# emreatilgan/P-Companion

Measured on AMD Instinct MI355X. Metric: triplets/sec (Product2Vec pretrain step: gather+fwd+bwd+Adam) + P-Companion joint step under `joint`, higher is better.
Workload: dtype f32

## Files before the change

### include/pcompanion_hip.h

```cpp
#ifndef PCOMPANION_HIP_H
#define PCOMPANION_HIP_H

#include <stddef.h>
#include <stdint.h>

#ifdef __cplusplus
extern "C" {
#endif

#define PC_OK 0
#define PC_EINVAL (-1)
#define PC_ESHAPE (-2)
#define PC_EWORKSPACE (-3)
#define PC_EBATCHNORM (-4)
#define PC_ECOMM (-5)

#define PC_D 128
#define PC_H 256
#define PC_HEADS 4
#define PC_L 64
#define PC_MAX_SEG 4
#define PC_BN_SYNC_DOUBLES (PC_MAX_SEG * 2 * 256 + PC_MAX_SEG)

#define PC_ABI_VERSION 8
int pc_abi_version(void);
enum { PC_OPT_SIDE_QUEUE = 1, PC_OPT_SORTED_TABLE_GRADIENTS = 2, PC_OPT_BN_FINALIZE_SIDE = 3, PC_OPT_FUSED_LOSS = 4,
       PC_OPT_FUSED_OUT_CHAIN = 5, PC_OPT_BN_FINALIZE_RIDES = 6 };
int pc_set_option(int option, int value);
int pc_get_option(int option, int* value);
int pc_release_device_state(void);
enum {
    PC_FLAG_EXP_NO_MFMA = 1, PC_FLAG_EXP_NO_SPLIT = 2, PC_FLAG_EXP_NO_LDSREAD = 4, PC_FLAG_EXP_NO_DMA = 8,
    PC_FLAG_EXP_NO_SLAB = 16, PC_FLAG_EXP_STAGGER = 32, PC_FLAG_EXP_DMA_L2 = 64, PC_FLAG_NT_TIMING = 128,
    PC_FLAG_JOINT_TIMING = 256, PC_FLAG_CHAIN_TIMING = 512, PC_FLAG_EXP_NO_BARRIER = 1024, PC_FLAG_EXP_NO_VMWAIT = 2048
};
unsigned pc_build_flags(void);

typedef struct {
    float p;
    uint64_t seed, offset;
} pc_dropout;

typedef struct {
    float *w0, *b0, *gamma, *beta, *w3, *b3, *w5, *b5;
    float *in_proj_w, *in_proj_b, *out_proj_w, *out_proj_b;
    float *running_mean, *running_var;
    int64_t *num_batches_tracked;
    pc_dropout dropout;
    int dim;
} pc_p2v_tensors;

typedef struct {
    int nseg;
    int start[PC_MAX_SEG + 1];
    int count[PC_MAX_SEG];
    int weighted_row;
    float weight;
    const float *row_weight;
    int row_weight_start, row_weight_rows;
} pc_segments;

typedef struct {
    float *h0;
    float *a2;
    float *bn_mean;
    float *bn_invstd;
    float *bn_scale;
    float *bn_shift;
    float *a1;
} pc_ffn_saved;

size_t pc_p2v_ffn_workspace_bytes(int rows);
int pc_p2v_ffn_forward_train(const pc_p2v_tensors *p, const float *table, const int32_t *idx,
                             int rows, const pc_segments *seg, int update_running,
                             float *y, const pc_ffn_saved *saved, void *ws, size_t ws_bytes,
                             void *stream);

int pc_p2v_ffn_forward_eval(const pc_p2v_tensors *p, const float *table, const int32_t *idx,
                            int rows, float *y, void *ws, size_t ws_bytes, void *stream);

int pc_p2v_ffn_backward(const pc_p2v_tensors *p, const pc_p2v_tensors *g, const float *table,
                        const int32_t *idx, int rows, const pc_segments *seg, const float *dy,
                        const pc_ffn_saved *saved, float *dx, int accumulate, void *ws,
                        size_t ws_bytes, void *stream);

typedef struct {
    float *q, *qt, *probs, *c, *sp, *ctx;
} pc_attn_saved;
size_t pc_p2v_attention_workspace_bytes(int batch, int n_keys);
size_t pc_p2v_attention_workspace_bytes_dim(int batch, int n_keys, int dim);
int pc_p2v_attention_forward(const pc_p2v_tensors *p, const float *query, const float *keys,
                             int batch, int n_keys, float *out, const pc_attn_saved *saved,
                             void *ws, size_t ws_bytes, void *stream);
int pc_p2v_attention_backward(const pc_p2v_tensors *p, const pc_p2v_tensors *g,
                              const float *query, const float *keys, int batch, int n_keys,
                              const float *dout, const pc_attn_saved *saved, float *dquery,
                              float *dkeys, int accumulate, void *ws, size_t ws_bytes,
                              void *stream);
int pc_p2v_attention_forward_masked(const pc_p2v_tensors *p, const float *query, const float *keys,
                                    const uint8_t *key_pad, int batch, int n_keys, float *out,
                                    const pc_attn_saved *saved, void *ws, size_t ws_bytes, void *stream);
int pc_p2v_attention_backward_masked(const pc_p2v_tensors *p, const pc_p2v_tensors *g,
                                     const float *query, const float *keys, const uint8_t *key_pad, int batch,
                                     int n_keys, const float *dout, const pc_attn_saved *saved, float *dquery,
                                     float *dkeys, int accumulate, void *ws, size_t ws_bytes, void *stream);

size_t pc_p2v_export_workspace_bytes(int chunk_rows, int dim);
int pc_p2v_export_embeddings(const pc_p2v_tensors *p, const float *features, int64_t n_products,
                             const int32_t *cv_rowptr, const int32_t *cv_col, float *e1, float *out,
                             int chunk_rows, void *ws, size_t ws_bytes, void *stream);

int pc_p2v_triplet_loss(const float *a, const float *p, const float *n, int batch, int k_neg,
                        float margin, float *loss, float *d_pos, float *d_neg, float *da,
                        float *dp, float *dn, void *stream);
int pc_p2v_triplet_loss_dim(const float *a, const float *p, const float *n, int batch, int k_neg, int dim,
                            float margin, float *loss, float *d_pos, float *d_neg, float *da,
                            float *dp, float *dn, void *stream);

int pc_adam_step(float *param, const float *grad, float *exp_avg, float *exp_avg_sq, size_t n,
                 int64_t *step_count, float *scalars, double lr, double beta1, double beta2,
                 double eps, void *stream);
int pc_adam_step_at(float *param, const float *grad, float *exp_avg, float *exp_avg_sq, size_t n,
                    int64_t *step_count, int64_t t, double lr, double beta1, double beta2, double eps,
                    void *stream);

size_t pc_p2v_train_step_workspace_bytes(int batch, int n_nbr, int k_neg);
size_t pc_p2v_train_step_workspace_bytes_dim(int batch, int n_nbr, int k_neg, int dim);
int pc_p2v_train_step(const pc_p2v_tensors *p, const pc_p2v_tensors *g, const float *table,
                      const int32_t *anchor_idx, const int32_t *positive_idx,
                      const int32_t *negative_idx, const int32_t *neighbor_idx, int batch,
                      int n_nbr, int k_neg, float margin, float *loss, float *d_pos,
                      float *d_neg, float *anchor_emb, void *profile, void *ws, size_t ws_bytes,
                      void *stream);

int pc_p2v_train_step_compact(const pc_p2v_tensors *p, const pc_p2v_tensors *g, const float *table,
                              const int32_t *anchor_idx, const int32_t *positive_idx,
                              const int32_t *negative_idx, const int32_t *nb_rows, int n_real,
                              const int32_t *slot_row, int batch, int n_nbr, int k_neg, float margin,
                              float *loss, float *d_pos, float *d_neg, float *anchor_emb, void *profile,
                              void *ws, size_t ws_bytes, void *stream);

int pc_p2v_train_step_unique(const pc_p2v_tensors *p, const pc_p2v_tensors *g, const float *table,
                             const int32_t *anchor_idx, const int32_t *positive_idx,
                             const int32_t *negative_idx, const int32_t *nb_rows, const float *nb_weight,
                             int n_unique, const int32_t *slot_row, const int32_t *ref_off,
                             const int32_t *ref_slot, int batch, int n_nbr, int k_neg,
                             float margin, float *loss, float *d_pos, float *d_neg, float *anchor_emb,
                             void *profile, int phase, double *fwd_sums, double *bwd_local,
                             const double *bwd_global, void *ws, size_t ws_bytes, void *stream);

int pc_p2v_train_step_compact_sync(const pc_p2v_tensors *p, const pc_p2v_tensors *g, const float *table,
                                   const int32_t *anchor_idx, const int32_t *positive_idx,
                                   const int32_t *negative_idx, const int32_t *nb_rows, int n_real,
                                   const int32_t *slot_row, int batch, int n_nbr, int k_neg, float margin,
                                   float *loss, float *d_pos, float *d_neg, float *anchor_emb, int phase,
                                   double *fwd_sums, double *bwd_local, const double *bwd_global,
                                   void *ws, size_t ws_bytes, void *stream);
int pc_build_similarity_batch_compact(const int32_t *pair_ids, int batch, const int32_t *sim_pairs,
                                      const int32_t *cv_rowptr, const int32_t *cv_col,
                                      const int32_t *sim_rowptr, const int32_t *sim_col,
                                      int n_products, int n_pad, int k_neg, uint64_t seed,
                                      uint64_t step, int32_t *anchor_idx, int32_t *positive_idx,
                                      int32_t *negative_idx, int32_t *nb_rows, int32_t *slot_row,
                                      int32_t *row_off, void *stream);

size_t pc_build_similarity_batch_unique_scratch_bytes(int n_products, int max_slots );
int pc_build_similarity_batch_unique(const int32_t *pair_ids, int batch, const int32_t *sim_pairs,
                                     const int32_t *cv_rowptr, const int32_t *cv_col,
                                     const int32_t *sim_rowptr, const int32_t *sim_col, int n_products,
                                     int n_pad, int k_neg, uint64_t seed, uint64_t step, int n_real,
                                     int32_t *anchor_idx, int32_t *positive_idx, int32_t *negative_idx,
                                     int32_t *nb_rows, float *nb_weight, int32_t *slot_row,
                                     int32_t *ref_off, int32_t *ref_slot, int32_t *n_unique, void *scratch,
                                     size_t scratch_bytes, void *stream);

int pc_profile_create(int capacity, void **out);
int pc_profile_destroy(void *profile);
int pc_profile_set_kinds(void *prof, unsigned kinds);
int pc_profile_reset(void *profile);
int pc_profile_summary(void *profile, int kind, int *launches, double *total_ms,
                       double *total_flops);

int pc_build_similarity_batch(const int32_t *pair_ids, int batch, const int32_t *sim_pairs,
                              const int32_t *cv_rowptr, const int32_t *cv_col,
                              const int32_t *sim_rowptr, const int32_t *sim_col, int n_products,
                              int n_pad, int k_neg, uint64_t seed, uint64_t step,
                              int32_t *anchor_idx, int32_t *positive_idx, int32_t *negative_idx,
                              int32_t *neighbor_idx, void *stream);

int pc_build_complementary_batch(const int32_t *pairs, int batch, const float *features,
                                 const int32_t *type_idx, int n_types, uint64_t seed, uint64_t step,
                                 int32_t *query_idx, int32_t *query_types, int32_t *pos_types,
                                 int32_t *neg_types, float *pos_items, float *neg_items,
                                 float *target_features, void *stream);
int pc_build_complementary_batch_dim(const int32_t *pairs, int batch, const float *features,
                                     const int32_t *type_idx, int n_types, int dim, uint64_t seed, uint64_t step,
                                     int32_t *query_idx, int32_t *query_types, int32_t *pos_types,
                                     int32_t *neg_types, float *pos_items, float *neg_items,
                                     float *target_features, void *stream);

size_t pc_mt_state_bytes(void);
int pc_mt_seed(void *state, uint64_t seed);
uint32_t pc_mt_getrandbits(void *state, int k);
uint64_t pc_mt_randbelow(void *state, uint64_t n);
int pc_mt_shuffle(void *state, int64_t *perm, int64_t n);
int pc_mt_negative_samples(void *state, int32_t n_products, const int32_t *sim_rowptr,
                           const int32_t *sim_col, const int32_t *anchors, int64_t n, int k,
                           int32_t *out);

typedef struct {
    float *product_table;
    float *enc_w, *enc_b;
    float *dec_w, *dec_b;
    float *typ_w, *typ_b;
    float *itm_w, *itm_b;
    float *query_types;
    float *comp_types;
    pc_dropout dropout;
} pc_joint_tensors;

typedef struct {
    float *h;
    float *c;
    float *pi;
    float *tp;
} pc_joint_saved;

size_t pc_joint_workspace_bytes(int batch, int num_types, int k);
int pc_joint_forward(const pc_joint_tensors *p, const int32_t *query_idx,
                     const int32_t *query_types, int batch, int num_types, int k, float *sims,
                     int32_t *topk, float *proj, const pc_joint_saved *saved, void *ws,
                     size_t ws_bytes, void *stream);

int pc_joint_loss(const float *sims, const float *proj, const int32_t *pos_types,
                  const int32_t *neg_types, const float *pos_items, const float *neg_items,
                  int batch, int num_types, int k, float margin, float alpha, float *losses,
                  float *dsims_val, float *dproj, float *partials, void *stream);
int pc_joint_loss_dim(const float *sims, const float *proj, const int32_t *pos_types, const int32_t *neg_types,
                      const float *pos_items, const float *neg_items, int batch, int num_types, int k, int dim,
                      float margin, float alpha, float *losses, float *dsims_val, float *dproj, float *partials,
                      void *stream);

int pc_expand_type_grad(const float *dsims_val, const int32_t *pos_types,
                        const int32_t *neg_types, int batch, int num_types, float *dense,
                        void *stream);

int pc_joint_backward(const pc_joint_tensors *p, const pc_joint_tensors *g,
                      const int32_t *query_idx, const int32_t *query_types,
                      const int32_t *pos_types, const int32_t *neg_types, const int32_t *topk,
                      int batch, int num_types, int k, const float *dsims_val,
                      const float *dproj, const pc_joint_saved *saved, void *ws,
                      size_t ws_bytes, void *stream);

int pc_joint_train_step(const pc_joint_tensors *p, const pc_joint_tensors *g,
                        const int32_t *query_idx, const int32_t *query_types,
                        const int32_t *pos_types, const int32_t *neg_types,
                        const float *pos_items, const float *neg_items, int batch,
                        int num_types, int k, float margin, float alpha, float *losses,
                        int32_t *topk, void *ws, size_t ws_bytes, void *stream);

size_t pc_joint_fused_workspace_bytes(int batch, int num_types, int k);
int pc_joint_fused_supported(int num_types, int k, float dropout_p);
int pc_joint_fused_touched(void *ws, size_t ws_bytes, int batch, int num_types, int k, const int32_t **rows_comp,
                           const int32_t **rows_query, const int32_t **n_touched);
int pc_joint_fused_step(const pc_joint_tensors *p, const pc_joint_tensors *g, const pc_joint_tensors *exp_avg,
                        const pc_joint_tensors *exp_avg_sq, int64_t *step_count, double lr, double beta1,
                        double beta2, double eps, const int32_t *query_idx, const int32_t *query_types,
                        const int32_t *pos_types, const int32_t *neg_types, const float *pos_items,
                        const float *neg_items, int batch, int num_types, int k, int num_products, float margin,
                        float alpha, float *losses, int32_t *topk, int32_t *bad_count, void *ws, size_t ws_bytes,
                        void *stream);

int pc_joint_fused_step_pairs(const pc_joint_tensors *p, const pc_joint_tensors *g, const pc_joint_tensors *exp_avg,
                              const pc_joint_tensors *exp_avg_sq, int64_t *step_count, double lr, double beta1,
                              double beta2, double eps, const int32_t *pairs, const float *features,
                              const int32_t *type_idx, int n_types, uint64_t seed, uint64_t step,
                              int32_t *query_idx, int32_t *query_types, int32_t *pos_types, int32_t *neg_types,
                              float *pos_items, float *neg_items, int batch, int num_types, int k, int num_products,
                              float margin, float alpha, float *losses, int32_t *topk, int32_t *bad_count, void *ws,
                              size_t ws_bytes, void *stream);

int pc_joint_train_epoch(const pc_joint_tensors *p, const pc_joint_tensors *g, const pc_joint_tensors *exp_avg,
                         const pc_joint_tensors *exp_avg_sq, int64_t *step_count, double lr, double beta1,
                         double beta2, double eps, const int32_t *pairs, int64_t n_pairs, const float *features,
                         const int32_t *type_idx, int n_types, uint64_t seed, uint64_t first_step,
                         int32_t *query_idx, int32_t *query_types, int32_t *pos_types, int32_t *neg_types,
                         float *pos_items, float *neg_items, int batch, int drop_last, int num_types, int k,
                         int num_products, float margin, float alpha, float *losses_out, int32_t *topk,
                         int32_t *bad_count, void *ws, size_t ws_bytes, void *stream);

typedef struct pc_adam_fused {
    float *param, *grad, *exp_avg, *exp_avg_sq;
    size_t n;
    int64_t *step_count;
    int64_t t;
    double lr, beta1, beta2, eps;
} pc_adam_fused;
int pc_p2v_train_step_unique_adam(const pc_p2v_tensors *p, const pc_p2v_tensors *g, const float *table,
                                  const int32_t *anchor_idx, const int32_t *positive_idx,
                                  const int32_t *negative_idx, const int32_t *nb_rows, const float *nb_weight,
                                  int n_unique, const int32_t *slot_row, const int32_t *ref_off,
                                  const int32_t *ref_slot, int batch, int n_nbr, int k_neg, float margin,
                                  float *loss, float *d_pos, float *d_neg, float *anchor_emb, void *profile,
                                  void *ws, size_t ws_bytes, const pc_adam_fused *adam, void *stream);

int pc_p2v_concat_step_rows(const int32_t *anchor_idx, const int32_t *positive_idx, const int32_t *negative_idx,
                            const int32_t *nb_rows, const int32_t *n_unique_dev, int nb_capacity, int batch, int k_neg,
                            int32_t *rows_out, int rows_capacity, void *stream);
int pc_p2v_train_step_unique_rows(const pc_p2v_tensors *p, const pc_p2v_tensors *g, const float *table,
                                  const int32_t *step_rows, const int32_t *nb_rows, const float *nb_weight, int n_unique,
                                  const int32_t *slot_row, const int32_t *ref_off, const int32_t *ref_slot, int batch,
                                  int n_nbr, int k_neg, float margin, float *loss, float *d_pos, float *d_neg,
                                  float *anchor_emb, void *profile, void *ws, size_t ws_bytes, const pc_adam_fused *adam,
                                  void *stream);

int pc_p2v_train_step_compact_masked(const pc_p2v_tensors *p, const pc_p2v_tensors *g, const float *table,
                                     const int32_t *anchor_idx, const int32_t *positive_idx,
                                     const int32_t *negative_idx, const int32_t *nb_rows, int n_real,
                                     const int32_t *slot_row, int batch, int n_nbr, int k_neg, float margin,
                                     float *loss, float *d_pos, float *d_neg, float *anchor_emb, void *profile,
                                     void *ws, size_t ws_bytes, void *stream);
int pc_p2v_train_step_unique_masked(const pc_p2v_tensors *p, const pc_p2v_tensors *g, const float *table,
                                    const int32_t *anchor_idx, const int32_t *positive_idx,
                                    const int32_t *negative_idx, const int32_t *step_rows, const int32_t *nb_rows,
                                    const float *nb_weight, int n_unique, int n_real_slots, const int32_t *slot_row,
                                    const int32_t *ref_off, const int32_t *ref_slot, int batch, int n_nbr, int k_neg,
                                    float margin, float *loss, float *d_pos, float *d_neg, float *anchor_emb,
                                    void *profile, void *ws, size_t ws_bytes, const pc_adam_fused *adam, void *stream);

typedef int (*pc_exchange_fn)(void *ctx, float *grad, size_t n, void *stream);

int pc_exchange_adam(pc_exchange_fn exchange, void *exchange_ctx, float *param, float *grad, float *exp_avg,
                     float *exp_avg_sq, size_t n, int64_t *step_count, int64_t t, float *scalars, double lr,
                     double beta1, double beta2, double eps, void *stream);

typedef int (*pc_shard_collective_fn)(void *ctx, float *buf, size_t n_per_rank, void *stream);
typedef struct pc_exchange_plan {
    pc_exchange_fn all_reduce_mean;
    pc_shard_collective_fn reduce_scatter_mean;
    pc_shard_collective_fn all_gather;
    void *ctx;
    int rank, world;
    int shard_optimizer;
} pc_exchange_plan;
int pc_rccl_reduce_scatter_mean(void *comm, float *buf, size_t n_per_rank, void *stream);
int pc_rccl_all_gather(void *comm, float *buf, size_t n_per_rank, void *stream);
int pc_exchange_adam_plan(const pc_exchange_plan *plan, float *param, float *grad, float *exp_avg, float *exp_avg_sq,
                          size_t n, int64_t *step_count, int64_t t, float *scalars, double lr, double beta1, double beta2,
                          double eps, void *stream);

int pc_joint_train_epoch_dp(const pc_joint_tensors *p, const pc_joint_tensors *g, float *param_flat, float *grad_flat,
                            float *exp_avg_flat, float *exp_avg_sq_flat, size_t n_flat, int64_t *step_count,
                            int64_t t_first, float *adam_scalars, double lr, double beta1, double beta2, double eps,
                            pc_exchange_fn exchange, void *exchange_ctx, const int32_t *pairs, int64_t n_pairs,
                            const float *features, const int32_t *type_idx, int n_types, uint64_t seed,
                            uint64_t first_step, int32_t *query_idx, int32_t *query_types, int32_t *pos_types,
                            int32_t *neg_types, float *pos_items, float *neg_items, int batch, int drop_last,
                            int num_types, int k, int num_products, float margin, float alpha, float *losses_out,
                            int32_t *topk, int32_t *bad_count, void *ws, size_t ws_bytes, void *stream);

int pc_joint_train_epoch_plan(const pc_joint_tensors *p, const pc_joint_tensors *g, float *param_flat, float *grad_flat,
                              float *exp_avg_flat, float *exp_avg_sq_flat, size_t n_flat, int64_t *step_count,
                              int64_t t_first, float *adam_scalars, double lr, double beta1, double beta2, double eps,
                              const pc_exchange_plan *plan, const int32_t *pairs, int64_t n_pairs,
                              const float *features, const int32_t *type_idx, int n_types, uint64_t seed,
                              uint64_t first_step, int32_t *query_idx, int32_t *query_types, int32_t *pos_types,
                              int32_t *neg_types, float *pos_items, float *neg_items, int batch, int drop_last,
                              int num_types, int k, int num_products, float margin, float alpha, float *losses_out,
                              int32_t *topk, int32_t *bad_count, void *ws, size_t ws_bytes, void *stream);

int pc_rccl_available(void);
int pc_rccl_unique_id(void *out_128_bytes);
int pc_rccl_comm_create(const void *unique_id_128_bytes, int rank, int world, void **comm_out);
int pc_rccl_comm_destroy(void *comm);
int pc_rccl_allreduce_mean(void *comm, float *grad, size_t n, void *stream);
int pc_rccl_allreduce_sum_f64(void *comm, double *buf, size_t n, void *stream);
int pc_rccl_alltoall(void *comm, const void *send, void *recv, size_t bytes_per_peer, void *stream);
int pc_rccl_comm_stats(void *comm, int64_t *issued, int64_t *chained);
const char *pc_rccl_last_error(void);

int pc_linear_forward(const float *x, const int32_t *idx, int rows, int in_dim, const float *w,
                      const float *b, int out_dim, int act, float *y, void *stream);
int pc_linear_backward_input(const float *dy, int rows, int out_dim, const float *w, int in_dim,
                             int act, const float *y_saved, float *dx, float *wt_scratch,
                             void *stream);
size_t pc_linear_backward_weight_workspace_bytes(int rows, int out_dim, int in_dim);
int pc_linear_backward_weight(const float *dy, int rows, int out_dim, const float *x,
                              const int32_t *idx, int in_dim, float *dw, float *db,
                              int accumulate, void *ws, size_t ws_bytes, void *stream);
int pc_topk_rows(const float *sims, int batch, int num_types, int k, int32_t *idx_out,
                 float *val_out, void *stream);
int pc_hit_rank(const float *sims, int rows, int cols, int32_t *rank, void *stream);
int pc_cosine_rows(const float *x, const float *y, int batch, int k, float *out, void *stream);
int pc_cosine_rows_dim(const float *x, const float *y, int batch, int k, int dim, float *out, void *stream);

int pc_eval_batch_stats(const float *proj, const float *targets, const float *pos_items, const int32_t *types, int batch,
                        int k, int dim, int32_t *stats, float *cos_sum, void *ws, size_t ws_bytes, void *stream);
size_t pc_joint_eval_workspace_bytes(int batch, int num_types, int k, int dim);
int pc_joint_eval_epoch(const pc_joint_tensors *p, const int32_t *pairs, int64_t n_pairs, const float *features,
                        const int32_t *type_idx, int n_types, int dim, uint64_t seed, uint64_t first_step, int batch,
                        int num_types, int k, int num_products, int32_t *stats_out, float *cos_sum_out, double *metrics_out,
                        int32_t *bad_count, void *ws, size_t ws_bytes, void *stream);

int pc_hadamard_forward(const float *pi, const float *tp, int batch, int k, float *proj,
                        void *stream);
int pc_hadamard_forward_dim(const float *pi, const float *tp, int batch, int k, int dim, float *proj, void *stream);
int pc_hadamard_backward(const float *dproj, const float *pi, const float *tp, int batch, int k,
                         float *dpi, float *dtp, void *stream);
int pc_hadamard_backward_dim(const float *dproj, const float *pi, const float *tp, int batch, int k, int dim,
                             float *dpi, float *dtp, void *stream);

int pc_gather_rows(const float *table, const int32_t *idx, int rows, int width, float *out,
                   void *stream);
int pc_scatter_add_rows(float *table, const int32_t *idx, int rows, int width, const float *src,
                        void *stream);
int pc_scatter_add_rows_small(float *table, int table_rows, const int32_t *idx, int rows, int width,
                              const float *src, void *stream);

int pc_scatter_rows(float *out, const int32_t *idx, int rows, int width, const float *src,
                    void *stream);
int pc_act_backward(const float *dy, const float *y, size_t n, int act, float *dx, void *stream);

int pc_sample_negatives_zipf(const int32_t *pair_ids, int batch, const int32_t *sim_pairs,
                             const int32_t *sim_rowptr, const int32_t *sim_col, int n_products, int k_neg,
                             uint64_t seed, uint64_t step, const uint32_t *octave_cum, int n_octaves,
                             const int32_t *perm, int32_t *negative_idx, int32_t *failed, void *stream);

int pc_gen_types(int64_t n_products, int num_types, uint64_t seed, int32_t *type_idx, void *stream);
int pc_gen_features(int64_t first, int64_t stride, int64_t n_local, int dim, int num_types, uint64_t seed,
                    float *features, void *stream);
int pc_gen_degrees(int64_t n_products, double mean_degree, int degree_cap, double comp_mean, uint64_t seed,
                   int32_t *deg, int32_t *comp_cand, void *stream);
size_t pc_scan_scratch_bytes(int64_t n);
int pc_exclusive_scan_i32(const int32_t *in, int64_t n, int32_t *out, int64_t *total_out, void *scratch,
                          size_t scratch_bytes, void *stream);
int pc_gen_coview(int64_t n_products, int num_types, uint64_t seed, const int32_t *cv_rowptr, int32_t *cv_col,
                  int32_t *sim_count, void *stream);
int pc_gen_similarity(int64_t n_products, const int32_t *cv_rowptr, int32_t *cv_col, const int32_t *sim_rowptr,
                      int32_t *sim_pairs, int32_t *sim_col, int32_t *pair_deg, void *stream);
int pc_gen_complementary(int64_t n_products, int num_types, uint64_t seed, const int32_t *comp_cand,
                         const int32_t *cv_rowptr, const int32_t *cv_col, int32_t *count,
                         const int32_t *comp_rowptr, int32_t *comp_pairs, void *stream);

int pc_ingest_count(const int32_t *edges, int64_t n_edges, int64_t n_products, int list_bit, int32_t *cnt, int32_t *bad,
                    void *stream);
int pc_ingest_scatter(const int32_t *edges, int64_t n_edges, int64_t n_products, const int32_t *rowptr, int32_t *cursor,
                      int32_t *bucket, void *stream);
int pc_ingest_row_limits(int *wave_row_max, int *lds_row_max);
size_t pc_ingest_rows_workspace_bytes(int64_t n_products);
int pc_ingest_rows(int64_t n_products, const int32_t *rowptr, int32_t *bucket, int32_t *scratch, int degree_cap,
                   int32_t *full_cnt, int32_t *kept_cnt, int32_t *max_kept, void *ws, size_t ws_bytes, void *stream);
int pc_ingest_flag(int64_t n_products, int32_t *src, const int32_t *src_rowptr, const int32_t *src_cnt, const int32_t *need,
                   const int32_t *need_rowptr, const int32_t *need_cnt, const int32_t *forbid1,
                   const int32_t *forbid1_rowptr, const int32_t *forbid1_cnt, const int32_t *forbid2,
                   const int32_t *forbid2_rowptr, const int32_t *forbid2_cnt, int32_t *count, void *stream);
int pc_ingest_emit(int64_t n_products, int32_t *src, const int32_t *src_rowptr, const int32_t *src_cnt,
                   const int32_t *out_rowptr, int32_t *out_col, int32_t *out_pairs, int32_t *out_deg,
                   const int32_t *deg_rowptr, int clear, void *stream);

int pc_epoch_permutation(int n, uint64_t seed, uint64_t epoch, int32_t *out, void *stream);
int pc_shuffle_rows_i32(const int32_t *rows, int n, int width, uint64_t seed, uint64_t epoch, int32_t *out,
                        void *stream);
int pc_comp_split_pairs(const int32_t *comp_pairs, int64_t n_comp, const int32_t *sim_pairs, int64_t n_sim, int64_t lo,
                        int64_t hi, uint64_t seed, int mode, int32_t *out, void *stream);
int pc_epoch_plan(const int32_t *order, const int32_t *deg, int n, int batch, int n_batches, int64_t *plan,
                  void *stream);

int pc_shard_bucket(const int32_t *const *ids, const int *n, const int32_t *const *n_dev, const int *n_dev_add,
                    int32_t *const *remap_out, int count, int world, int capacity, int32_t *counts,
                    int32_t *send_ids, int32_t *overflow, void *stream);
int pc_shard_bucket_hot(const int32_t *const *ids, const int *n, const int32_t *const *n_dev, const int *n_dev_add,
                        int32_t *const *remap_out, int count, int world, int capacity, const int32_t *hot_ids,
                        int hot_rows, int32_t *counts, int32_t *send_ids, int32_t *overflow, int32_t *hot_served,
                        void *stream);

int pc_dropout_hidden(const float *x, size_t n, const pc_dropout *d, float *y, void *stream);

int pc_check_indices(const int32_t *const *idx, const int *n, const int *hi, const int *allow_pad, int count,
                     int32_t *bad, void *stream);

int pc_retrieve_topk(const float *proj, const int32_t *types, int rows, const int32_t *type_rowptr,
                     const int32_t *type_col, const float *table, int n_types, int n, int32_t *out_idx,
                     float *out_score, void *stream);
int pc_retrieve_topk_dim(const float *proj, const int32_t *types, int rows, const int32_t *type_rowptr,
                        const int32_t *type_col, const float *table, int n_types, int n, int dim, int32_t *out_idx,
                        float *out_score, void *stream);
size_t pc_retrieve_topk_grouped_workspace_bytes(int rows, int n_types, int n, int slices);
int pc_retrieve_topk_grouped(const float *proj, const int32_t *types, int rows, const int32_t *type_rowptr,
                             const int32_t *type_col, const float *table, int n_types, int n, int dim, int slices,
                             int32_t *out_idx, float *out_score, void *ws, size_t ws_bytes, void *stream);

size_t pc_rank_grouped_workspace_bytes(int rows, int n_types, int slices);
int pc_rank_grouped(const float *proj, const int32_t *types, const int32_t *targets, int rows,
                    const int32_t *type_rowptr, const int32_t *type_col, const float *table,
                    int n_types, int num_products, int dim, int slices,
                    int32_t *rank_out, int32_t *bad_count, void *ws, size_t ws_bytes, void *stream);

size_t pc_retrieve_topk_grouped_excluding_workspace_bytes(int rows, int n_types, int n, int slices);
int pc_retrieve_topk_grouped_excluding(const float *proj, const int32_t *types, const int32_t *row_key, int rows,
                                       const int32_t *type_rowptr, const int32_t *type_col, const float *table, int n_types,
                                       const int32_t *ex_rowptr, const int32_t *ex_col, int n_keys, int n, int dim, int slices,
                                       int32_t *out_idx, float *out_score, int32_t *bad_count, void *ws, size_t ws_bytes,
                                       void *stream);
int pc_rank_grouped_excluding(const float *proj, const int32_t *types, const int32_t *targets, const int32_t *row_key, int rows,
                              const int32_t *type_rowptr, const int32_t *type_col, const float *table, int n_types,
                              int num_products, const int32_t *ex_rowptr, const int32_t *ex_col, int n_keys,
                              const int32_t *cand_type, int dim, int slices, int32_t *rank_out, int32_t *bad_count, void *ws,
                              size_t ws_bytes, void *stream);

size_t pc_retrieve_list_grouped_workspace_bytes(int rows, int n_types, int n, int slices);
int pc_retrieve_list_grouped(const float *proj, const int32_t *types, const int32_t *row_key, int rows,
                             const int32_t *type_rowptr, const int32_t *type_col, const float *table, int n_types,
                             const int32_t *ex_rowptr, const int32_t *ex_col, int n_keys, int n, int dim, int slices,
                             int32_t *out_idx, float *out_score, int32_t *bad_count, void *ws, size_t ws_bytes,
                             void *stream);

size_t pc_retrieve_topk_grouped_bf16_workspace_bytes(int rows, int n_types, int n, int slices);
int pc_retrieve_topk_grouped_bf16(const float *proj, const int32_t *types, const int32_t *row_key, int rows,
                                  const int32_t *type_rowptr, const int32_t *type_col, const uint16_t *table_bf16,
                                  int n_types, const int32_t *ex_rowptr, const int32_t *ex_col, int n_keys, int n, int dim,
                                  int slices, int32_t *out_idx, float *out_score, int32_t *bad_count, void *ws,
                                  size_t ws_bytes, void *stream);

int pc_half_sq_norm_bias(const float *table, int rows, int dim, float *out, void *stream);
size_t pc_retrieve_topk_grouped_biased_workspace_bytes(int rows, int n_types, int n, int slices);
int pc_retrieve_topk_grouped_biased(const float *proj, const int32_t *types, const int32_t *row_key, int rows,
                                    const int32_t *type_rowptr, const int32_t *type_col, const float *table,
                                    const float *bias, int n_types, const int32_t *ex_rowptr, const int32_t *ex_col,
                                    int n_keys, int n, int dim, int slices, int32_t *out_idx, float *out_score,
                                    int32_t *bad_count, void *ws, size_t ws_bytes, void *stream);
size_t pc_rank_grouped_biased_workspace_bytes(int rows, int n_types, int slices);
int pc_rank_grouped_biased(const float *proj, const int32_t *types, const int32_t *targets, const int32_t *row_key, int rows,
                           const int32_t *type_rowptr, const int32_t *type_col, const float *table, const float *bias,
                           int n_types, int num_products, const int32_t *ex_rowptr, const int32_t *ex_col, int n_keys,
                           const int32_t *cand_type, int dim, int slices, int32_t *rank_out, int32_t *bad_count, void *ws,
                           size_t ws_bytes, void *stream);

size_t pc_joint_query_grad_workspace_bytes(int batch, int k, int dim);
int pc_joint_query_grad(const pc_joint_tensors *p, const int32_t *query_idx, const int32_t *topk, const float *pos_items,
                        const float *neg_items, int batch, int64_t num_products, int num_types, int k, int dim, float margin,
                        float alpha, float *dq, int32_t *bad, void *ws, size_t ws_bytes, void *stream);
size_t pc_sparse_adam_rows_workspace_bytes(int rows);
int pc_sparse_adam_rows(float *table, float *exp_avg, float *exp_avg_sq, int64_t num_products, int dim, const int32_t *idx,
                        const float *grad, int rows, int64_t t, double lr, double beta1, double beta2, double eps,
                        int32_t *bad, void *ws, size_t ws_bytes, void *stream);

int pc_cell_means(const float *table, const int32_t *cell_rowptr, const int32_t *cell_col, int n_cells, int num_products,
                  int dim, float *centroids, void *stream);
int pc_merge_lists(const int32_t *idx, const float *score, int rows, int L, int n, int32_t *out_idx, float *out_score,
                   void *stream);

int pc_diversify_lists(const int32_t *idx, const float *score, int rows, int m, const float *table, const float *scale,
                       int num_products, int dim, int n, float lam, int32_t *out_idx, float *out_score, int32_t *bad_count,
                       void *stream);
int pc_inv_norm(const float *table, int rows, int dim, float *out, void *stream);

size_t pc_retrieve_list_grouped_bf16_workspace_bytes(int rows, int n_types, int n, int slices);
int pc_retrieve_list_grouped_bf16(const float *proj, const int32_t *types, const int32_t *row_key, int rows,
                                  const int32_t *type_rowptr, const int32_t *type_col, const uint16_t *table_bf16,
                                  int n_types, const int32_t *ex_rowptr, const int32_t *ex_col, int n_keys, int n, int dim,
                                  int slices, int32_t *out_idx, float *out_score, int32_t *bad_count, void *ws,
                                  size_t ws_bytes, void *stream);
int pc_diversify_lists_bf16(const int32_t *idx, const float *score, int rows, int m, const uint16_t *table_bf16,
                            const float *scale, int num_products, int dim, int n, float lam, int32_t *out_idx,
                            float *out_score, int32_t *bad_count, void *stream);
int pc_inv_norm_bf16(const uint16_t *table_bf16, int rows, int dim, float *out, void *stream);

#ifdef __cplusplus
}
#endif
#endif
```

### p_companion_amd/_lib.py

```python
import ctypes
import os

_HERE = os.path.dirname(os.path.abspath(__file__))
LIB_PATH = os.path.join(_HERE, "libpcompanion_hip.so")
if os.environ.get("PC_DEV_LIB"):
    import sys as _sys
    LIB_PATH = os.path.abspath(os.environ["PC_DEV_LIB"])
    print(f"[p_companion_amd] PC_DEV_LIB: loading {LIB_PATH} instead of the in-tree library (developer A/B run)", file=_sys.stderr, flush=True)

c_f32p = ctypes.c_void_p
c_i32p = ctypes.c_void_p
PC_MAX_SEG = 4
D, H, HEADS, L = 128, 256, 4, 64

_ERR = {-1: "PC_EINVAL (null pointer / bad size)", -2: "PC_ESHAPE (unsupported dimension/alignment)",
        -3: "PC_EWORKSPACE (workspace too small)",
        -4: "PC_EBATCHNORM (a BatchNorm call group of one row in training mode)",
        -5: "PC_ECOMM (RCCL could not be loaded, or a communicator call failed)"}


class HipKernelError(RuntimeError):
    pass


class Dropout(ctypes.Structure):
    _fields_ = [("p", ctypes.c_float), ("seed", ctypes.c_uint64), ("offset", ctypes.c_uint64)]


class P2VTensors(ctypes.Structure):
    _fields_ = [(n, ctypes.c_void_p) for n in (
        "w0", "b0", "gamma", "beta", "w3", "b3", "w5", "b5", "in_proj_w", "in_proj_b", "out_proj_w",
        "out_proj_b", "running_mean", "running_var", "num_batches_tracked")] + [("dropout", Dropout), ("dim", ctypes.c_int)]


class Segments(ctypes.Structure):
    _fields_ = [("nseg", ctypes.c_int), ("start", ctypes.c_int * (PC_MAX_SEG + 1)),
                ("count", ctypes.c_int * PC_MAX_SEG), ("weighted_row", ctypes.c_int), ("weight", ctypes.c_float),
                ("row_weight", ctypes.c_void_p), ("row_weight_start", ctypes.c_int), ("row_weight_rows", ctypes.c_int)]


class FfnSaved(ctypes.Structure):
    _fields_ = [(n, ctypes.c_void_p) for n in ("h0", "a2", "bn_mean", "bn_invstd", "bn_scale", "bn_shift", "a1")]


class AttnSaved(ctypes.Structure):
    _fields_ = [(n, ctypes.c_void_p) for n in ("q", "qt", "probs", "c", "sp", "ctx")]


class JointTensors(ctypes.Structure):
    _fields_ = [(n, ctypes.c_void_p) for n in (
        "product_table", "enc_w", "enc_b", "dec_w", "dec_b", "typ_w", "typ_b", "itm_w", "itm_b",
        "query_types", "comp_types")] + [("dropout", Dropout)]


class JointSaved(ctypes.Structure):
    _fields_ = [(n, ctypes.c_void_p) for n in ("h", "c", "pi", "tp")]


_vp, _i, _sz, _f, _d, _u64, _i64 = (ctypes.c_void_p, ctypes.c_int, ctypes.c_size_t, ctypes.c_float,
                                    ctypes.c_double, ctypes.c_uint64, ctypes.c_int64)
_P = ctypes.POINTER

class AdamFused(ctypes.Structure):
    _fields_ = [("param", ctypes.c_void_p), ("grad", ctypes.c_void_p), ("exp_avg", ctypes.c_void_p), ("exp_avg_sq", ctypes.c_void_p),
                ("n", ctypes.c_size_t), ("step_count", ctypes.c_void_p), ("t", ctypes.c_int64),
                ("lr", ctypes.c_double), ("beta1", ctypes.c_double), ("beta2", ctypes.c_double), ("eps", ctypes.c_double)]


PC_OPT_SIDE_QUEUE = 1
PC_OPT_FUSED_OUT_CHAIN = 5
PC_OPT_FUSED_LOSS = 4
PC_OPT_BN_FINALIZE_SIDE = 3
PC_OPT_BN_FINALIZE_RIDES = 6
PC_OPT_SORTED_TABLE_GRADIENTS = 2

SIGNATURES = {
    "pc_abi_version": (_i, []),
    "pc_build_flags": (ctypes.c_uint, []),
    "pc_set_option": (_i, [_i, _i]),
    "pc_get_option": (_i, [_i, ctypes.POINTER(ctypes.c_int)]),
    "pc_release_device_state": (_i, []),
    "pc_p2v_ffn_workspace_bytes": (_sz, [_i]),
    "pc_p2v_ffn_forward_train": (_i, [_P(P2VTensors), _vp, _vp, _i, _P(Segments), _i, _vp, _P(FfnSaved), _vp, _sz, _vp]),
    "pc_p2v_ffn_forward_eval": (_i, [_P(P2VTensors), _vp, _vp, _i, _vp, _vp, _sz, _vp]),
    "pc_p2v_ffn_backward": (_i, [_P(P2VTensors), _P(P2VTensors), _vp, _vp, _i, _P(Segments), _vp, _P(FfnSaved),
                                 _vp, _i, _vp, _sz, _vp]),
    "pc_p2v_attention_workspace_bytes": (_sz, [_i, _i]),
    "pc_p2v_attention_workspace_bytes_dim": (_sz, [_i, _i, _i]),
    "pc_p2v_attention_forward": (_i, [_P(P2VTensors), _vp, _vp, _i, _i, _vp, _P(AttnSaved), _vp, _sz, _vp]),
    "pc_p2v_attention_backward": (_i, [_P(P2VTensors), _P(P2VTensors), _vp, _vp, _i, _i, _vp, _P(AttnSaved), _vp,
                                       _vp, _i, _vp, _sz, _vp]),
    "pc_p2v_attention_forward_masked": (_i, [_P(P2VTensors), _vp, _vp, _vp, _i, _i, _vp, _P(AttnSaved), _vp, _sz, _vp]),
    "pc_p2v_attention_backward_masked": (_i, [_P(P2VTensors), _P(P2VTensors), _vp, _vp, _vp, _i, _i, _vp, _P(AttnSaved), _vp,
                                              _vp, _i, _vp, _sz, _vp]),
    "pc_p2v_train_step_compact_masked": (_i, [_P(P2VTensors), _P(P2VTensors), _vp, _vp, _vp, _vp, _vp, _i, _vp, _i, _i, _i, _f,
                                              _vp, _vp, _vp, _vp, _vp, _vp, _sz, _vp]),
    "pc_p2v_train_step_unique_masked": (_i, [_P(P2VTensors), _P(P2VTensors), _vp, _vp, _vp, _vp, _vp, _vp, _vp, _i, _i, _vp, _vp,
                                             _vp, _i, _i, _i, _f, _vp, _vp, _vp, _vp, _vp, _vp, _sz, _P(AdamFused), _vp]),
    "pc_p2v_export_workspace_bytes": (_sz, [_i, _i]),
    "pc_p2v_export_embeddings": (_i, [_P(P2VTensors), _vp, _i64, _vp, _vp, _vp, _vp, _i, _vp, _sz, _vp]),
    "pc_p2v_triplet_loss": (_i, [_vp, _vp, _vp, _i, _i, _f, _vp, _vp, _vp, _vp, _vp, _vp, _vp]),
    "pc_p2v_triplet_loss_dim": (_i, [_vp, _vp, _vp, _i, _i, _i, _f, _vp, _vp, _vp, _vp, _vp, _vp, _vp]),
    "pc_adam_step": (_i, [_vp, _vp, _vp, _vp, _sz, _vp, _vp, _d, _d, _d, _d, _vp]),
    "pc_adam_step_at": (_i, [_vp, _vp, _vp, _vp, _sz, _vp, _i64, _d, _d, _d, _d, _vp]),
    "pc_p2v_train_step_workspace_bytes": (_sz, [_i, _i, _i]),
    "pc_p2v_train_step_workspace_bytes_dim": (_sz, [_i, _i, _i, _i]),
    "pc_p2v_train_step": (_i, [_P(P2VTensors), _P(P2VTensors), _vp, _vp, _vp, _vp, _vp, _i, _i, _i, _f, _vp, _vp,
                               _vp, _vp, _vp, _vp, _sz, _vp]),
    "pc_p2v_train_step_compact": (_i, [_P(P2VTensors), _P(P2VTensors), _vp, _vp, _vp, _vp, _vp, _i, _vp, _i, _i, _i, _f,
                                       _vp, _vp, _vp, _vp, _vp, _vp, _sz, _vp]),
    "pc_p2v_train_step_unique_adam": (_i, [_P(P2VTensors), _P(P2VTensors), _vp, _vp, _vp, _vp, _vp, _vp, _i, _vp, _vp, _vp, _i, _i,
                                           _i, _f, _vp, _vp, _vp, _vp, _vp, _vp, _sz, _P(AdamFused), _vp]),
    "pc_p2v_concat_step_rows": (_i, [_vp, _vp, _vp, _vp, _vp, _i, _i, _i, _vp, _i, _vp]),
    "pc_p2v_train_step_unique_rows": (_i, [_P(P2VTensors), _P(P2VTensors), _vp, _vp, _vp, _vp, _i, _vp, _vp, _vp, _i, _i,
                                           _i, _f, _vp, _vp, _vp, _vp, _vp, _vp, _sz, _P(AdamFused), _vp]),
    "pc_p2v_train_step_unique": (_i, [_P(P2VTensors), _P(P2VTensors), _vp, _vp, _vp, _vp, _vp, _vp, _i, _vp, _vp, _vp, _i, _i,
                                      _i, _f, _vp, _vp, _vp, _vp, _vp, _i, _vp, _vp, _vp, _vp, _sz, _vp]),
    "pc_build_similarity_batch_unique_scratch_bytes": (_sz, [_i, _i]),
    "pc_build_similarity_batch_unique": (_i, [_vp, _i, _vp, _vp, _vp, _vp, _vp, _i, _i, _i, _u64, _u64, _i, _vp, _vp, _vp,
                                              _vp, _vp, _vp, _vp, _vp, _vp, _vp, _sz, _vp]),
    "pc_p2v_train_step_compact_sync": (_i, [_P(P2VTensors), _P(P2VTensors), _vp, _vp, _vp, _vp, _vp, _i, _vp, _i, _i, _i,
                                            _f, _vp, _vp, _vp, _vp, _i, _vp, _vp, _vp, _vp, _sz, _vp]),
    "pc_build_similarity_batch_compact": (_i, [_vp, _i, _vp, _vp, _vp, _vp, _vp, _i, _i, _i, _u64, _u64, _vp, _vp, _vp,
                                               _vp, _vp, _vp, _vp]),
    "pc_profile_create": (_i, [_i, _P(ctypes.c_void_p)]),
    "pc_profile_destroy": (_i, [_vp]),
    "pc_profile_reset": (_i, [_vp]),
    "pc_profile_set_kinds": (_i, [_vp, ctypes.c_uint]),
    "pc_profile_summary": (_i, [_vp, _i, _P(ctypes.c_int), _P(ctypes.c_double), _P(ctypes.c_double)]),
    "pc_build_similarity_batch": (_i, [_vp, _i, _vp, _vp, _vp, _vp, _vp, _i, _i, _i, _u64, _u64, _vp, _vp, _vp,
                                       _vp, _vp]),
    "pc_build_complementary_batch": (_i, [_vp, _i, _vp, _vp, _i, _u64, _u64, _vp, _vp, _vp, _vp, _vp, _vp, _vp, _vp]),
    "pc_build_complementary_batch_dim": (_i, [_vp, _i, _vp, _vp, _i, _i, _u64, _u64, _vp, _vp, _vp, _vp, _vp, _vp, _vp, _vp]),
    "pc_mt_state_bytes": (_sz, []),
    "pc_mt_seed": (_i, [_vp, _u64]),
    "pc_mt_getrandbits": (ctypes.c_uint32, [_vp, _i]),
    "pc_mt_randbelow": (_u64, [_vp, _u64]),
    "pc_mt_shuffle": (_i, [_vp, _vp, _i64]),
    "pc_mt_negative_samples": (_i, [_vp, ctypes.c_int32, _vp, _vp, _vp, _i64, _i, _vp]),
    "pc_joint_workspace_bytes": (_sz, [_i, _i, _i]),
    "pc_joint_forward": (_i, [_P(JointTensors), _vp, _vp, _i, _i, _i, _vp, _vp, _vp, _P(JointSaved), _vp, _sz, _vp]),
    "pc_joint_loss": (_i, [_vp, _vp, _vp, _vp, _vp, _vp, _i, _i, _i, _f, _f, _vp, _vp, _vp, _vp, _vp]),
    "pc_joint_loss_dim": (_i, [_vp, _vp, _vp, _vp, _vp, _vp, _i, _i, _i, _i, _f, _f, _vp, _vp, _vp, _vp, _vp]),
    "pc_expand_type_grad": (_i, [_vp, _vp, _vp, _i, _i, _vp, _vp]),
    "pc_joint_backward": (_i, [_P(JointTensors), _P(JointTensors), _vp, _vp, _vp, _vp, _vp, _i, _i, _i, _vp, _vp,
                               _P(JointSaved), _vp, _sz, _vp]),
    "pc_joint_train_step": (_i, [_P(JointTensors), _P(JointTensors), _vp, _vp, _vp, _vp, _vp, _vp, _i, _i, _i, _f,
                                 _f, _vp, _vp, _vp, _sz, _vp]),
    "pc_joint_fused_workspace_bytes": (_sz, [_i, _i, _i]),
    "pc_joint_fused_supported": (_i, [_i, _i, _f]),
    "pc_joint_fused_touched": (_i, [_vp, _sz, _i, _i, _i, _P(ctypes.c_void_p), _P(ctypes.c_void_p), _P(ctypes.c_void_p)]),
    "pc_joint_fused_step": (_i, [_P(JointTensors), _P(JointTensors), _P(JointTensors), _P(JointTensors), _vp, _d, _d, _d, _d,
                                 _vp, _vp, _vp, _vp, _vp, _vp, _i, _i, _i, _i, _f, _f, _vp, _vp, _vp, _vp, _sz, _vp]),
    "pc_joint_fused_step_pairs": (_i, [_P(JointTensors), _P(JointTensors), _P(JointTensors), _P(JointTensors), _vp, _d, _d, _d, _d,
                                       _vp, _vp, _vp, _i, _u64, _u64, _vp, _vp, _vp, _vp, _vp, _vp, _i, _i, _i, _i, _f, _f,
                                       _vp, _vp, _vp, _vp, _sz, _vp]),
    "pc_joint_train_epoch": (_i, [_P(JointTensors), _P(JointTensors), _P(JointTensors), _P(JointTensors), _vp, _d, _d, _d, _d,
                                  _vp, _i64, _vp, _vp, _i, _u64, _u64, _vp, _vp, _vp, _vp, _vp, _vp, _i, _i, _i, _i, _i, _f, _f,
                                  _vp, _vp, _vp, _vp, _sz, _vp]),
    "pc_exchange_adam": (_i, [_vp, _vp, _vp, _vp, _vp, _vp, _sz, _vp, _i64, _vp, _d, _d, _d, _d, _vp]),
    "pc_joint_train_epoch_dp": (_i, [_P(JointTensors), _P(JointTensors), _vp, _vp, _vp, _vp, _sz, _vp, _i64, _vp, _d, _d, _d, _d,
                                     _vp, _vp, _vp, _i64, _vp, _vp, _i, _u64, _u64, _vp, _vp, _vp, _vp, _vp, _vp, _i, _i, _i, _i,
                                     _i, _f, _f, _vp, _vp, _vp, _vp, _sz, _vp]),
    "pc_exchange_adam_plan": (_i, [_vp, _vp, _vp, _vp, _vp, _sz, _vp, _i64, _vp, _d, _d, _d, _d, _vp]),
    "pc_joint_train_epoch_plan": (_i, [_P(JointTensors), _P(JointTensors), _vp, _vp, _vp, _vp, _sz, _vp, _i64, _vp, _d, _d, _d, _d,
                                       _vp, _vp, _i64, _vp, _vp, _i, _u64, _u64, _vp, _vp, _vp, _vp, _vp, _vp, _i, _i, _i, _i,
                                       _i, _f, _f, _vp, _vp, _vp, _vp, _sz, _vp]),
    "pc_rccl_reduce_scatter_mean": (_i, [_vp, _vp, _sz, _vp]),
    "pc_rccl_all_gather": (_i, [_vp, _vp, _sz, _vp]),
    "pc_rccl_available": (_i, []),
    "pc_rccl_unique_id": (_i, [_vp]),
    "pc_rccl_comm_create": (_i, [_vp, _i, _i, _P(ctypes.c_void_p)]),
    "pc_rccl_comm_destroy": (_i, [_vp]),
    "pc_rccl_allreduce_mean": (_i, [_vp, _vp, _sz, _vp]),
    "pc_rccl_allreduce_sum_f64": (_i, [_vp, _vp, _sz, _vp]),
    "pc_rccl_alltoall": (_i, [_vp, _vp, _vp, _sz, _vp]),
    "pc_rccl_comm_stats": (_i, [_vp, _P(ctypes.c_int64), _P(ctypes.c_int64)]),
    "pc_rccl_last_error": (ctypes.c_char_p, []),
    "pc_linear_forward": (_i, [_vp, _vp, _i, _i, _vp, _vp, _i, _i, _vp, _vp]),
    "pc_linear_backward_input": (_i, [_vp, _i, _i, _vp, _i, _i, _vp, _vp, _vp, _vp]),
    "pc_linear_backward_weight_workspace_bytes": (_sz, [_i, _i, _i]),
    "pc_linear_backward_weight": (_i, [_vp, _i, _i, _vp, _vp, _i, _vp, _vp, _i, _vp, _sz, _vp]),
    "pc_topk_rows": (_i, [_vp, _i, _i, _i, _vp, _vp, _vp]),
    "pc_hit_rank": (_i, [_vp, _i, _i, _vp, _vp]),
    "pc_cosine_rows": (_i, [_vp, _vp, _i, _i, _vp, _vp]),
    "pc_cosine_rows_dim": (_i, [_vp, _vp, _i, _i, _i, _vp, _vp]),
    "pc_eval_batch_stats": (_i, [_vp, _vp, _vp, _vp, _i, _i, _i, _vp, _vp, _vp, _sz, _vp]),
    "pc_joint_eval_workspace_bytes": (_sz, [_i, _i, _i, _i]),
    "pc_joint_eval_epoch": (_i, [_P(JointTensors), _vp, _i64, _vp, _vp, _i, _i, _u64, _u64, _i, _i, _i, _i, _vp, _vp, _vp,
                                 _vp, _vp, _sz, _vp]),
    "pc_retrieve_topk": (_i, [_vp, _vp, _i, _vp, _vp, _vp, _i, _i, _vp, _vp, _vp]),
    "pc_retrieve_topk_dim": (_i, [_vp, _vp, _i, _vp, _vp, _vp, _i, _i, _i, _vp, _vp, _vp]),
    "pc_retrieve_topk_grouped_workspace_bytes": (_sz, [_i, _i, _i, _i]),
    "pc_retrieve_topk_grouped": (_i, [_vp, _vp, _i, _vp, _vp, _vp, _i, _i, _i, _i, _vp, _vp, _vp, _sz, _vp]),
    "pc_rank_grouped_workspace_bytes": (_sz, [_i, _i, _i]),
    "pc_rank_grouped": (_i, [_vp, _vp, _vp, _i, _vp, _vp, _vp, _i, _i, _i, _i, _vp, _vp, _vp, _sz, _vp]),
    "pc_retrieve_topk_grouped_excluding_workspace_bytes": (_sz, [_i, _i, _i, _i]),
    "pc_retrieve_topk_grouped_excluding": (_i, [_vp, _vp, _vp, _i, _vp, _vp, _vp, _i, _vp, _vp, _i, _i, _i, _i, _vp, _vp, _vp, _vp,
                                                _sz, _vp]),
    "pc_rank_grouped_excluding": (_i, [_vp, _vp, _vp, _vp, _i, _vp, _vp, _vp, _i, _i, _vp, _vp, _i, _vp, _i, _i, _vp, _vp, _vp, _sz,
                                       _vp]),
    "pc_retrieve_list_grouped_workspace_bytes": (_sz, [_i, _i, _i, _i]),
    "pc_retrieve_list_grouped": (_i, [_vp, _vp, _vp, _i, _vp, _vp, _vp, _i, _vp, _vp, _i, _i, _i, _i, _vp, _vp, _vp, _vp, _sz,
                                      _vp]),
    "pc_retrieve_topk_grouped_bf16_workspace_bytes": (_sz, [_i, _i, _i, _i]),
    "pc_retrieve_topk_grouped_bf16": (_i, [_vp, _vp, _vp, _i, _vp, _vp, _vp, _i, _vp, _vp, _i, _i, _i, _i, _vp, _vp, _vp, _vp,
                                           _sz, _vp]),
    "pc_half_sq_norm_bias": (_i, [_vp, _i, _i, _vp, _vp]),
    "pc_retrieve_topk_grouped_biased_workspace_bytes": (_sz, [_i, _i, _i, _i]),
    "pc_retrieve_topk_grouped_biased": (_i, [_vp, _vp, _vp, _i, _vp, _vp, _vp, _vp, _i, _vp, _vp, _i, _i, _i, _i, _vp, _vp, _vp,
                                             _vp, _sz, _vp]),
    "pc_rank_grouped_biased_workspace_bytes": (_sz, [_i, _i, _i]),
    "pc_rank_grouped_biased": (_i, [_vp, _vp, _vp, _vp, _i, _vp, _vp, _vp, _vp, _i, _i, _vp, _vp, _i, _vp, _i, _i, _vp, _vp, _vp,
                                    _sz, _vp]),
    "pc_joint_query_grad_workspace_bytes": (_sz, [_i, _i, _i]),
    "pc_joint_query_grad": (_i, [_P(JointTensors), _vp, _vp, _vp, _vp, _i, _i64, _i, _i, _i, _f, _f, _vp, _vp, _vp, _sz, _vp]),
    "pc_sparse_adam_rows_workspace_bytes": (_sz, [_i]),
    "pc_sparse_adam_rows": (_i, [_vp, _vp, _vp, _i64, _i, _vp, _vp, _i, _i64, _d, _d, _d, _d, _vp, _vp, _sz, _vp]),
    "pc_cell_means": (_i, [_vp, _vp, _vp, _i, _i, _i, _vp, _vp]),
    "pc_merge_lists": (_i, [_vp, _vp, _i, _i, _i, _vp, _vp, _vp]),
    "pc_diversify_lists": (_i, [_vp, _vp, _i, _i, _vp, _vp, _i, _i, _i, _f, _vp, _vp, _vp, _vp]),
    "pc_inv_norm": (_i, [_vp, _i, _i, _vp, _vp]),
    "pc_retrieve_list_grouped_bf16_workspace_bytes": (_sz, [_i, _i, _i, _i]),
    "pc_retrieve_list_grouped_bf16": (_i, [_vp, _vp, _vp, _i, _vp, _vp, _vp, _i, _vp, _vp, _i, _i, _i, _i, _vp, _vp, _vp, _vp,
                                           _sz, _vp]),
    "pc_diversify_lists_bf16": (_i, [_vp, _vp, _i, _i, _vp, _vp, _i, _i, _i, _f, _vp, _vp, _vp, _vp]),
    "pc_inv_norm_bf16": (_i, [_vp, _i, _i, _vp, _vp]),
    "pc_hadamard_forward":(_i, [_vp, _vp, _i, _i, _vp, _vp]),
    "pc_hadamard_forward_dim": (_i, [_vp, _vp, _i, _i, _i, _vp, _vp]),
    "pc_hadamard_backward": (_i, [_vp, _vp, _vp, _i, _i, _vp, _vp, _vp]),
    "pc_hadamard_backward_dim": (_i, [_vp, _vp, _vp, _i, _i, _i, _vp, _vp, _vp]),
    "pc_gather_rows": (_i, [_vp, _vp, _i, _i, _vp, _vp]),
    "pc_scatter_add_rows": (_i, [_vp, _vp, _i, _i, _vp, _vp]),
    "pc_scatter_add_rows_small": (_i, [_vp, _i, _vp, _i, _i, _vp, _vp]),
    "pc_scatter_rows": (_i, [_vp, _vp, _i, _i, _vp, _vp]),
    "pc_act_backward": (_i, [_vp, _vp, _sz, _i, _vp, _vp]),
    "pc_sample_negatives_zipf": (_i, [_vp, _i, _vp, _vp, _vp, _i, _i, _u64, _u64, _vp, _i, _vp, _vp, _vp, _vp]),
    "pc_epoch_permutation": (_i, [_i, _u64, _u64, _vp, _vp]),
    "pc_gen_types": (_i, [_i64, _i, _u64, _vp, _vp]),
    "pc_gen_features": (_i, [_i64, _i64, _i64, _i, _i, _u64, _vp, _vp]),
    "pc_gen_degrees": (_i, [_i64, ctypes.c_double, _i, ctypes.c_double, _u64, _vp, _vp, _vp]),
    "pc_scan_scratch_bytes": (_sz, [_i64]),
    "pc_exclusive_scan_i32": (_i, [_vp, _i64, _vp, _vp, _vp, _sz, _vp]),
    "pc_gen_coview": (_i, [_i64, _i, _u64, _vp, _vp, _vp, _vp]),
    "pc_gen_similarity": (_i, [_i64, _vp, _vp, _vp, _vp, _vp, _vp, _vp]),
    "pc_gen_complementary": (_i, [_i64, _i, _u64, _vp, _vp, _vp, _vp, _vp, _vp, _vp]),
    "pc_ingest_count": (_i, [_vp, _i64, _i64, _i, _vp, _vp, _vp]),
    "pc_ingest_scatter": (_i, [_vp, _i64, _i64, _vp, _vp, _vp, _vp]),
    "pc_ingest_row_limits": (_i, [_P(ctypes.c_int), _P(ctypes.c_int)]),
    "pc_ingest_rows_workspace_bytes": (_sz, [_i64]),
    "pc_ingest_rows": (_i, [_i64, _vp, _vp, _vp, _i, _vp, _vp, _vp, _vp, _sz, _vp]),
    "pc_ingest_flag": (_i, [_i64, _vp, _vp, _vp, _vp, _vp, _vp, _vp, _vp, _vp, _vp, _vp, _vp, _vp, _vp]),
    "pc_ingest_emit": (_i, [_i64, _vp, _vp, _vp, _vp, _vp, _vp, _vp, _vp, _i, _vp]),
    "pc_shuffle_rows_i32": (_i, [_vp, _i, _i, _u64, _u64, _vp, _vp]),
    "pc_comp_split_pairs": (_i, [_vp, _i64, _vp, _i64, _i64, _i64, _u64, _i, _vp, _vp]),
    "pc_epoch_plan": (_i, [_vp, _vp, _i, _i, _i, _vp, _vp]),
    "pc_shard_bucket": (_i, [_P(ctypes.c_void_p), _P(ctypes.c_int), _P(ctypes.c_void_p), _P(ctypes.c_int), _P(ctypes.c_void_p),
                             _i, _i, _i, _vp, _vp, _vp, _vp]),
    "pc_shard_bucket_hot": (_i, [_P(ctypes.c_void_p), _P(ctypes.c_int), _P(ctypes.c_void_p), _P(ctypes.c_int), _P(ctypes.c_void_p),
                                 _i, _i, _i, _vp, _i, _vp, _vp, _vp, _vp, _vp]),
    "pc_dropout_hidden": (_i, [_vp, _sz, _P(Dropout), _vp, _vp]),
    "pc_check_indices": (_i, [_P(ctypes.c_void_p), _P(ctypes.c_int), _P(ctypes.c_int), _P(ctypes.c_int), _i, _vp, _vp]),
}

_lib = None


def lib():
    global _lib
    if _lib is None:
        if not os.path.exists(LIB_PATH):
            raise HipKernelError(
                f"{LIB_PATH} not found: build it with `python -m p_companion_amd.build` "
                "(hipcc --offload-arch=gfx950).  There is no CPU fallback.")
        import torch
        L = ctypes.CDLL(LIB_PATH)
        for name, (res, args) in SIGNATURES.items():
            fn = getattr(L, name)
            fn.restype = res
            fn.argtypes = args
        _lib = L
    return _lib


def check(rc, what):
    if rc == 0:
        return
    if rc == -4:
        raise ValueError(f"Expected more than 1 value per channel when training, got input size torch.Size([1, {H}])")
    if rc == -5:
        raise HipKernelError(f"{what}: {_ERR[rc]}: {lib().pc_rccl_last_error().decode(errors='replace')}")
    if rc < 0:
        raise HipKernelError(f"{what}: {_ERR.get(rc, rc)}")
    raise HipKernelError(f"{what}: hipError_t {rc}")
```

### p_companion_amd/csrc/common.h

```cpp
#pragma once
#include <hip/hip_runtime.h>
#include <stdint.h>
#include "../../include/pcompanion_hip.h"

typedef float f32x16 __attribute__((ext_vector_type(16)));
typedef float f32x4 __attribute__((ext_vector_type(4)));

#define PC_WAVE 64

#define PC_HIP_TRY(expr)                          \
    do {                                          \
        hipError_t _e = (expr);                   \
        if (_e != hipSuccess) return (int)_e;     \
    } while (0)

#define PC_TRY(expr)                 \
    do {                             \
        int _r = (expr);             \
        if (_r != 0) return _r;      \
    } while (0)

extern thread_local int pc_tls_launch_err;
#define PC_LAUNCH(...)                                                           \
    do {                                                                         \
        (void)hipGetLastError();                                                 \
        hipLaunchKernelGGL(__VA_ARGS__);                                         \
        const hipError_t _le = hipGetLastError();                                \
        if (_le != hipSuccess && pc_tls_launch_err == 0) pc_tls_launch_err = (int)_le; \
    } while (0)

static inline int pc_launch_status() {
    const int e = pc_tls_launch_err;
    pc_tls_launch_err = 0;
    return e;
}

struct SegInfo {
    int nseg;
    int start[PC_MAX_SEG + 1];
    int tile0[PC_MAX_SEG + 1];
    int count[PC_MAX_SEG];
    int wrow;
    float wmult;
    const float* roww;
    int w0, wn;
};

static inline SegInfo make_seginfo(const pc_segments* s, int rows, int tile_rows) {
    SegInfo si;
    si.nseg = 1;
    for (int i = 0; i <= PC_MAX_SEG; i++) { si.start[i] = rows; si.tile0[i] = 0; }
    si.start[0] = 0;
    si.wrow = -1;
    si.wmult = 1.f;
    si.roww = nullptr; si.w0 = 0; si.wn = 0;
    if (s) {
        si.nseg = s->nseg;
        for (int i = 0; i <= s->nseg; i++) si.start[i] = s->start[i];
        for (int i = s->nseg + 1; i <= PC_MAX_SEG; i++) si.start[i] = s->start[s->nseg];
        si.wrow = s->weighted_row;
        si.wmult = s->weight;
        if (s->row_weight && s->row_weight_rows > 0) { si.roww = s->row_weight; si.w0 = s->row_weight_start; si.wn = s->row_weight_rows; }
    }
    for (int i = 0; i < PC_MAX_SEG; i++) {
        const int phys = si.start[i + 1] - si.start[i];
        si.count[i] = (s && i < s->nseg && s->count[i] > 0) ? s->count[i] : phys;
    }
    int t = 0;
    for (int i = 0; i < PC_MAX_SEG; i++) {
        si.tile0[i] = t;
        int n = si.start[i + 1] - si.start[i];
        t += (n + tile_rows - 1) / tile_rows;
    }
    si.tile0[PC_MAX_SEG] = t;
    return si;
}

static inline int seg_valid(const pc_segments* s, int rows) {
    if (!s) return 1;
    if (s->nseg < 1 || s->nseg > PC_MAX_SEG || s->start[0] != 0 || s->start[s->nseg] != rows) return 0;
    for (int i = 0; i < s->nseg; i++)
        if (s->start[i + 1] < s->start[i] || s->count[i] < 0) return 0;
    if (s->weighted_row >= rows || (s->weighted_row >= 0 && s->weight < 0.f)) return 0;
    if (s->row_weight && (s->row_weight_start < 0 || s->row_weight_rows < 0 || s->row_weight_start + s->row_weight_rows > rows))
        return 0;
    return 1;
}

#ifdef __HIPCC__
__device__ __forceinline__ int seg_of_row(const SegInfo& si, int r) {
    int s = 0;
#pragma unroll
    for (int i = 1; i < PC_MAX_SEG; i++) s += (i < si.nseg && r >= si.start[i]) ? 1 : 0;
    return s;
}

__device__ __forceinline__ float row_multiplicity(const SegInfo& si, int r) {
#ifdef PC_EXP_NO_ROWMULT
    return 1.f;
#endif
    if (si.roww && (unsigned)(r - si.w0) < (unsigned)si.wn) return si.roww[r - si.w0];
    return r == si.wrow ? si.wmult : 1.f;
}

__device__ __forceinline__ int seg_of_tile(const SegInfo& si, int t) {
    int s = 0;
#pragma unroll
    for (int i = 1; i < PC_MAX_SEG; i++) s += (i < si.nseg && t >= si.tile0[i]) ? 1 : 0;
    return s;
}

__device__ __forceinline__ float fast_tanh(float x) {
    const float e = __builtin_amdgcn_exp2f(x * 2.8853900817779268f);
    return 1.0f - 2.0f * __builtin_amdgcn_rcpf(e + 1.0f);
}

__device__ __forceinline__ float wave_sum(float v) {
#pragma unroll
    for (int o = 32; o >= 1; o >>= 1) v += __shfl_xor(v, o, 64);
    return v;
}

__device__ __forceinline__ float group16_sum(float v) {
#pragma unroll
    for (int o = 8; o >= 1; o >>= 1) v += __shfl_xor(v, o, 64);
    return v;
}

__device__ __forceinline__ f32x16 mfma32(float a, float b, f32x16 c) {
    return __builtin_amdgcn_mfma_f32_32x32x2f32(a, b, c, 0, 0, 0);
}

typedef __bf16 bf16x8 __attribute__((ext_vector_type(8)));
struct Split3 { bf16x8 p0, p1, p2; };
__device__ __forceinline__ Split3 split3(const float4& lo, const float4& hi) {
    const float v[8] = {lo.x, lo.y, lo.z, lo.w, hi.x, hi.y, hi.z, hi.w};
    unsigned u0[8], u1[8], u2[8];
#pragma unroll
    for (int i = 0; i < 8; i++) {
        u0[i] = __float_as_uint(v[i]);
        const float r1 = v[i] - __uint_as_float(u0[i] & 0xffff0000u);
        u1[i] = __float_as_uint(r1);
        const float r2 = r1 - __uint_as_float(u1[i] & 0xffff0000u);
        u2[i] = __float_as_uint(r2);
    }
    typedef unsigned u32x4 __attribute__((ext_vector_type(4)));
    u32x4 q0, q1, q2;
#pragma unroll
    for (int j = 0; j < 4; j++) {
        q0[j] = __builtin_amdgcn_perm(u0[2 * j + 1], u0[2 * j], 0x07060302u);
        q1[j] = __builtin_amdgcn_perm(u1[2 * j + 1], u1[2 * j], 0x07060302u);
        q2[j] = __builtin_amdgcn_perm(u2[2 * j + 1], u2[2 * j], 0x07060302u);
    }
    Split3 s;
    s.p0 = __builtin_bit_cast(bf16x8, q0);
    s.p1 = __builtin_bit_cast(bf16x8, q1);
    s.p2 = __builtin_bit_cast(bf16x8, q2);
    return s;
}
__device__ __forceinline__ f32x16 mfma_bf16(const bf16x8& a, const bf16x8& b, f32x16 c) {
    return __builtin_amdgcn_mfma_f32_32x32x16_bf16(a, b, c, 0, 0, 0);
}
#define PC_PRIO_MFMA(COND, x) do { if constexpr (COND) __builtin_amdgcn_s_setprio(x); } while (0)
#ifndef PC_PRIO_NT_COND
#define PC_PRIO_NT_COND false
#endif
#ifndef PC_PRIO_TN_COND
#define PC_PRIO_TN_COND (!APRO && !ZPRO)
#endif
#endif

struct DropCfg {
    unsigned thr;
    float scale;
    unsigned k0, k1, c2, c3;
};
enum { PC_DROP_STREAM_ATTENTION = 0, PC_DROP_STREAM_HIDDEN = 1 };
static inline DropCfg make_dropcfg(const pc_dropout& d) {
    DropCfg c = {};
    if (d.p > 0.f) {
        double t = (double)d.p * 4294967296.0;
        c.thr = t >= 4294967295.0 ? 4294967295u : (unsigned)t;
        c.scale = 1.0f / (1.0f - d.p);
        c.k0 = (unsigned)d.seed; c.k1 = (unsigned)(d.seed >> 32);
        c.c2 = (unsigned)d.offset; c.c3 = (unsigned)(d.offset >> 32);
    }
    return c;
}
#ifdef __HIPCC__
__device__ __forceinline__ void pc_dropout_keep4(const DropCfg& c, unsigned group, unsigned stream, float (&m)[4]) {
    unsigned x0 = group, x1 = stream, x2 = c.c2, x3 = c.c3, k0 = c.k0, k1 = c.k1;
#pragma unroll
    for (int r = 0; r < 10; r++) {
        const unsigned long long p0 = (unsigned long long)0xD2511F53u * x0, p1 = (unsigned long long)0xCD9E8D57u * x2;
        const unsigned y0 = (unsigned)(p1 >> 32) ^ x1 ^ k0, y1 = (unsigned)p1;
        const unsigned y2 = (unsigned)(p0 >> 32) ^ x3 ^ k1, y3 = (unsigned)p0;
        x0 = y0; x1 = y1; x2 = y2; x3 = y3;
        k0 += 0x9E3779B9u; k1 += 0xBB67AE85u;
    }
    m[0] = x0 >= c.thr ? c.scale : 0.f; m[1] = x1 >= c.thr ? c.scale : 0.f;
    m[2] = x2 >= c.thr ? c.scale : 0.f; m[3] = x3 >= c.thr ? c.scale : 0.f;
}
__device__ __forceinline__ void pc_adam_update(float& p, float& m, float& v, float g, float step_size, float bc2s,
                                               float omb1, float beta2, float omb2, float eps) {
#pragma clang fp contract(off)
    m = m + (g - m) * omb1;
    v = v * beta2 + (omb2 * g) * g;
    p = p - step_size * (m / (sqrtf(v) / bc2s + eps));
}
__device__ __forceinline__ bool pc_adam_dead(const float4& g, const float4& m, const float4& v) {
    return g.x == 0.f && g.y == 0.f && g.z == 0.f && g.w == 0.f && m.x == 0.f && m.y == 0.f && m.z == 0.f && m.w == 0.f &&
           v.x == 0.f && v.y == 0.f && v.z == 0.f && v.w == 0.f;
}
__device__ __forceinline__ float2 pc_box_muller(uint32_t a, uint32_t b) {
    const float u1 = ((float)(a >> 8) + 0.5f) * (1.0f / 16777216.0f);
    const float u2 = ((float)(b >> 8) + 0.5f) * (1.0f / 16777216.0f);
    const float r = sqrtf(-2.0f * __logf(u1));
    float sn, cs;
    __sincosf(6.283185307179586f * u2, &sn, &cs);
    return make_float2(r * cs, r * sn);
}
__device__ __forceinline__ float4 pc_filler_chunk(uint64_t seed, uint64_t step, uint32_t t) {
    uint32_t x0 = 0u, x1 = t, x2 = (uint32_t)step, x3 = (uint32_t)(step >> 32), k0 = (uint32_t)seed, k1 = (uint32_t)(seed >> 32);
#pragma unroll
    for (int r = 0; r < 10; r++) {
        const uint64_t p0 = (uint64_t)0xD2511F53u * x0, p1 = (uint64_t)0xCD9E8D57u * x2;
        const uint32_t y0 = (uint32_t)(p1 >> 32) ^ x1 ^ k0, y1 = (uint32_t)p1;
        const uint32_t y2 = (uint32_t)(p0 >> 32) ^ x3 ^ k1, y3 = (uint32_t)p0;
        x0 = y0; x1 = y1; x2 = y2; x3 = y3;
        k0 += 0x9E3779B9u; k1 += 0xBB67AE85u;
    }
    const float2 n0 = pc_box_muller(x0, x1), n1 = pc_box_muller(x2, x3);
    return make_float4(n0.x, n0.y, n1.x, n1.y);
}
#endif

#ifdef __HIPCC__
struct Philox {
    uint32_t c[4], k[2], out[4];
    int have;
    __device__ Philox(uint64_t seed, uint64_t step, uint32_t sample) {
        k[0] = (uint32_t)seed; k[1] = (uint32_t)(seed >> 32);
        c[0] = 0; c[1] = sample; c[2] = (uint32_t)step; c[3] = (uint32_t)(step >> 32);
        have = 0;
    }
    __device__ void block() {
        uint32_t x0 = c[0], x1 = c[1], x2 = c[2], x3 = c[3], k0 = k[0], k1 = k[1];
#pragma unroll
        for (int r = 0; r < 10; r++) {
            const uint64_t p0 = (uint64_t)0xD2511F53u * x0, p1 = (uint64_t)0xCD9E8D57u * x2;
            const uint32_t y0 = (uint32_t)(p1 >> 32) ^ x1 ^ k0, y1 = (uint32_t)p1;
            const uint32_t y2 = (uint32_t)(p0 >> 32) ^ x3 ^ k1, y3 = (uint32_t)p0;
            x0 = y0; x1 = y1; x2 = y2; x3 = y3;
            k0 += 0x9E3779B9u; k1 += 0xBB67AE85u;
        }
        out[0] = x0; out[1] = x1; out[2] = x2; out[3] = x3;
        c[0]++;
        have = 4;
    }
    __device__ uint32_t next() {
        if (have == 0) block();
        return out[4 - have--];
    }
    __device__ uint32_t below(uint32_t n) {
        const int bits = 32 - __clz(n);
        uint32_t r = next() >> (32 - bits);
        while (r >= n) r = next() >> (32 - bits);
        return r;
    }
};
#endif

struct pc_profile {
    hipEvent_t* ev;
    int* kind;
    double* flops;
    int capacity, used;
    unsigned kinds;
};
enum { PC_KIND_GEMM_NT = 0, PC_KIND_GEMM_TN = 1, PC_KIND_GEMM_NT_SMALL = 2 };
extern thread_local pc_profile* pc_tls_profile;
struct ProfileScope {
    explicit ProfileScope(pc_profile* p) { pc_tls_profile = p; }
    ~ProfileScope() { pc_tls_profile = nullptr; }
};
int pc_prof_begin(int kind, double flops, hipStream_t st);
void pc_prof_end(int bracket, hipStream_t st);

enum NtPrologue { NT_PRO_NONE = 0, NT_PRO_BNTANH = 1 };
enum NtEpilogue {
    NT_EPI_NONE = 0,
    NT_EPI_TANH = 1,
    NT_EPI_RELU = 2,
    NT_EPI_DTANH = 3,
    NT_EPI_DTANH_BN = 4,
    NT_EPI_DRELU = 5
};
enum NtStats {
    NT_STAT_NONE = 0,
    NT_STAT_SUMSQ = 1,
    NT_STAT_BNBWD = 2
};

struct NtArgs {
    const float* A; int lda; const int32_t* gather;
    const float* W; int ldw;
    const float* bias;
    float* C; int ldc;
    int M, N, K;
    SegInfo seg;
    int prologue; const float* pscale; const float* pshift;
    float* pro_out; int ldpo;
    int epilogue; const float* aux; int ldaux;
    const float* escale; const float* eshift;
    int stats; float* stat_sum; float* stat_aux;
    const float* mean; const float* invstd;
    const float* brs; int ldbrs;
};
int launch_gemm_nt(const NtArgs& a, hipStream_t st);
int gemm_nt_tiles(const SegInfo& si);
#define PC_NT_GROUP 8
struct NtSmallGroup { NtArgs a[PC_NT_GROUP]; int ks_log2[PC_NT_GROUP], block0[PC_NT_GROUP + 1], n; };
static_assert(sizeof(NtSmallGroup) <= 4096, "kernel argument segment");
int launch_gemm_nt_group(const NtArgs* args, int n, hipStream_t st);
enum { NT_MODE_PLAIN = 0, NT_MODE_KHEAD = 1, NT_MODE_AHEAD = 2 };
struct HingeMeanJob { const float* d_pos; const float* d_neg; int B; float margin; float* loss; };
#ifdef __HIPCC__
#define PC_LOSS_MAX_K 8
#define PC_PAIR_EPS 1e-6f
__device__ __forceinline__ void triplet_sample16(const float* __restrict__ a, const float* __restrict__ p, const float* __restrict__ n,
                                                 int b, int B, int K, float margin, bool live, float* d_pos, float* d_neg,
                                                 float* dp, float* dn, bool grads, int l16, float (&ga)[8]) {
    constexpr int D = 128;
    const size_t bb = live ? (size_t)b : 0;
    float av[8], dpv[8], dnv[PC_LOSS_MAX_K][8], dn_j[PC_LOSS_MAX_K];
    {
        const float4 a0 = *reinterpret_cast<const float4*>(a + bb * D + 8 * l16), a1 = *reinterpret_cast<const float4*>(a + bb * D + 8 * l16 + 4);
        const float4 p0 = *reinterpret_cast<const float4*>(p + bb * D + 8 * l16), p1 = *reinterpret_cast<const float4*>(p + bb * D + 8 * l16 + 4);
        av[0] = a0.x; av[1] = a0.y; av[2] = a0.z; av[3] = a0.w; av[4] = a1.x; av[5] = a1.y; av[6] = a1.z; av[7] = a1.w;
        const float pv[8] = {p0.x, p0.y, p0.z, p0.w, p1.x, p1.y, p1.z, p1.w};
#pragma unroll
        for (int c = 0; c < 8; c++) dpv[c] = av[c] - pv[c] + PC_PAIR_EPS;
    }
#pragma unroll
    for (int j = 0; j < PC_LOSS_MAX_K; j++)
        if (j < K) {
            const float* r = n + (bb * K + j) * D + 8 * l16;
            const float4 n0 = *reinterpret_cast<const float4*>(r), n1 = *reinterpret_cast<const float4*>(r + 4);
            const float nv[8] = {n0.x, n0.y, n0.z, n0.w, n1.x, n1.y, n1.z, n1.w};
#pragma unroll
            for (int c = 0; c < 8; c++) dnv[j][c] = av[c] - nv[c] + PC_PAIR_EPS;
        }
    float s = 0.f;
#pragma unroll
    for (int c = 0; c < 8; c++) s += dpv[c] * dpv[c];
    const float dpos = sqrtf(group16_sum(s));
    float dneg = 0.f;
#pragma unroll
    for (int j = 0; j < PC_LOSS_MAX_K; j++)
        if (j < K) {
            float t = 0.f;
#pragma unroll
            for (int c = 0; c < 8; c++) t += dnv[j][c] * dnv[j][c];
            dn_j[j] = sqrtf(group16_sum(t));
            dneg += dn_j[j];
        }
    dneg /= (float)K;
    if (live && l16 == 0) { d_pos[b] = dpos; d_neg[b] = dneg; }
#pragma unroll
    for (int c = 0; c < 8; c++) ga[c] = 0.f;
    if (!grads) return;
    const bool active = (margin - dpos + dneg) > 0.f;
    const float gs = (active && live) ? 1.0f / (float)B : 0.f;
    const float ip = gs / dpos;
#pragma unroll
    for (int c = 0; c < 8; c++) ga[c] = -dpv[c] * ip;
    if (live) {
        *reinterpret_cast<float4*>(dp + bb * D + 8 * l16) = make_float4(dpv[0] * ip, dpv[1] * ip, dpv[2] * ip, dpv[3] * ip);
        *reinterpret_cast<float4*>(dp + bb * D + 8 * l16 + 4) = make_float4(dpv[4] * ip, dpv[5] * ip, dpv[6] * ip, dpv[7] * ip);
    }
#pragma unroll
    for (int j = 0; j < PC_LOSS_MAX_K; j++)
        if (j < K) {
            const float in = gs / ((float)K * dn_j[j]);
#pragma unroll
            for (int c = 0; c < 8; c++) ga[c] += dnv[j][c] * in;
            if (live) {
                float* r = dn + (bb * K + j) * D + 8 * l16;
                *reinterpret_cast<float4*>(r) = make_float4(-dnv[j][0] * in, -dnv[j][1] * in, -dnv[j][2] * in, -dnv[j][3] * in);
                *reinterpret_cast<float4*>(r + 4) = make_float4(-dnv[j][4] * in, -dnv[j][5] * in, -dnv[j][6] * in, -dnv[j][7] * in);
            }
        }
}
#endif

struct LossPro { const float *emb, *pos, *neg; int B, K; float margin; float *d_pos, *d_neg, *dp, *dn, *demb; };
int launch_gemm_nt_chain(const NtArgs* args, const int* modes, int n, hipStream_t st, const HingeMeanJob* rider = nullptr,
                         const LossPro* loss = nullptr);
int launch_gemm_nt_chain_pair(const NtArgs* fwd, const NtArgs* bwd, const LossPro* loss, hipStream_t st);
#ifdef __HIPCC__
__device__ __forceinline__ void hinge_mean_body(const HingeMeanJob& j, float* red ) {
    const int t = threadIdx.x;
    float s = 0.f;
    if (t < 256)
        for (int b = t; b < j.B; b += 256) {
            const float l = j.margin - j.d_pos[b] + j.d_neg[b];
            s += l > 0.f ? l : 0.f;
        }
    if (t < 256) red[t] = s;
    __syncthreads();
    for (int o = 128; o >= 1; o >>= 1) {
        if (t < o) red[t] += red[t + o];
        __syncthreads();
    }
    if (t == 0) *j.loss = red[0] / (float)j.B;
}
#endif

struct TransposeJob { const float* in; float* out; int rows, cols; };
#define PC_TRANSPOSE_JOBS 8
struct TransposeBatch { TransposeJob job[PC_TRANSPOSE_JOBS]; int n; float* zero; int nzero; };
int launch_transpose_batch(const TransposeBatch& tb, hipStream_t st);
#ifdef __HIPCC__
template <int NT>
__device__ __forceinline__ void transpose_tile_body(const TransposeBatch& tb, int tile, int tiles_x, int tiles_y, float (*t)[33], int tid) {
    const int jz = tile / (tiles_x * tiles_y), rem = tile % (tiles_x * tiles_y);
    const TransposeJob j = tb.job[jz];
    const int tx = tid & 31, ty = tid >> 5;
    if (tb.zero && tile == 0)
        for (int i = tid; i < tb.nzero; i += NT) tb.zero[i] = 0.f;
    const int bx = (rem % tiles_x) * 32, by = (rem / tiles_x) * 32;
    if (bx >= j.cols || by >= j.rows) return;
    for (int i = ty; i < 32; i += NT / 32) {
        const int r = by + i, cc = bx + tx;
        t[i][tx] = (r < j.rows && cc < j.cols) ? j.in[(size_t)r * j.cols + cc] : 0.f;
    }
    __syncthreads();
    for (int i = ty; i < 32; i += NT / 32) {
        const int cc = bx + i, r = by + tx;
        if (r < j.rows && cc < j.cols) j.out[(size_t)cc * j.rows + r] = t[tx][i];
    }
}
#endif
static inline void transpose_batch_tiles(const TransposeBatch& tb, int* tiles_x, int* tiles_y) {
    int mx = 0, my = 0;
    for (int i = 0; i < tb.n; i++) { mx = tb.job[i].cols > mx ? tb.job[i].cols : mx; my = tb.job[i].rows > my ? tb.job[i].rows : my; }
    *tiles_x = (mx + 31) / 32; *tiles_y = (my + 31) / 32;
}

struct TnArgs {
    const float* Z; int ldz;
    const float* A; int lda; const int32_t* gather;
    int R, No, Ni;
    SegInfo seg;
    int prologue; const float* pscale; const float* pshift;
    const float* zaux; int ldzaux;
    const float *z_mean, *z_invstd, *z_scale, *z_c1, *z_c2;
    const int32_t* z_onehot;
    float* dW; int lddw; float* db;
    int accumulate;
    float* slabs; size_t slab_floats;
};
struct TnDefer;
int launch_gemm_tn(const TnArgs& a, hipStream_t st, TnDefer* defer = nullptr);
struct TnRider;
int launch_gemm_tn_halves(const TnArgs& a, float* slabs0, float* slabs1, size_t slab_floats, hipStream_t st, TnDefer* defer,
                          const TnRider* rider = nullptr);
size_t gemm_tn_workspace_floats(int R, int No, int Ni);
#define PC_TN_GROUP 10
#define PC_TN_EXTRA 2
#define PC_TN_RGROUP (PC_TN_GROUP + PC_TN_EXTRA + 4)
struct TnGroup { TnArgs a[PC_TN_GROUP]; int tiles_i[PC_TN_GROUP], nsplit[PC_TN_GROUP], rps[PC_TN_GROUP], block0[PC_TN_GROUP + 1], n; };
struct TnReduceJob { const float* slabs; int nsplit, n; float* out; int accumulate; };
#define PC_ADAM_REST (2 * (PC_TN_GROUP + PC_TN_EXTRA + 4) + 1)
struct AdamRider {
    float *p, *m, *v; const float* g; size_t n;
    int64_t* step_count; long long t; double lr, beta1, beta2; float omb1, beta2f, omb2, eps;
    int block0;
    int n_rest, rest_lo[PC_ADAM_REST], rest_hi[PC_ADAM_REST], rest_block0[PC_ADAM_REST + 1];
};
struct TnReduceGroup {
    const float* slabs[PC_TN_RGROUP]; float* dW[PC_TN_RGROUP]; float* db[PC_TN_RGROUP];
    int nsplit[PC_TN_RGROUP], n_w[PC_TN_RGROUP], n_b[PC_TN_RGROUP], accumulate[PC_TN_RGROUP], block0[PC_TN_RGROUP + 1], n;
    AdamRider ad;
};
#define PC_FORK_EVENTS 3
struct PcFork { hipStream_t side; hipEvent_t fork[PC_FORK_EVENTS]; hipEvent_t join[PC_FORK_EVENTS]; int pending; };
PcFork* pc_fork_get(hipStream_t main_st);
int pc_fork_begin(PcFork* f, int i, hipStream_t main_st);
int pc_fork_mark(PcFork* f, int i);
int pc_fork_wait(PcFork* f, int i, hipStream_t main_st);
int pc_fork_join(PcFork* f, int i, hipStream_t main_st);
struct TnDefer { TnReduceGroup r; int rblocks; PcFork* fork; int bn_finalized; const pc_adam_fused* adam; };
static_assert(sizeof(TnGroup) <= 4096, "kernel argument segment");
int launch_gemm_tn_group(const TnArgs* args, int n, const TnReduceJob* extra, int n_extra, hipStream_t st,
                         TnDefer* defer = nullptr);
int launch_tn_reduce_deferred(TnDefer* d, hipStream_t st);
static inline void tn_defer_init(TnDefer* d) { d->r = TnReduceGroup{}; d->rblocks = 0; d->fork = nullptr; d->bn_finalized = 0; d->adam = nullptr; }
int scatter_add_slab_blocks(int table_rows, int rows, int width);
int launch_scatter_add_slabs(const int32_t* idx, int rows, int width, int table_rows, const float* src, float* slabs,
                             hipStream_t st);

struct WsCarver {
    char* base; size_t total;
    explicit WsCarver(void* b) : base(static_cast<char*>(b)), total(0) {}
    void* bytes(size_t n) {
        void* p = base ? base + total : nullptr;
        total += (n + 255) & ~(size_t)255;
        return p;
    }
    float* floats(size_t n) { return static_cast<float*>(bytes(n * sizeof(float))); }
};

static inline void joint_fields(const pc_joint_tensors* t, float* (&out)[10]) {
    float* const f[10] = {t->itm_w, t->itm_b, t->typ_w, t->typ_b, t->dec_w, t->dec_b, t->enc_w, t->enc_b, t->comp_types, t->query_types};
    for (int i = 0; i < 10; i++) out[i] = f[i];
}
static inline bool joint_tensors_ok(const pc_joint_tensors* t, bool need_table) {
    if (!t || (need_table && !t->product_table)) return false;
    float* f[10];
    joint_fields(t, f);
    for (float* x : f)
        if (!x) return false;
    return true;
}

int pc_opt_sorted_tables();
int pc_opt_bn_finalize_side();
int pc_opt_bn_finalize_rides();
int pc_opt_fused_loss();
int pc_opt_fused_out_chain();
int triplet_loss_launch(const float* a, const float* p, const float* n, int batch, int k_neg, int dim, float margin,
                        float* loss, float* d_pos, float* d_neg, float* da, float* dp, float* dn, void* stream, int with_mean);
int launch_dropout(const float* x, size_t n, const pc_dropout& d, unsigned stream_id, float* y, hipStream_t st);
int launch_transpose(const float* in, int rows, int cols, float* out, hipStream_t st);
struct FfnCall {
    const pc_p2v_tensors *p = nullptr, *g = nullptr;
    const float* table = nullptr;
    const int32_t* idx = nullptr;
    int rows = 0;
    const pc_segments* seg = nullptr;
    const pc_ffn_saved* sv = nullptr;
    void* ws = nullptr; size_t ws_bytes = 0; void* stream = nullptr;
    double* local_sums = nullptr; const double* global_sums = nullptr;
    int update_running = 0; float* y = nullptr;
    const TransposeBatch* ride = nullptr;
    const float* dy = nullptr; float* dx = nullptr;
    int with_dx = 0, transposed = 0;
    int accumulate = 0;
    TnDefer* defer = nullptr;
};
int ffn_forward_part1(const FfnCall& c);
int ffn_forward_part2(const FfnCall& c);
int ffn_backward_part1(const FfnCall& c);
int ffn_backward_part2(const FfnCall& c);
int ffn_transposes(const pc_p2v_tensors* p, void* ws, int rows, int with_dx, TransposeBatch* tb);
int attention_transposes(const pc_p2v_tensors* p, void* ws, int B, int N, int key_rows, TransposeBatch* tb, float* zero_bk);
struct AttnCall {
    const pc_p2v_tensors* p = nullptr;
    const float *query = nullptr, *keys = nullptr;
    int B = 0, N = 0, key_rows = 0;
    const int32_t* slot_row = nullptr;
    const pc_attn_saved* sv = nullptr;
    void* ws = nullptr; size_t ws_bytes = 0; void* stream = nullptr;
    bool transposed = false;
    bool masked = false;
    const uint8_t* key_pad = nullptr;
    float* out = nullptr;
    const pc_p2v_tensors* g = nullptr;
    int pad_row = -1;
    const float* dout = nullptr;
    float *dquery = nullptr, *dkeys = nullptr;
    int accumulate = 0;
    const int32_t *ref_off = nullptr, *ref_slot = nullptr;
    TnDefer* defer = nullptr;
    const HingeMeanJob* rider = nullptr;
    const LossPro* loss = nullptr;
    const NtArgs* fwd_out_chain = nullptr;
    NtArgs* defer_out_chain = nullptr;
};
int attention_forward_impl(const AttnCall& c);
int attention_backward_impl(const AttnCall& c);

static inline NtArgs nt_plain(const float* A, int lda, const float* W, int ldw, const float* bias, float* C, int ldc, int M,
                              int N, int K, const SegInfo* si = nullptr) {
    NtArgs a = {};
    a.A = A; a.lda = lda; a.W = W; a.ldw = ldw; a.bias = bias; a.C = C; a.ldc = ldc;
    a.M = M; a.N = N; a.K = K; a.seg = si ? *si : make_seginfo(nullptr, M, 128);
    return a;
}
static inline bool p2v_dim_ok(const pc_p2v_tensors* p) { return p->dim == 0 || p->dim == 128 || p->dim == 256; }
static inline int p2v_dim(const pc_p2v_tensors* p) { return p && p->dim == 256 ? 256 : PC_D; }
```

### p_companion_amd/csrc/ffn.hip

```cpp
#include "common.h"
#include "bn_finalize.h"

#define BN_EPS 1e-5f
#define BN_MOMENTUM 0.1f

#define FIN_LANES 32
__device__ __forceinline__ void fold_partials(const float* p1, const float* p2, int t0, int t1, int j, int q,
                                              double (*red)[FIN_LANES][FIN_COLS], double* o1, double* o2) {
    double a = 0.0, b = 0.0, a1 = 0.0, b1 = 0.0;
    int t = t0 + q;
    for (; t + FIN_LANES < t1; t += 2 * FIN_LANES) {
        a += (double)p1[(size_t)t * PC_H + j];                b += (double)p2[(size_t)t * PC_H + j];
        a1 += (double)p1[(size_t)(t + FIN_LANES) * PC_H + j]; b1 += (double)p2[(size_t)(t + FIN_LANES) * PC_H + j];
    }
    if (t < t1) { a += (double)p1[(size_t)t * PC_H + j]; b += (double)p2[(size_t)t * PC_H + j]; }
    red[0][q][threadIdx.x] = a + a1;
    red[1][q][threadIdx.x] = b + b1;
    __syncthreads();
    if (q == 0) {
        double s1 = 0.0, s2 = 0.0;
#pragma unroll 8
        for (int i = 0; i < FIN_LANES; i++) { s1 += red[0][i][threadIdx.x]; s2 += red[1][i][threadIdx.x]; }
        *o1 = s1; *o2 = s2;
    }
    __syncthreads();
}

__global__ __launch_bounds__(FIN_COLS * FIN_LANES) void bn_fold_kernel(const float* p1, const float* p2, SegInfo si,
                                                                       double* sums) {
    __shared__ double red[2][FIN_LANES][FIN_COLS];
    const int j = blockIdx.x * FIN_COLS + threadIdx.x, q = threadIdx.y;
    for (int s = 0; s < PC_MAX_SEG; s++) {
        double a = 0.0, b = 0.0;
        if (s < si.nseg) fold_partials(p1, p2, si.tile0[s], si.tile0[s + 1], j, q, red, &a, &b);
        if (q == 0) {
            sums[(2 * s) * PC_H + j] = a;
            sums[(2 * s + 1) * PC_H + j] = b;
            if (j == 0) sums[2 * PC_MAX_SEG * PC_H + s] = s < si.nseg ? (double)si.count[s] : 0.0;
        }
    }
}

__global__ __launch_bounds__(FIN4_CG * FIN4_LANES) void bn_finalize_fwd_kernel(
    const float* psum, const float* psq, SegInfo si, const double* gsum, const float* gamma, const float* beta,
    float* running_mean, float* running_var, int64_t* nbt, int update_running, float* mean_o, float* invstd_o,
    float* scale_o, float* shift_o, TransposeBatch ride, int tiles_x, int tiles_y) {
    __shared__ double red[FIN4_WAVES][2][PC_MAX_SEG][FIN_COLS];
    __shared__ float seg_mean[PC_MAX_SEG][FIN_COLS], seg_unb[PC_MAX_SEG][FIN_COLS];
    __shared__ int seg_live[PC_MAX_SEG][FIN_COLS];
    const int tid = threadIdx.y * FIN4_CG + threadIdx.x;
    if (blockIdx.x >= PC_H / FIN_COLS) {
        static_assert(sizeof(red) >= 32 * 33 * sizeof(float), "transpose tile");
        transpose_tile_body<FIN4_CG * FIN4_LANES>(ride, (int)blockIdx.x - PC_H / FIN_COLS, tiles_x, tiles_y,
                                                  reinterpret_cast<float(*)[33]>(&red[0][0][0][0]), tid);
        return;
    }
    double a = 0.0, b = 0.0;
    if (!gsum) fold_partials_all4(psum, psq, si, blockIdx.x * FIN_COLS, tid, red, &a, &b);
    if (tid < PC_MAX_SEG * FIN_COLS) {
        const int s = tid / FIN_COLS, col = tid % FIN_COLS, j = blockIdx.x * FIN_COLS + col;
        double n = s < si.nseg ? (double)si.count[s] : 0.0;
        if (gsum && s < si.nseg) { a = gsum[(2 * s) * PC_H + j]; b = gsum[(2 * s + 1) * PC_H + j]; n = gsum[2 * PC_MAX_SEG * PC_H + s]; }
        int live = 0;
        if (s < si.nseg && n > 0) {
            const double m = a / n;
            double var = b / n - m * m;
            if (var < 0.0) var = 0.0;
            const float mf = (float)m, vf = (float)var;
            const float is = 1.0f / sqrtf(vf + BN_EPS);
            const float sc = gamma[j] * is;
            mean_o[s * PC_H + j] = mf;
            invstd_o[s * PC_H + j] = is;
            scale_o[s * PC_H + j] = sc;
            shift_o[s * PC_H + j] = beta[j] - mf * sc;
            seg_mean[s][col] = mf;
            seg_unb[s][col] = n > 1 ? (float)(var * (n / (n - 1))) : vf;
            live = 1;
        }
        seg_live[s][col] = live;
    }
    __syncthreads();
    if (tid < FIN_COLS && update_running) {
        const int j = blockIdx.x * FIN_COLS + tid;
        float rm = running_mean[j], rv = running_var[j];
        int nseen = 0;
        for (int s = 0; s < si.nseg; s++) {
            if (!seg_live[s][tid]) continue;
            rm = BN_MOMENTUM * seg_mean[s][tid] + (1.0f - BN_MOMENTUM) * rm;
            rv = BN_MOMENTUM * seg_unb[s][tid] + (1.0f - BN_MOMENTUM) * rv;
            nseen++;
        }
        running_mean[j] = rm;
        running_var[j] = rv;
        if (j == 0 && nbt) *nbt += nseen;
    }
}

__global__ void bn_eval_coeff_kernel(const float* gamma, const float* beta, const float* running_mean,
                                     const float* running_var, float* scale_o, float* shift_o) {
    const int j = threadIdx.x;
    const float is = 1.0f / sqrtf(running_var[j] + BN_EPS);
    const float sc = gamma[j] * is;
    scale_o[j] = sc;
    shift_o[j] = beta[j] - running_mean[j] * sc;
}

__global__ __launch_bounds__(FIN4_CG * FIN4_LANES) void bn_finalize_bwd_kernel(
    const float* psum, const float* pdot, SegInfo si, const double* lsum, const double* gsum, const float* mean,
    const float* invstd, float* dgamma, float* dbeta, int accumulate, float* c1, float* c2) {
    __shared__ BnFinBwdScratch sm;
    const BnFinBwd f = {psum, pdot, lsum, gsum, mean, invstd, dgamma, dbeta, accumulate, c1, c2};
    bn_finalize_bwd_body(f, si, (int)blockIdx.x, (int)(threadIdx.y * FIN4_CG + threadIdx.x), &sm);
}

__global__ void bn_bwd_apply_kernel(float* dz, const float* h0, int rows, SegInfo si, const float* mean,
                                    const float* invstd, const float* scale, const float* c1, const float* c2) {
    const int c4 = (threadIdx.x & 63) * 4;
    const int rl = threadIdx.x >> 6;
    for (int r = blockIdx.x * 4 + rl; r < rows; r += gridDim.x * 4) {
        const int s = seg_of_row(si, r);
        const float m = row_multiplicity(si, r);
        float4 g = *reinterpret_cast<float4*>(dz + (size_t)r * PC_H + c4);
        const float4 h = *reinterpret_cast<const float4*>(h0 + (size_t)r * PC_H + c4);
        const float4 mu = *reinterpret_cast<const float4*>(mean + s * PC_H + c4);
        const float4 is = *reinterpret_cast<const float4*>(invstd + s * PC_H + c4);
        const float4 sc = *reinterpret_cast<const float4*>(scale + s * PC_H + c4);
        const float4 a = *reinterpret_cast<const float4*>(c1 + s * PC_H + c4);
        const float4 b = *reinterpret_cast<const float4*>(c2 + s * PC_H + c4);
        g.x = sc.x * (g.x - m * (a.x + (h.x - mu.x) * is.x * b.x));
        g.y = sc.y * (g.y - m * (a.y + (h.y - mu.y) * is.y * b.y));
        g.z = sc.z * (g.z - m * (a.z + (h.z - mu.z) * is.z * b.z));
        g.w = sc.w * (g.w - m * (a.w + (h.w - mu.w) * is.w * b.w));
        *reinterpret_cast<float4*>(dz + (size_t)r * PC_H + c4) = g;
    }
}

__global__ void transpose_kernel(const float* in, int rows, int cols, float* out) {
    __shared__ float t[32][33];
    const int bx = blockIdx.x * 32, by = blockIdx.y * 32;
    for (int i = threadIdx.y; i < 32; i += 8) {
        const int r = by + i, c = bx + threadIdx.x;
        t[i][threadIdx.x] = (r < rows && c < cols) ? in[(size_t)r * cols + c] : 0.f;
    }
    __syncthreads();
    for (int i = threadIdx.y; i < 32; i += 8) {
        const int c = bx + i, r = by + threadIdx.x;
        if (r < rows && c < cols) out[(size_t)c * rows + r] = t[threadIdx.x][i];
    }
}

__global__ void transpose_batch_kernel(TransposeBatch tb) {
    __shared__ float t[32][33];
    const TransposeJob j = tb.job[blockIdx.z];
    const int bx = blockIdx.x * 32, by = blockIdx.y * 32;
    if (tb.zero && blockIdx.x + blockIdx.y + blockIdx.z == 0)
        for (int i = threadIdx.y * 32 + threadIdx.x; i < tb.nzero; i += 256) tb.zero[i] = 0.f;
    if (bx >= j.cols || by >= j.rows) return;
    for (int i = threadIdx.y; i < 32; i += 8) {
        const int r = by + i, c = bx + threadIdx.x;
        t[i][threadIdx.x] = (r < j.rows && c < j.cols) ? j.in[(size_t)r * j.cols + c] : 0.f;
    }
    __syncthreads();
    for (int i = threadIdx.y; i < 32; i += 8) {
        const int c = bx + i, r = by + threadIdx.x;
        if (r < j.rows && c < j.cols) j.out[(size_t)c * j.rows + r] = t[threadIdx.x][i];
    }
}

int launch_transpose_batch(const TransposeBatch& tb, hipStream_t st) {
    int mx = 0, my = 0;
    for (int i = 0; i < tb.n; i++) {
        mx = tb.job[i].cols > mx ? tb.job[i].cols : mx;
        my = tb.job[i].rows > my ? tb.job[i].rows : my;
    }
    PC_LAUNCH(transpose_batch_kernel, dim3((mx + 31) / 32, (my + 31) / 32, tb.n), dim3(32, 8), 0, st, tb);
    return pc_launch_status();
}

int launch_transpose(const float* in, int rows, int cols, float* out, hipStream_t st) {
    PC_LAUNCH(transpose_kernel, dim3((cols + 31) / 32, (rows + 31) / 32), dim3(32, 8), 0, st, in, rows, cols, out);
    return pc_launch_status();
}

struct FfnWs {
    float *stat_a, *stat_b;
    float *dz2, *dz1;
    float *w5t, *w3t, *w0t;
    float *c1, *c2;
    float *coef;
    float *slabs[4]; size_t slab_floats;
    size_t total;
};

static FfnWs ffn_ws_layout(void* base, int rows) {
    FfnWs w;
    const int max_tiles = (rows + 127) / 128 + PC_MAX_SEG;
    WsCarver cv(base);
    auto take = [&](size_t floats) { return cv.floats(floats); };
    w.stat_a = take((size_t)max_tiles * PC_H);
    w.stat_b = take((size_t)max_tiles * PC_H);
    w.dz2 = take((size_t)rows * PC_H);
    w.dz1 = take((size_t)rows * PC_H);
    w.w5t = take(PC_H * 256);
    w.w3t = take(PC_H * PC_H);
    w.w0t = take(256 * PC_H);
    w.c1 = take(PC_MAX_SEG * PC_H);
    w.c2 = take(PC_MAX_SEG * PC_H);
    w.coef = take(2 * PC_H);
    w.slab_floats = gemm_tn_workspace_floats(rows, PC_H, PC_H);
    for (size_t f : {gemm_tn_workspace_floats(rows, PC_D, PC_H), gemm_tn_workspace_floats(rows, PC_H, PC_D)})
        if (f > w.slab_floats) w.slab_floats = f;
    for (int i = 0; i < 4; i++) w.slabs[i] = take(w.slab_floats);
    w.total = cv.total;
    return w;
}

extern "C" size_t pc_p2v_ffn_workspace_bytes(int rows) {
    if (rows <= 0) return 0;
    return ffn_ws_layout(nullptr, rows).total;
}

static int ffn_check(const pc_p2v_tensors* p, const float* table, int rows, const pc_segments* seg, void* ws,
                     size_t ws_bytes) {
    if (!p || !table || rows <= 0 || !ws) return PC_EINVAL;
    if (!p2v_dim_ok(p)) return PC_ESHAPE;
    if (!p->w0 || !p->b0 || !p->gamma || !p->beta || !p->w3 || !p->b3 || !p->w5 || !p->b5) return PC_EINVAL;
    if (!seg_valid(seg, rows)) return PC_EINVAL;
    if (ws_bytes < pc_p2v_ffn_workspace_bytes(rows)) return PC_EWORKSPACE;
    return PC_OK;
}

static int launch_bn_fold(hipStream_t st, const FfnWs& w, const SegInfo& si, double* local_sums) {
    PC_LAUNCH(bn_fold_kernel, dim3(PC_H / FIN_COLS), dim3(FIN_COLS, FIN_LANES), 0, st, w.stat_a, w.stat_b, si, local_sums);
    return pc_launch_status();
}

static int launch_bn_finalize_bwd(hipStream_t st, const BnFinBwd& f, const SegInfo& si) {
    PC_LAUNCH(bn_finalize_bwd_kernel, dim3(PC_H / FIN_COLS), dim3(FIN4_CG, FIN4_LANES), 0, st, f.psum, f.pdot, si, f.lsum, f.gsum, f.mean,
              f.invstd, f.dgamma, f.dbeta, f.accumulate, f.c1, f.c2);
    return pc_launch_status();
}

int ffn_forward_part1(const FfnCall& c) {
    const pc_p2v_tensors* p = c.p;
    const pc_ffn_saved* sv = c.sv;
    const int rows = c.rows;
    PC_TRY(ffn_check(p, c.table, rows, c.seg, c.ws, c.ws_bytes));
    if (!sv || !sv->h0 || !sv->a2 || !sv->bn_mean || !sv->bn_invstd || !sv->bn_scale || !sv->bn_shift) return PC_EINVAL;
    hipStream_t st = (hipStream_t)c.stream;
    const int D = p2v_dim(p);
    const SegInfo si = make_seginfo(c.seg, rows, 128);
    FfnWs w = ffn_ws_layout(c.ws, rows);
    NtArgs g1 = nt_plain(c.table, D, p->w0, D, p->b0, sv->h0, PC_H, rows, PC_H, D, &si);
    g1.gather = c.idx;
    g1.stats = NT_STAT_SUMSQ; g1.stat_sum = w.stat_a; g1.stat_aux = w.stat_b;
    PC_TRY(launch_gemm_nt(g1, st));
    if (c.local_sums) PC_TRY(launch_bn_fold(st, w, si, c.local_sums));
    return PC_OK;
}

int ffn_forward_part2(const FfnCall& c) {
    const pc_p2v_tensors* p = c.p;
    const pc_ffn_saved* sv = c.sv;
    const int rows = c.rows;
    if (!c.y || (c.update_running && (!p->running_mean || !p->running_var))) return PC_EINVAL;
    hipStream_t st = (hipStream_t)c.stream;
    const SegInfo si = make_seginfo(c.seg, rows, 128);
    FfnWs w = ffn_ws_layout(c.ws, rows);
    TransposeBatch tb = {};
    int tiles_x = 0, tiles_y = 0;
    if (c.ride && c.ride->n > 0) { tb = *c.ride; transpose_batch_tiles(tb, &tiles_x, &tiles_y); }
    PC_LAUNCH(bn_finalize_fwd_kernel, dim3(PC_H / FIN_COLS + tiles_x * tiles_y * tb.n), dim3(FIN4_CG, FIN4_LANES), 0, st, w.stat_a,
              w.stat_b, si, c.global_sums, p->gamma, p->beta, p->running_mean, p->running_var, p->num_batches_tracked,
              c.update_running, sv->bn_mean, sv->bn_invstd, sv->bn_scale, sv->bn_shift, tb, tiles_x, tiles_y);
    PC_TRY(pc_launch_status());

    NtArgs g2 = nt_plain(sv->h0, PC_H, p->w3, PC_H, p->b3, sv->a2, PC_H, rows, PC_H, PC_H, &si);
    g2.prologue = NT_PRO_BNTANH; g2.pscale = sv->bn_scale; g2.pshift = sv->bn_shift;
    g2.pro_out = sv->a1; g2.ldpo = PC_H;
    g2.epilogue = NT_EPI_TANH;
    PC_TRY(launch_gemm_nt(g2, st));

    const int D = p2v_dim(p);
    NtArgs g3 = nt_plain(sv->a2, PC_H, p->w5, PC_H, p->b5, c.y, D, rows, D, PC_H, &si);
    return launch_gemm_nt(g3, st);
}

#define FFN_COMMON(c)                                                                                   \
    c.p = p; c.table = table; c.idx = idx; c.rows = rows; c.seg = seg; c.sv = sv;                       \
    c.ws = ws; c.ws_bytes = ws_bytes; c.stream = stream

extern "C" int pc_p2v_ffn_forward_train(const pc_p2v_tensors* p, const float* table, const int32_t* idx, int rows,
                                        const pc_segments* seg, int update_running, float* y,
                                        const pc_ffn_saved* sv, void* ws, size_t ws_bytes, void* stream) {
    if (!y) return PC_EINVAL;
    FfnCall c;
    FFN_COMMON(c);
    c.update_running = update_running; c.y = y;
    PC_TRY(ffn_forward_part1(c));
    return ffn_forward_part2(c);
}

extern "C" int pc_p2v_ffn_forward_eval(const pc_p2v_tensors* p, const float* table, const int32_t* idx, int rows,
                                       float* y, void* ws, size_t ws_bytes, void* stream) {
    PC_TRY(ffn_check(p, table, rows, nullptr, ws, ws_bytes));
    if (!y || !p->running_mean || !p->running_var) return PC_EINVAL;
    hipStream_t st = (hipStream_t)stream;
    const SegInfo si = make_seginfo(nullptr, rows, 128);
    FfnWs w = ffn_ws_layout(ws, rows);
    float* h0 = w.dz2;
    float* a2 = w.dz1;
    PC_LAUNCH(bn_eval_coeff_kernel, dim3(1), dim3(PC_H), 0, st, p->gamma, p->beta, p->running_mean,
                       p->running_var, w.coef, w.coef + PC_H);
    PC_TRY(pc_launch_status());
    const int D = p2v_dim(p);
    NtArgs g1 = nt_plain(table, D, p->w0, D, p->b0, h0, PC_H, rows, PC_H, D, &si);
    g1.gather = idx;
    PC_TRY(launch_gemm_nt(g1, st));
    NtArgs g2 = nt_plain(h0, PC_H, p->w3, PC_H, p->b3, a2, PC_H, rows, PC_H, PC_H, &si);
    g2.prologue = NT_PRO_BNTANH; g2.pscale = w.coef; g2.pshift = w.coef + PC_H;
    g2.epilogue = NT_EPI_TANH;
    PC_TRY(launch_gemm_nt(g2, st));
    NtArgs g3 = nt_plain(a2, PC_H, p->w5, PC_H, p->b5, y, D, rows, D, PC_H, &si);
    return launch_gemm_nt(g3, st);
}

int ffn_transposes(const pc_p2v_tensors* p, void* ws, int rows, int with_dx, TransposeBatch* tb) {
    FfnWs w = ffn_ws_layout(ws, rows);
    const int D = p2v_dim(p);
    if (tb->n + 2 + (with_dx ? 1 : 0) > PC_TRANSPOSE_JOBS) return PC_EINVAL;
    tb->job[tb->n++] = {p->w5, w.w5t, D, PC_H};
    tb->job[tb->n++] = {p->w3, w.w3t, PC_H, PC_H};
    if (with_dx) tb->job[tb->n++] = {p->w0, w.w0t, PC_H, D};
    return PC_OK;
}

int ffn_backward_part1(const FfnCall& c) {
    const pc_p2v_tensors *p = c.p, *g = c.g;
    const pc_ffn_saved* sv = c.sv;
    const float* dy = c.dy;
    const int rows = c.rows, accumulate = c.accumulate;
    PC_TRY(ffn_check(p, c.table, rows, c.seg, c.ws, c.ws_bytes));
    if (!g || !dy || !sv || !sv->h0 || !sv->a2) return PC_EINVAL;
    if (!g->w0 || !g->b0 || !g->gamma || !g->beta || !g->w3 || !g->b3 || !g->w5 || !g->b5) return PC_EINVAL;
    hipStream_t st = (hipStream_t)c.stream;
    const SegInfo si = make_seginfo(c.seg, rows, 128);
    FfnWs w = ffn_ws_layout(c.ws, rows);
    TnDefer own;
    tn_defer_init(&own);
    TnDefer* df = c.defer ? c.defer : &own;

    const int D = p2v_dim(p);
    if (!c.transposed) {
        TransposeBatch tb = {};
        PC_TRY(ffn_transposes(p, c.ws, rows, c.with_dx, &tb));
        PC_TRY(launch_transpose_batch(tb, st));
    }

    NtArgs b1 = nt_plain(dy, D, w.w5t, D, nullptr, w.dz2, PC_H, rows, PC_H, D, &si);
    b1.epilogue = NT_EPI_DTANH; b1.aux = sv->a2; b1.ldaux = PC_H;
    PC_TRY(launch_gemm_nt(b1, st));

    TnArgs t5 = {};
    t5.Z = dy; t5.ldz = D; t5.A = sv->a2; t5.lda = PC_H; t5.R = rows; t5.No = D; t5.Ni = PC_H; t5.seg = si;
    t5.dW = g->w5; t5.lddw = PC_H; t5.db = g->b5; t5.accumulate = accumulate; t5.slabs = w.slabs[0];
    t5.slab_floats = w.slab_floats;
    if (D == 256 && rows >= 8192 && (size_t)2 * 128 * ((size_t)128 * PC_H + 128) <= w.slab_floats) {
        const size_t half = (size_t)128 * ((size_t)128 * PC_H + 128);
        PC_TRY(launch_gemm_tn_halves(t5, w.slabs[0], w.slabs[0] + half, half, st, df));
    } else {
        PC_TRY(launch_gemm_tn(t5, st, df));
    }

    NtArgs b2 = nt_plain(w.dz2, PC_H, w.w3t, PC_H, nullptr, w.dz1, PC_H, rows, PC_H, PC_H, &si);
    b2.epilogue = NT_EPI_DTANH_BN; b2.aux = sv->h0; b2.ldaux = PC_H; b2.escale = sv->bn_scale; b2.eshift = sv->bn_shift;
    b2.stats = NT_STAT_BNBWD; b2.stat_sum = w.stat_a; b2.stat_aux = w.stat_b;
    PC_TRY(launch_gemm_nt(b2, st));
    TnRider fin_rider = {};
    if (df->fork && !c.local_sums) {
        const BnFinBwd fin = {w.stat_a, w.stat_b, nullptr, nullptr, sv->bn_mean, sv->bn_invstd, g->gamma, g->beta, accumulate, w.c1, w.c2};
        if (pc_opt_bn_finalize_side()) {
            PC_TRY(pc_fork_begin(df->fork, 1, st));
            PC_TRY(launch_bn_finalize_bwd(df->fork->side, fin, si));
            df->bn_finalized = 1;
        } else if (pc_opt_bn_finalize_rides() && sv->a1 && rows >= 8192 && (size_t)128 * ((size_t)128 * PC_H + 128) <= w.slab_floats) {
            fin_rider.n = PC_TN_RIDERS;
            fin_rider.fin = fin;
            fin_rider.si = si;
            df->bn_finalized = 2;
        } else {
            PC_TRY(launch_bn_finalize_bwd(st, fin, si));
            df->bn_finalized = 2;
        }
    }

    TnArgs t3 = {};
    t3.Z = w.dz2; t3.ldz = PC_H; t3.A = sv->a1 ? sv->a1 : sv->h0; t3.lda = PC_H; t3.R = rows; t3.No = PC_H; t3.Ni = PC_H; t3.seg = si;
    if (!sv->a1) { t3.prologue = NT_PRO_BNTANH; t3.pscale = sv->bn_scale; t3.pshift = sv->bn_shift; }
    t3.dW = g->w3; t3.lddw = PC_H; t3.db = g->b3; t3.accumulate = accumulate; t3.slabs = w.slabs[1];
    t3.slab_floats = w.slab_floats;
    if (sv->a1) {
        if (rows >= 8192 && (size_t)128 * ((size_t)128 * PC_H + 128) <= w.slab_floats) {
            PC_TRY(launch_gemm_tn_halves(t3, w.slabs[1], w.slabs[2], w.slab_floats, st, df, fin_rider.n ? &fin_rider : nullptr));
        } else {
            for (int half = 0; half < 2; half++) {
                TnArgs th = t3;
                th.Z = w.dz2 + half * (PC_H / 2); th.No = PC_H / 2;
                th.dW = g->w3 + (size_t)half * (PC_H / 2) * PC_H; th.db = g->b3 + half * (PC_H / 2);
                th.slabs = w.slabs[1 + half];
                PC_TRY(launch_gemm_tn(th, st, df));
            }
        }
    } else {
        PC_TRY(launch_gemm_tn(t3, st, df));
    }
    if (c.local_sums) PC_TRY(launch_bn_fold(st, w, si, c.local_sums));
    if (!c.defer) PC_TRY(launch_tn_reduce_deferred(&own, st));
    return PC_OK;
}

int ffn_backward_part2(const FfnCall& c) {
    const pc_p2v_tensors* g = c.g;
    const pc_ffn_saved* sv = c.sv;
    float* const dx = c.dx;
    const int rows = c.rows, accumulate = c.accumulate;
    TnDefer* const defer = c.defer;
    hipStream_t st = (hipStream_t)c.stream;
    const SegInfo si = make_seginfo(c.seg, rows, 128);
    FfnWs w = ffn_ws_layout(c.ws, rows);
    if (defer && defer->bn_finalized) {
        if (c.local_sums || c.global_sums) return PC_EINVAL;
        if (defer->bn_finalized == 1) PC_TRY(pc_fork_join(defer->fork, 0, st));
    } else {
        const BnFinBwd fin = {w.stat_a, w.stat_b, c.local_sums, c.global_sums, sv->bn_mean, sv->bn_invstd, g->gamma, g->beta, accumulate,
                              w.c1, w.c2};
        PC_TRY(launch_bn_finalize_bwd(st, fin, si));
    }

    const int D = p2v_dim(g);
    TnArgs t0 = {};
    t0.Z = w.dz1; t0.ldz = PC_H; t0.A = c.table; t0.lda = D; t0.gather = c.idx; t0.R = rows; t0.No = PC_H;
    t0.Ni = D; t0.seg = si;
    t0.dW = g->w0; t0.lddw = D; t0.db = g->b0; t0.accumulate = accumulate; t0.slabs = w.slabs[3];
    t0.slab_floats = w.slab_floats;
    if (dx) {
        int blocks = (rows + 3) / 4;
        if (blocks > 4096) blocks = 4096;
        PC_LAUNCH(bn_bwd_apply_kernel, dim3(blocks), dim3(256), 0, st, w.dz1, sv->h0, rows, si, sv->bn_mean,
                  sv->bn_invstd, sv->bn_scale, w.c1, w.c2);
        PC_TRY(pc_launch_status());
    } else {
        t0.zaux = sv->h0; t0.ldzaux = PC_H;
        t0.z_mean = sv->bn_mean; t0.z_invstd = sv->bn_invstd; t0.z_scale = sv->bn_scale; t0.z_c1 = w.c1; t0.z_c2 = w.c2;
    }
    PC_TRY(launch_gemm_tn(t0, st, defer));

    if (dx) {
        NtArgs b3 = nt_plain(w.dz1, PC_H, w.w0t, PC_H, nullptr, dx, D, rows, D, PC_H, &si);
        PC_TRY(launch_gemm_nt(b3, st));
    }
    return PC_OK;
}

extern "C" int pc_p2v_ffn_backward(const pc_p2v_tensors* p, const pc_p2v_tensors* g, const float* table,
                                   const int32_t* idx, int rows, const pc_segments* seg, const float* dy,
                                   const pc_ffn_saved* sv, float* dx, int accumulate, void* ws, size_t ws_bytes,
                                   void* stream) {
    TnDefer df;
    tn_defer_init(&df);
    FfnCall c;
    FFN_COMMON(c);
    c.g = g; c.dy = dy; c.dx = dx; c.with_dx = dx != nullptr; c.accumulate = accumulate; c.defer = &df;
    PC_TRY(ffn_backward_part1(c));
    PC_TRY(ffn_backward_part2(c));
    return launch_tn_reduce_deferred(&df, (hipStream_t)stream);
}
```

### p_companion_amd/csrc/gemm_tn.hip

```cpp
#include <atomic>
#include <mutex>
#include <type_traits>
#include "common.h"
#include "bn_finalize.h"
#include "lds_dma.h"

#define TM 128
#define TK 32

__device__ __forceinline__ void tn_small_body(const TnArgs& a, int tiles_i, int nsplit, int rows_per_split, int bid) {
    __shared__ __attribute__((aligned(16))) float smem[2][2][TK * TM];

    const int tid = threadIdx.x, lane = tid & 63, w = tid >> 6, wo = w >> 1, wi = w & 1;
    const int split = bid % nsplit;
    const int tile = bid / nsplit;
    const int o0 = (tile / tiles_i) * TM, i0 = (tile % tiles_i) * TM;
    const int r_begin = split * rows_per_split;
    const int r_end = min(a.R, r_begin + rows_per_split);

    const int lrow = tid >> 5, lcol = (tid & 31) * 4;
    const bool zcol_ok = o0 + lcol < a.No, acol_ok = i0 + lcol < a.Ni;

    float4 rz[4], ra[4];
    float4 dbacc = make_float4(0.f, 0.f, 0.f, 0.f);
    int zseg = -1;
    float4 zmu, zis, zsc, zc1, zc2;
    auto gload = [&](int r0) {
#pragma unroll
        for (int p = 0; p < 4; p++) {
            const int r = r0 + lrow + 8 * p;
            const bool rv = r < r_end;
            if (a.z_onehot) {
                const int t = rv ? a.z_onehot[r] : -1, c = o0 + lcol;
                rz[p] = make_float4(t == c ? 1.f : 0.f, t == c + 1 ? 1.f : 0.f, t == c + 2 ? 1.f : 0.f, t == c + 3 ? 1.f : 0.f);
            } else {
                rz[p] = (rv && zcol_ok) ? *reinterpret_cast<const float4*>(a.Z + (size_t)r * a.ldz + o0 + lcol)
                                        : make_float4(0.f, 0.f, 0.f, 0.f);
            }
            if (a.zaux && rv && zcol_ok) {
                const int s = seg_of_row(a.seg, r);
                if (s != zseg) {
                    const size_t o = (size_t)s * a.No + o0 + lcol;
                    zmu = *reinterpret_cast<const float4*>(a.z_mean + o);
                    zis = *reinterpret_cast<const float4*>(a.z_invstd + o);
                    zsc = *reinterpret_cast<const float4*>(a.z_scale + o);
                    zc1 = *reinterpret_cast<const float4*>(a.z_c1 + o);
                    zc2 = *reinterpret_cast<const float4*>(a.z_c2 + o);
                    zseg = s;
                }
                const float4 h = *reinterpret_cast<const float4*>(a.zaux + (size_t)r * a.ldzaux + o0 + lcol);
                const float zm = row_multiplicity(a.seg, r);
                rz[p].x = zsc.x * (rz[p].x - zm * (zc1.x + (h.x - zmu.x) * zis.x * zc2.x));
                rz[p].y = zsc.y * (rz[p].y - zm * (zc1.y + (h.y - zmu.y) * zis.y * zc2.y));
                rz[p].z = zsc.z * (rz[p].z - zm * (zc1.z + (h.z - zmu.z) * zis.z * zc2.z));
                rz[p].w = zsc.w * (rz[p].w - zm * (zc1.w + (h.w - zmu.w) * zis.w * zc2.w));
            }
            int src = r;
            bool av = rv && acol_ok;
            if (av && a.gather) { src = a.gather[r]; av = src >= 0; }
            ra[p] = av ? *reinterpret_cast<const float4*>(a.A + (size_t)src * a.lda + i0 + lcol)
                       : make_float4(0.f, 0.f, 0.f, 0.f);
            if (a.prologue == NT_PRO_BNTANH && rv && acol_ok) {
                const int s = seg_of_row(a.seg, r);
                const float4 sc = *reinterpret_cast<const float4*>(a.pscale + (size_t)s * a.Ni + i0 + lcol);
                const float4 sh = *reinterpret_cast<const float4*>(a.pshift + (size_t)s * a.Ni + i0 + lcol);
                ra[p].x = fast_tanh(ra[p].x * sc.x + sh.x);
                ra[p].y = fast_tanh(ra[p].y * sc.y + sh.y);
                ra[p].z = fast_tanh(ra[p].z * sc.z + sh.z);
                ra[p].w = fast_tanh(ra[p].w * sc.w + sh.w);
            }
            dbacc.x += rz[p].x; dbacc.y += rz[p].y; dbacc.z += rz[p].z; dbacc.w += rz[p].w;
        }
    };
    auto lstore = [&](int buf) {
#pragma unroll
        for (int p = 0; p < 4; p++) {
            *reinterpret_cast<float4*>(&smem[buf][0][(lrow + 8 * p) * TM + lcol]) = rz[p];
            *reinterpret_cast<float4*>(&smem[buf][1][(lrow + 8 * p) * TM + lcol]) = ra[p];
        }
    };

    f32x16 acc[2][2];
#pragma unroll
    for (int i = 0; i < 2; i++)
#pragma unroll
        for (int j = 0; j < 2; j++)
#pragma unroll
            for (int r = 0; r < 16; r++) acc[i][j][r] = 0.f;

    const int nchunk = (r_end - r_begin + TK - 1) / TK;
    if (nchunk > 0) {
        gload(r_begin);
        lstore(0);
    }
    __syncthreads();
    const int fz = (lane >> 5) * TM + wo * 64 + (lane & 31);
    const int fa = (lane >> 5) * TM + wi * 64 + (lane & 31);
    const bool vz0 = __builtin_amdgcn_readfirstlane(o0 + wo * 64 < a.No), vz1 = __builtin_amdgcn_readfirstlane(o0 + wo * 64 + 32 < a.No);
    const bool vx0 = __builtin_amdgcn_readfirstlane(i0 + wi * 64 < a.Ni), vx1 = __builtin_amdgcn_readfirstlane(i0 + wi * 64 + 32 < a.Ni);
    for (int c = 0; c < nchunk; c++) {
        const int cur = c & 1;
        if (c + 1 < nchunk) gload(r_begin + (c + 1) * TK);
        const float* Zs = &smem[cur][0][fz];
        const float* As = &smem[cur][1][fa];
#pragma unroll
        for (int k = 0; k < TK; k += 2) {
            const float z0 = Zs[k * TM], z1 = Zs[k * TM + 32];
            const float x0 = As[k * TM], x1 = As[k * TM + 32];
            if (vz0 && vx0) acc[0][0] = mfma32(z0, x0, acc[0][0]);
            if (vz0 && vx1) acc[0][1] = mfma32(z0, x1, acc[0][1]);
            if (vz1 && vx0) acc[1][0] = mfma32(z1, x0, acc[1][0]);
            if (vz1 && vx1) acc[1][1] = mfma32(z1, x1, acc[1][1]);
        }
        if (c + 1 < nchunk) lstore(cur ^ 1);
        __syncthreads();
    }

    float* slab = a.slabs + (size_t)split * ((size_t)a.No * a.Ni + a.No);
#pragma unroll
    for (int mt = 0; mt < 2; mt++)
#pragma unroll
        for (int nt = 0; nt < 2; nt++) {
            const int i = i0 + wi * 64 + nt * 32 + (lane & 31);
#pragma unroll
            for (int reg = 0; reg < 16; reg++) {
                const int o = o0 + wo * 64 + mt * 32 + (reg & 3) + 8 * (reg >> 2) + 4 * (lane >> 5);
                if (o < a.No && i < a.Ni) slab[(size_t)o * a.Ni + i] = acc[mt][nt][reg];
            }
        }
    if (a.db && i0 == 0) {
        float* red = &smem[0][0][0];
        *reinterpret_cast<float4*>(&red[lrow * TM + lcol]) = dbacc;
        __syncthreads();
        if (tid < TM && o0 + tid < a.No) {
            float s = 0.f;
#pragma unroll
            for (int g = 0; g < 8; g++) s += red[g * TM + tid];
            slab[(size_t)a.No * a.Ni + o0 + tid] = s;
        }
    }
}

__global__ __launch_bounds__(256, 2) void gemm_tn_kernel(TnArgs a, int tiles_i, int nsplit, int rows_per_split) {
    tn_small_body(a, tiles_i, nsplit, rows_per_split, blockIdx.x);
}

__global__ __launch_bounds__(256, 2) void gemm_tn_group_kernel(TnGroup g) {
    const int b = blockIdx.x;
    int j = 0;
#pragma unroll
    for (int i = 1; i < PC_TN_GROUP; i++) j += (i < g.n && b >= g.block0[i]) ? 1 : 0;
    tn_small_body(g.a[j], g.tiles_i[j], g.nsplit[j], g.rps[j], b - g.block0[j]);
}

__device__ __attribute__((aligned(64))) float pc_tn_zero_chunk[16];

struct TnNoRider {};
template <int WO, int WI, int TO, int TI, int TKC, int NST, bool APRO, bool ZPRO, bool RIDER = false>
__global__ __launch_bounds__(64 * WO * WI, WO * WI / 4) void gemm_tn8_kernel(TnArgs a, int nsplit, int rows_per_split, int halves,
                                                                             size_t slab_half_off,
                                                                             std::conditional_t<RIDER, TnRider, TnNoRider> rider) {
    constexpr int NWV = WO * WI, THREADS = 64 * NWV;
    constexpr int NO = WO * TO * 32, NI = WI * TI * 32;
    constexpr int ZRS = NO == 256 ? 260 : NO, ARS = NI == 256 ? 260 : NI;
    constexpr bool ZSW = NO == 128, ASW = NI == 128;
    static_assert((NO == 128 || NO == 256) && (NI == 128 || NI == 256), "image widths");
    constexpr int ZF = TKC * ZRS, AF = TKC * ARS;
    constexpr int STAGE = ZF * (ZPRO ? 2 : 1) + AF;
    constexpr int JZ = TKC * NO / 256 / NWV, JA = TKC * NI / 256 / NWV;
    static_assert((TKC * NO) % (256 * NWV) == 0 && (TKC * NI) % (256 * NWV) == 0, "images must split into whole wave instructions over the waves");
    constexpr int JALL = JZ * (ZPRO ? 2 : 1) + JA;
    __shared__ __attribute__((aligned(1024))) float smem[NST * STAGE];

    const int tid = threadIdx.x, lane = tid & 63;
    const int w = __builtin_amdgcn_readfirstlane(tid >> 6), wo = w % WO, wi = w / WO;
    const int half = halves == 2 ? ((int)blockIdx.x >> 3) & 1 : 0;
    const int split = halves == 2 ? (((int)blockIdx.x >> 4) << 3) + ((int)blockIdx.x & 7) : (int)blockIdx.x;
    if (halves == 2) {
        a.Z += half * (WO * TO * 32);
        a.slabs += half * slab_half_off;
        if (a.db) a.db += half * (WO * TO * 32);
    }
    const int r_begin = split * rows_per_split;
    const int r_end = min(a.R, r_begin + rows_per_split);
    const float* const zsrc0 = pc_tn_zero_chunk;
    const unsigned lds0 = (unsigned)(uintptr_t)(lptr_t)&smem[0];
    if constexpr (RIDER) {
        int rid = -1;
#pragma unroll
        for (int i = 0; i < PC_TN_RIDERS; i++) rid = (int)blockIdx.x == rider.block[i] ? i : rid;
        if (rid >= 0) {
            static_assert(sizeof(smem) >= sizeof(BnFinBwdScratch) && THREADS == FIN4_CG * FIN4_LANES, "a finalize workgroup");
            bn_finalize_bwd_body(rider.fin, rider.si, rid, (int)threadIdx.x, reinterpret_cast<BnFinBwdScratch*>(smem));
            return;
        }
    }

    int zr[JZ], zc[JZ], ar[JA], ac[JA];
    unsigned zd[JZ], ad[JA];
#pragma unroll
    for (int j = 0; j < JZ; j++) {
        const int g = w + NWV * j, f = g * 256 + lane * 4;
        zr[j] = f / NO; zc[j] = f % NO;
        if (ZSW && (zr[j] & 8)) zc[j] ^= 32;
        zd[j] = (NO == 256 ? g * ZRS : g * 256) * 4;
    }
#pragma unroll
    for (int j = 0; j < JA; j++) {
        const int g = w + NWV * j, f = g * 256 + lane * 4;
        ar[j] = f / NI; ac[j] = f % NI;
        if (ASW && (ar[j] & 8)) ac[j] ^= 32;
        ad[j] = (NI == 256 ? g * ARS : g * 256) * 4;
    }
    int gidx[JA];
    auto load_gather = [&](int r0) {
#pragma unroll
        for (int j = 0; j < JA; j++) {
            const int r = r0 + ar[j];
            gidx[j] = (a.gather && r < r_end) ? a.gather[r] : r;
        }
    };
    auto issue = [&](int st, int r0) {
        const unsigned base = lds0 + st * (STAGE * 4);
#pragma unroll
        for (int j = 0; j < JZ; j++) {
            const int r = r0 + zr[j];
            const bool v = r < r_end && zc[j] < a.No;
            dma16(v ? a.Z + (size_t)r * a.ldz + zc[j] : zsrc0, base + zd[j]);
            if (ZPRO) dma16(v ? a.zaux + (size_t)r * a.ldzaux + zc[j] : zsrc0, base + ZF * 4 + zd[j]);
        }
#pragma unroll
        for (int j = 0; j < JA; j++) {
            const int r = r0 + ar[j];
            const bool v = r < r_end && ac[j] < a.Ni && gidx[j] >= 0;
            dma16(v ? a.A + (size_t)gidx[j] * a.lda + ac[j] : zsrc0, base + (ZPRO ? 2 : 1) * ZF * 4 + ad[j]);
        }
    };

    constexpr int ZT = NO / 4, AT = NI / 4;
    const int zrow = tid / ZT, zcol = (tid % ZT) * 4, arow = tid / AT, acol = (tid % AT) * 4;
    int zseg = -1;
    float4 zmu, zis, zsc, zc1, zc2;
    auto transform = [&](float* stage, int r0) {
        if (ZPRO && zcol < a.No) {
            float* Zs = stage;
            const float* Hs = stage + ZF;
#pragma unroll
            for (int p = 0; p < TKC / (THREADS / ZT); p++) {
                const int rr = zrow + (THREADS / ZT) * p, r = r0 + rr;
                if (r < r_end) {
                    const int s = seg_of_row(a.seg, r);
                    if (s != zseg) {
                        const size_t o = (size_t)s * a.No + zcol;
                        zmu = *reinterpret_cast<const float4*>(a.z_mean + o);
                        zis = *reinterpret_cast<const float4*>(a.z_invstd + o);
                        zsc = *reinterpret_cast<const float4*>(a.z_scale + o);
                        zc1 = *reinterpret_cast<const float4*>(a.z_c1 + o);
                        zc2 = *reinterpret_cast<const float4*>(a.z_c2 + o);
                        zseg = s;
                    }
                    const int zp = rr * ZRS + ((ZSW && (rr & 8)) ? zcol ^ 32 : zcol);
                    float4 z = *reinterpret_cast<const float4*>(&Zs[zp]);
                    const float4 h = *reinterpret_cast<const float4*>(&Hs[zp]);
                    const float zm = row_multiplicity(a.seg, r);
                    z.x = zsc.x * (z.x - zm * (zc1.x + (h.x - zmu.x) * zis.x * zc2.x));
                    z.y = zsc.y * (z.y - zm * (zc1.y + (h.y - zmu.y) * zis.y * zc2.y));
                    z.z = zsc.z * (z.z - zm * (zc1.z + (h.z - zmu.z) * zis.z * zc2.z));
                    z.w = zsc.w * (z.w - zm * (zc1.w + (h.w - zmu.w) * zis.w * zc2.w));
                    *reinterpret_cast<float4*>(&Zs[zp]) = z;
                }
            }
        }
        if (APRO && acol < a.Ni) {
            float* As = stage + (ZPRO ? 2 : 1) * ZF;
            int aseg = -1;
            float4 asc, ash;
#pragma unroll
            for (int p = 0; p < TKC / (THREADS / AT); p++) {
                const int rr = arow + (THREADS / AT) * p, r = r0 + rr;
                if (r < r_end) {
                    const int s = seg_of_row(a.seg, r);
                    if (s != aseg) {
                        asc = *reinterpret_cast<const float4*>(a.pscale + (size_t)s * a.Ni + acol);
                        ash = *reinterpret_cast<const float4*>(a.pshift + (size_t)s * a.Ni + acol);
                        aseg = s;
                    }
                    const int ap = rr * ARS + ((ASW && (rr & 8)) ? acol ^ 32 : acol);
                    float4 x = *reinterpret_cast<const float4*>(&As[ap]);
                    x.x = fast_tanh(x.x * asc.x + ash.x);
                    x.y = fast_tanh(x.y * asc.y + ash.y);
                    x.z = fast_tanh(x.z * asc.z + ash.z);
                    x.w = fast_tanh(x.w * asc.w + ash.w);
                    *reinterpret_cast<float4*>(&As[ap]) = x;
                }
            }
        }
    };

    f32x16 acc[TO][TI];
    float zsum[TO];
#pragma unroll
    for (int i = 0; i < TO; i++) {
        zsum[i] = 0.f;
#pragma unroll
        for (int j = 0; j < TI; j++)
#pragma unroll
            for (int r = 0; r < 16; r++) acc[i][j][r] = 0.f;
    }

    const int nchunk = (r_end - r_begin + TKC - 1) / TKC;
#pragma unroll
    for (int i = 0; i < NST - 1; i++)
        if (i < nchunk) { load_gather(r_begin + i * TKC); issue(i, r_begin + i * TKC); }
    if (NST - 1 < nchunk) load_gather(r_begin + (NST - 1) * TKC);
    static_assert(TKC % 16 == 0, "chunks are whole k groups");
    const int fz = 8 * (lane >> 5) * ZRS, fa = 8 * (lane >> 5) * ARS;
    int zo[TO], xo[TI];
#pragma unroll
    for (int i = 0; i < TO; i++) zo[i] = (wo * (TO * 32) + 32 * i + (lane & 31)) ^ ((ZSW && lane >= 32) ? 32 : 0);
#pragma unroll
    for (int j = 0; j < TI; j++) xo[j] = (wi * (TI * 32) + 32 * j + (lane & 31)) ^ ((ASW && lane >= 32) ? 32 : 0);
    int cur = 0;
    for (int c = 0; c < nchunk; c++) {
#ifndef PC_EXP_NO_VMWAIT
        if (c + NST - 1 <= nchunk) { asm volatile("s_waitcnt vmcnt(%0)" ::"n"((NST - 2) * JALL) : "memory"); }
        else { asm volatile("s_waitcnt vmcnt(0)" ::: "memory"); }
#endif
#ifndef PC_EXP_NO_BARRIER
        __syncthreads();
#endif
#ifndef PC_EXP_NO_DMA
        if (c + NST - 1 < nchunk) {
            issue(cur == 0 ? NST - 1 : cur - 1, r_begin + (c + NST - 1) * TKC);
            if (c + NST < nchunk) load_gather(r_begin + (c + NST) * TKC);
        }
#endif
        float* stage = smem + cur * STAGE;
        if (APRO || ZPRO) { transform(stage, r_begin + c * TKC); lds_sync(); }
        const float* Zs = stage + fz;
        const float* As = stage + (ZPRO ? 2 : 1) * ZF + fa;
#pragma unroll
        for (int g = 0; g < TKC / 16; g++) {
#if defined(PC_EXP_NO_LDSREAD)
#define PC_TNV(PTR, OFF) __int_as_float(a.R + t)
#else
#define PC_TNV(PTR, OFF) (PTR)[OFF]
#endif
            Split3 sx[TI];
#pragma unroll
            for (int j = 0; j < TI; j++) {
                float v[8];
#pragma unroll
                for (int t = 0; t < 8; t++) v[t] = PC_TNV(As, (16 * g + t) * ARS + xo[j]);
                sx[j] = PC_SPLIT(make_float4(v[0], v[1], v[2], v[3]), make_float4(v[4], v[5], v[6], v[7]));
            }
#pragma unroll
            for (int i = 0; i < TO; i++) {
                float v[8];
#pragma unroll
                for (int t = 0; t < 8; t++) v[t] = PC_TNV(Zs, (16 * g + t) * ZRS + zo[i]);
                zsum[i] += ((v[0] + v[1]) + (v[2] + v[3])) + ((v[4] + v[5]) + (v[6] + v[7]));
                const Split3 sz = PC_SPLIT(make_float4(v[0], v[1], v[2], v[3]), make_float4(v[4], v[5], v[6], v[7]));
#define PC_TERM(PZ, PX) _Pragma("unroll") for (int j = 0; j < TI; j++) acc[i][j] = PC_MFMA(sz.PZ, sx[j].PX, acc[i][j]);
                PC_PRIO_MFMA(PC_PRIO_TN_COND, 1);
                PC_TERM(p2, p0) PC_TERM(p0, p2) PC_TERM(p1, p1) PC_TERM(p1, p0) PC_TERM(p0, p1) PC_TERM(p0, p0)
                PC_PRIO_MFMA(PC_PRIO_TN_COND, 0);
#undef PC_TERM
            }
        }
        cur = cur + 1 == NST ? 0 : cur + 1;
    }

    float* slab = a.slabs + (size_t)split * ((size_t)a.No * a.Ni + a.No);
#pragma unroll
    for (int i = 0; i < TO; i++)
#pragma unroll
        for (int j = 0; j < TI; j++) {
            const int ci = wi * (TI * 32) + j * 32 + (lane & 31);
#pragma unroll
            for (int reg = 0; reg < 16; reg++) {
                const int o = wo * (TO * 32) + i * 32 + (reg & 3) + 8 * (reg >> 2) + 4 * (lane >> 5);
#ifdef PC_EXP_NO_SLAB
                if (o < a.No && ci < a.Ni && acc[i][j][reg] == 12345.678f) slab[(size_t)o * a.Ni + ci] = acc[i][j][reg];
#else
                if (o < a.No && ci < a.Ni) slab[(size_t)o * a.Ni + ci] = acc[i][j][reg];
#endif
            }
        }
    if (a.db && wi == 0) {
#pragma unroll
        for (int i = 0; i < TO; i++) {
            const float s = zsum[i] + __shfl_xor(zsum[i], 32, 64);
            const int o = wo * (TO * 32) + i * 32 + (lane & 31);
            if (lane < 32 && o < a.No) slab[(size_t)a.No * a.Ni + o] = s;
        }
    }
}

__device__ __forceinline__ void adam_rider4(const AdamRider& ad, size_t off, const float4 gv, float step_size, float bc2s) {
    float4 pv = *reinterpret_cast<float4*>(ad.p + off);
    float4 mv = *reinterpret_cast<float4*>(ad.m + off);
    float4 vv = *reinterpret_cast<float4*>(ad.v + off);
    if (pc_adam_dead(gv, mv, vv)) return;
#define ADAM1(c) pc_adam_update(pv.c, mv.c, vv.c, gv.c, step_size, bc2s, ad.omb1, ad.beta2f, ad.omb2, ad.eps);
    ADAM1(x) ADAM1(y) ADAM1(z) ADAM1(w)
#undef ADAM1
    *reinterpret_cast<float4*>(ad.p + off) = pv;
    *reinterpret_cast<float4*>(ad.m + off) = mv;
    *reinterpret_cast<float4*>(ad.v + off) = vv;
}

__device__ __forceinline__ void tn_reduce_body(const float* slabs, int nsplit, int n_w, int n_b, float* dW, float* db,
                                               int accumulate, int bid, const AdamRider* ad = nullptr, float step_size = 0.f,
                                               float bc2s = 0.f) {
    const int total4 = (n_w + (db ? n_b : 0)) / 4;
    const int t = bid * blockDim.x + threadIdx.x;
    const int j4 = t >> 3, g = t & 7;
    if (j4 >= total4) return;
    const size_t stride = (size_t)n_w + n_b;
    const float* src = slabs + (size_t)j4 * 4;
    float4 s = make_float4(0.f, 0.f, 0.f, 0.f);
#pragma unroll 4
    for (int k = g; k < nsplit; k += 8) {
        const float4 v = *reinterpret_cast<const float4*>(src + (size_t)k * stride);
        s.x += v.x; s.y += v.y; s.z += v.z; s.w += v.w;
    }
#pragma unroll
    for (int o = 1; o < 8; o <<= 1) {
        s.x += __shfl_xor(s.x, o, 64); s.y += __shfl_xor(s.y, o, 64);
        s.z += __shfl_xor(s.z, o, 64); s.w += __shfl_xor(s.w, o, 64);
    }
    if (g == 0) {
        const int j = j4 * 4;
        float* dst = j < n_w ? dW + j : db + (j - n_w);
        if (accumulate) {
            const float4 old = *reinterpret_cast<const float4*>(dst);
            s.x += old.x; s.y += old.y; s.z += old.z; s.w += old.w;
        }
        *reinterpret_cast<float4*>(dst) = s;
        if (ad) adam_rider4(*ad, (size_t)(dst - ad->g), s, step_size, bc2s);
    }
}

__global__ __launch_bounds__(256) void tn_reduce_kernel(const float* slabs, int nsplit, int n_w, int n_b, float* dW,
                                                        float* db, int accumulate) {
    tn_reduce_body(slabs, nsplit, n_w, n_b, dW, db, accumulate, blockIdx.x);
}
__global__ __launch_bounds__(256) void tn_reduce_group_kernel(TnReduceGroup g) {
    __shared__ float sc[2];
    const bool with_adam = g.ad.p != nullptr;
    const int n_rider = with_adam ? g.ad.rest_block0[g.ad.n_rest] : 0;
    const int b = (int)blockIdx.x - n_rider;
    if (with_adam) {
        if (threadIdx.x == 0) {
            const double bc1 = 1.0 - pow(g.ad.beta1, (double)g.ad.t);
            const double bc2 = 1.0 - pow(g.ad.beta2, (double)g.ad.t);
            sc[0] = (float)(g.ad.lr / bc1);
            sc[1] = (float)sqrt(bc2);
            if (blockIdx.x == 0 && g.ad.step_count) *g.ad.step_count = g.ad.t;
        }
        __syncthreads();
        if (b < 0) {
            const int rb = (int)blockIdx.x;
            int r = 0;
            for (int i = 1; i < g.ad.n_rest; i++) r += rb >= g.ad.rest_block0[i] ? 1 : 0;
            const int off = g.ad.rest_lo[r] + ((rb - g.ad.rest_block0[r]) * 256 + (int)threadIdx.x) * 4;
            if (off < g.ad.rest_hi[r])
                adam_rider4(g.ad, (size_t)off, *reinterpret_cast<const float4*>(g.ad.g + off), sc[0], sc[1]);
            return;
        }
    }
    int j = 0;
#pragma unroll
    for (int i = 1; i < PC_TN_RGROUP; i++) j += (i < g.n && b >= g.block0[i]) ? 1 : 0;
    tn_reduce_body(g.slabs[j], g.nsplit[j], g.n_w[j], g.n_b[j], g.dW[j], g.db[j], g.accumulate[j], b - g.block0[j],
                   with_adam ? &g.ad : nullptr, with_adam ? sc[0] : 0.f, with_adam ? sc[1] : 0.f);
}

static bool tn_full_tile(int R, int No, int Ni) {
    return R >= 8192 && No <= 256 && Ni <= 256 && (No > 128 || Ni > 128) && No % 64 == 0 && Ni % 64 == 0;
}

static void tn_plan(int R, int No, int Ni, int* nsplit, int* rows_per_split) {
    int s;
    if (tn_full_tile(R, No, Ni)) {
        s = 256;
    } else {
        const int tiles = ((No + TM - 1) / TM) * ((Ni + TM - 1) / TM);
        s = (512 + tiles - 1) / tiles;
    }
    const int max_s = (R + 63) / 64;
    if (s > max_s) s = max_s;
    if (s < 1) s = 1;
    int rps = (R + s - 1) / s;
    rps = (rps + TK - 1) / TK * TK;
    s = (R + rps - 1) / rps;
    *nsplit = s;
    *rows_per_split = rps;
}

size_t gemm_tn_workspace_floats(int R, int No, int Ni) {
    const int tiles = ((No + TM - 1) / TM) * ((Ni + TM - 1) / TM);
    int cap = (512 + tiles - 1) / tiles;
    if (No <= 256 && Ni <= 256 && (No > 128 || Ni > 128) && No % 64 == 0 && Ni % 64 == 0 && cap < 256) cap = 256;
    int s = (R + 63) / 64;
    if (s > cap) s = cap;
    if (s < 1) s = 1;
    return (size_t)s * ((size_t)No * Ni + No);
}

static int tn_defer_push(TnDefer* d, const float* slabs, size_t slab_floats, int nsplit, int n_w, int n_b, float* dW,
                         float* db, int accumulate) {
    if (d->r.n >= PC_TN_RGROUP) return PC_EINVAL;
    const size_t used = (size_t)nsplit * ((size_t)n_w + n_b);
    if (used > slab_floats) return PC_EWORKSPACE;
    for (int k = 0; k < d->r.n; k++) {
        const float* lo = d->r.slabs[k];
        const float* hi = lo + (size_t)d->r.nsplit[k] * ((size_t)d->r.n_w[k] + d->r.n_b[k]);
        if (slabs < hi && lo < slabs + used) return PC_EINVAL;
    }
    const int k = d->r.n++;
    d->r.slabs[k] = slabs; d->r.nsplit[k] = nsplit; d->r.n_w[k] = n_w; d->r.n_b[k] = n_b; d->r.dW[k] = dW; d->r.db[k] = db;
    d->r.accumulate[k] = accumulate; d->r.block0[k] = d->rblocks;
    d->rblocks += ((n_w + (db ? n_b : 0)) / 4 * 8 + 255) / 256;
    return PC_OK;
}

int launch_gemm_tn(const TnArgs& a, hipStream_t st, TnDefer* defer) {
    if ((!a.Z && !a.z_onehot) || !a.A || !a.dW || !a.slabs || a.R <= 0 || a.No <= 0 || a.Ni <= 0) return PC_EINVAL;
    if (a.No % 4 || a.Ni % 4 || (a.Z && a.ldz % 4) || a.lda % 4 || a.lddw != a.Ni) return PC_ESHAPE;
    if (a.z_onehot && (a.zaux || tn_full_tile(a.R, a.No, a.Ni))) return PC_ESHAPE;
    if (((uintptr_t)a.dW & 15) || (a.db && ((uintptr_t)a.db & 15)) || ((uintptr_t)a.slabs & 15)) return PC_ESHAPE;
    int nsplit, rps;
    tn_plan(a.R, a.No, a.Ni, &nsplit, &rps);
    if ((size_t)nsplit * ((size_t)a.No * a.Ni + a.No) > a.slab_floats) return PC_EWORKSPACE;
    const int tiles_o = (a.No + TM - 1) / TM, tiles_i = (a.Ni + TM - 1) / TM;
    const bool apro = a.prologue == NT_PRO_BNTANH, zpro = a.zaux != nullptr;
    const int pb = pc_prof_begin(PC_KIND_GEMM_TN, 2.0 * a.R * (double)a.No * a.Ni, st);
    if (tn_full_tile(a.R, a.No, a.Ni) && !(apro && zpro)) {
#define TN8(WO, WI, TO, TI, TKC, NST)                                                                         \
    do {                                                                                                      \
        if (apro) PC_LAUNCH((gemm_tn8_kernel<WO, WI, TO, TI, TKC, NST, true, false>), dim3(nsplit), dim3(64 * WO * WI), 0, st, a, nsplit, rps, 1, (size_t)0, TnNoRider{});    \
        else if (zpro && a.Ni > 128) PC_LAUNCH((gemm_tn8_kernel<2, 4, 4, 2, 16, 3, false, true>), dim3(nsplit), dim3(512), 0, st, a, nsplit, rps, 1, (size_t)0, TnNoRider{});  \
        else if (zpro) PC_LAUNCH((gemm_tn8_kernel<4, 2, 2, 2, 16, 3, false, true>), dim3(nsplit), dim3(512), 0, st, a, nsplit, rps, 1, (size_t)0, TnNoRider{});  \
        else PC_LAUNCH((gemm_tn8_kernel<WO, WI, TO, TI, TKC, NST, false, false>), dim3(nsplit), dim3(64 * WO * WI), 0, st, a, nsplit, rps, 1, (size_t)0, TnNoRider{});        \
    } while (0)
        if (a.No > 128 && a.Ni > 128) TN8(2, 4, 4, 2, 16, 3);
        else if (a.No > 128) TN8(4, 2, 2, 2, 32, 2);
        else TN8(2, 4, 2, 2, 32, 2);
#undef TN8
    } else {
        PC_LAUNCH(gemm_tn_kernel, dim3(tiles_o * tiles_i * nsplit), dim3(256), 0, st, a, tiles_i, nsplit, rps);
    }
    pc_prof_end(pb, st);
    PC_TRY(pc_launch_status());
    const int n_w = a.No * a.Ni, n_b = a.No;
    const int threads = (n_w + (a.db ? n_b : 0)) / 4 * 8;
    if (defer) return tn_defer_push(defer, a.slabs, a.slab_floats, nsplit, n_w, n_b, a.dW, a.db, a.accumulate);
    PC_LAUNCH(tn_reduce_kernel, dim3((threads + 255) / 256), dim3(256), 0, st, a.slabs, nsplit, n_w, n_b,
                       a.dW, a.db, a.accumulate);
    return pc_launch_status();
}

int launch_gemm_tn_halves(const TnArgs& a, float* slabs0, float* slabs1, size_t slab_floats, hipStream_t st, TnDefer* defer,
                          const TnRider* rider) {
    if (!a.Z || !a.A || !a.dW || !slabs0 || !slabs1 || !defer || a.R <= 0) return PC_EINVAL;
    if (a.No != 256 || a.Ni != 256 || a.ldz % 4 || a.lda % 4 || a.lddw != a.Ni || a.prologue != NT_PRO_NONE || a.zaux || a.z_onehot || a.gather)
        return PC_ESHAPE;
    if (slabs1 < slabs0) return PC_EINVAL;
    const int nsplit = 128;
    int rps = (a.R + nsplit - 1) / nsplit;
    rps = (rps + 31) / 32 * 32;
    const int used = (a.R + rps - 1) / rps;
    const size_t per = (size_t)128 * a.Ni + 128;
    if ((size_t)nsplit * per > slab_floats) return PC_EWORKSPACE;
    TnArgs h = a;
    h.No = 128; h.slabs = slabs0; h.slab_floats = slab_floats;
    TnRider rd = {};
    int blocks = 2 * nsplit, nred = nsplit;
    if (rider && rider->n) {
        if (rider->n != PC_TN_RIDERS) return PC_EINVAL;
        rd = *rider;
        int k = 0;
        for (int b = 0; b < 2 * nsplit && k < rd.n; b++)
            if (((b >> 4) << 3) + (b & 7) >= used) rd.block[k++] = b;
        if (k == rd.n) nred = used;
        else {
            for (k = 0; k < rd.n; k++) rd.block[k] = blocks + k;
            blocks += rd.n;
        }
    }
    const int pb = pc_prof_begin(PC_KIND_GEMM_TN, 2.0 * a.R * (double)a.No * a.Ni, st);
    if (rd.n)
        PC_LAUNCH((gemm_tn8_kernel<2, 4, 2, 2, 32, 2, false, false, true>), dim3(blocks), dim3(512), 0, st, h, nsplit, rps, 2,
                  (size_t)(slabs1 - slabs0), rd);
    else
        PC_LAUNCH((gemm_tn8_kernel<2, 4, 2, 2, 32, 2, false, false>), dim3(blocks), dim3(512), 0, st, h, nsplit, rps, 2,
                  (size_t)(slabs1 - slabs0), TnNoRider{});
    pc_prof_end(pb, st);
    PC_TRY(pc_launch_status());
    PC_TRY(tn_defer_push(defer, slabs0, slab_floats, nred, 128 * a.Ni, 128, a.dW, a.db, a.accumulate));
    return tn_defer_push(defer, slabs1, slab_floats, nred, 128 * a.Ni, 128, a.dW + (size_t)128 * a.Ni, a.db ? a.db + 128 : nullptr,
                         a.accumulate);
}

namespace {
struct ForkSlot { int dev; hipStream_t main_st; int state; PcFork f; };
ForkSlot g_fork_slots[32];
std::mutex g_fork_mu;
std::atomic<int> g_opt_side_queue{1};
std::atomic<int> g_opt_sorted_tables{1};
std::atomic<int> g_opt_bn_finalize_side{0};
std::atomic<int> g_opt_bn_finalize_rides{1};
std::atomic<int> g_opt_fused_loss{1};
std::atomic<int> g_opt_fused_out_chain{1};
std::atomic<int>* opt_slot(int option) {
    switch (option) {
        case PC_OPT_SIDE_QUEUE: return &g_opt_side_queue;
        case PC_OPT_SORTED_TABLE_GRADIENTS: return &g_opt_sorted_tables;
        case PC_OPT_BN_FINALIZE_SIDE: return &g_opt_bn_finalize_side;
        case PC_OPT_FUSED_LOSS: return &g_opt_fused_loss;
        case PC_OPT_FUSED_OUT_CHAIN: return &g_opt_fused_out_chain;
        case PC_OPT_BN_FINALIZE_RIDES: return &g_opt_bn_finalize_rides;
        default: return nullptr;
    }
}
}
int pc_opt_sorted_tables() { return g_opt_sorted_tables.load(std::memory_order_relaxed); }
int pc_opt_bn_finalize_side() { return g_opt_bn_finalize_side.load(std::memory_order_relaxed); }
int pc_opt_bn_finalize_rides() { return g_opt_bn_finalize_rides.load(std::memory_order_relaxed); }
int pc_opt_fused_loss() { return g_opt_fused_loss.load(std::memory_order_relaxed); }
int pc_opt_fused_out_chain() { return g_opt_fused_out_chain.load(std::memory_order_relaxed); }

extern "C" int pc_set_option(int option, int value) {
    std::atomic<int>* o = opt_slot(option);
    if (!o || (value != 0 && value != 1)) return PC_EINVAL;
    o->store(value, std::memory_order_relaxed);
    return PC_OK;
}
extern "C" int pc_get_option(int option, int* value) {
    std::atomic<int>* o = opt_slot(option);
    if (!o || !value) return PC_EINVAL;
    *value = o->load(std::memory_order_relaxed);
    return PC_OK;
}
extern "C" int pc_release_device_state(void) {
    std::lock_guard<std::mutex> lock(g_fork_mu);
    int cur = 0, rc = PC_OK;
    const bool have_cur = hipGetDevice(&cur) == hipSuccess;
    for (ForkSlot& c : g_fork_slots) {
        if (c.state == 1) {
            if (hipSetDevice(c.dev) != hipSuccess) { rc = (int)hipErrorInvalidDevice; continue; }
            (void)hipStreamSynchronize(c.f.side);
            for (int i = 0; i < PC_FORK_EVENTS; i++) { (void)hipEventDestroy(c.f.fork[i]); (void)hipEventDestroy(c.f.join[i]); }
            (void)hipStreamDestroy(c.f.side);
        }
        c = ForkSlot{};
    }
    if (have_cur) (void)hipSetDevice(cur);
    return rc;
}

PcFork* pc_fork_get(hipStream_t main_st) {
    int dev = 0;
    if (!g_opt_side_queue.load(std::memory_order_relaxed) || hipGetDevice(&dev) != hipSuccess) return nullptr;
    hipStreamCaptureStatus cap = hipStreamCaptureStatusNone;
    if (hipStreamIsCapturing(main_st, &cap) != hipSuccess || cap != hipStreamCaptureStatusNone) return nullptr;
    std::lock_guard<std::mutex> lock(g_fork_mu);
    ForkSlot* s = nullptr;
    for (ForkSlot& c : g_fork_slots) {
        if (c.state != 0 && c.dev == dev && c.main_st == main_st) { s = &c; break; }
        if (c.state == 0 && !s) s = &c;
    }
    if (!s) return nullptr;
    if (s->state == 0) {
        s->dev = dev; s->main_st = main_st;
        PcFork& f = s->f;
        int prio = 0;
        bool ok = (hipStreamGetPriority(main_st, &prio) == hipSuccess
                       ? hipStreamCreateWithPriority(&f.side, hipStreamNonBlocking, prio)
                       : hipStreamCreateWithFlags(&f.side, hipStreamNonBlocking)) == hipSuccess;
        for (int i = 0; ok && i < PC_FORK_EVENTS; i++)
            ok = hipEventCreateWithFlags(&f.fork[i], hipEventDisableTiming) == hipSuccess &&
                 hipEventCreateWithFlags(&f.join[i], hipEventDisableTiming) == hipSuccess;
        f.pending = 0;
        s->state = ok ? 1 : -1;
    }
    return s->state == 1 ? &s->f : nullptr;
}
int pc_fork_begin(PcFork* f, int i, hipStream_t main_st) {
    PC_HIP_TRY(hipEventRecord(f->fork[i], main_st));
    PC_HIP_TRY(hipStreamWaitEvent(f->side, f->fork[i], 0));
    f->pending = 1;
    return PC_OK;
}
int pc_fork_mark(PcFork* f, int i) {
    PC_HIP_TRY(hipEventRecord(f->join[i], f->side));
    return PC_OK;
}
int pc_fork_wait(PcFork* f, int i, hipStream_t main_st) {
    PC_HIP_TRY(hipStreamWaitEvent(main_st, f->join[i], 0));
    return PC_OK;
}
int pc_fork_join(PcFork* f, int i, hipStream_t main_st) {
    PC_TRY(pc_fork_mark(f, i));
    PC_TRY(pc_fork_wait(f, i, main_st));
    f->pending = 0;
    return PC_OK;
}

int launch_tn_reduce_deferred(TnDefer* d, hipStream_t st) {
    if (!d) return PC_EINVAL;
    if (d->fork && d->fork->pending) PC_TRY(pc_fork_join(d->fork, 1, st));
    if (d->r.n == 0 && !d->adam) return PC_OK;
    for (int k = d->r.n; k <= PC_TN_RGROUP; k++) d->r.block0[k] = d->rblocks;
    int blocks = d->rblocks;
    if (d->adam) {
        const pc_adam_fused* a = d->adam;
        if (!a->param || !a->grad || !a->exp_avg || !a->exp_avg_sq || a->n == 0 || a->n % 4 || a->t < 1 || a->n > 0x7fffffffu) return PC_EINVAL;
        if (((uintptr_t)a->param | (uintptr_t)a->grad | (uintptr_t)a->exp_avg | (uintptr_t)a->exp_avg_sq) & 15) return PC_ESHAPE;
        AdamRider& ad = d->r.ad;
        ad.p = a->param; ad.m = a->exp_avg; ad.v = a->exp_avg_sq; ad.g = a->grad; ad.n = a->n;
        ad.step_count = a->step_count; ad.t = (long long)a->t; ad.lr = a->lr; ad.beta1 = a->beta1; ad.beta2 = a->beta2;
        ad.omb1 = (float)(1.0 - a->beta1); ad.beta2f = (float)a->beta2; ad.omb2 = (float)(1.0 - a->beta2); ad.eps = (float)a->eps;
        long lo[2 * PC_TN_RGROUP], hi[2 * PC_TN_RGROUP];
        int ni = 0;
        for (int k = 0; k < d->r.n; k++) {
            const float* outs[2] = {d->r.dW[k], d->r.db[k]};
            const int lens[2] = {d->r.n_w[k], d->r.db[k] ? d->r.n_b[k] : 0};
            for (int u = 0; u < 2; u++) {
                if (!outs[u] || lens[u] == 0) continue;
                const long o = outs[u] - a->grad;
                if (o < 0 || o + lens[u] > (long)a->n || (o & 3) || (lens[u] & 3)) return PC_EINVAL;
                lo[ni] = o; hi[ni] = o + lens[u]; ni++;
            }
        }
        for (int i = 1; i < ni; i++)
            for (int j2 = i; j2 > 0 && lo[j2] < lo[j2 - 1]; j2--) { long t0 = lo[j2]; lo[j2] = lo[j2 - 1]; lo[j2 - 1] = t0; t0 = hi[j2]; hi[j2] = hi[j2 - 1]; hi[j2 - 1] = t0; }
        long cur = 0;
        int nr = 0, rb = 0;
        for (int i = 0; i <= ni; i++) {
            const long stop = i < ni ? lo[i] : (long)a->n;
            if (stop > cur) {
                if (nr >= PC_ADAM_REST) return PC_EINVAL;
                ad.rest_lo[nr] = (int)cur; ad.rest_hi[nr] = (int)stop; ad.rest_block0[nr] = rb;
                rb += (int)((stop - cur + 1023) / 1024);
                nr++;
            }
            if (i < ni) {
                if (lo[i] < cur) return PC_EINVAL;
                cur = hi[i];
            }
        }
        ad.n_rest = nr; ad.rest_block0[nr] = rb;
        ad.block0 = d->rblocks;
        blocks += rb;
    }
    if (blocks == 0) { tn_defer_init(d); return PC_OK; }
    PC_LAUNCH(tn_reduce_group_kernel, dim3(blocks), dim3(256), 0, st, d->r);
    tn_defer_init(d);
    return pc_launch_status();
}

int launch_gemm_tn_group(const TnArgs* args, int n, const TnReduceJob* extra, int n_extra, hipStream_t st, TnDefer* defer) {
    if (!args || n < 1 || n > PC_TN_GROUP || n_extra < 0 || n_extra > PC_TN_EXTRA || (n_extra && !extra)) return PC_EINVAL;
    TnGroup g = {};
    TnReduceGroup r = {};
    double flops = 0.0;
    int blocks = 0, rblocks = 0;
    int planned = 0;
    for (int i = 0; i < n; i++) {
        const TnArgs& a = args[i];
        if (tn_full_tile(a.R, a.No, a.Ni) || a.prologue != NT_PRO_NONE || a.R <= 0 || a.No <= 0 || a.Ni <= 0) continue;
        int ns, rp;
        tn_plan(a.R, a.No, a.Ni, &ns, &rp);
        planned += ((a.No + TM - 1) / TM) * ((a.Ni + TM - 1) / TM) * ns;
    }
    const double thin = planned > 512 ? 512.0 / planned : 1.0;
    for (int i = 0; i < n; i++) {
        const TnArgs& a = args[i];
        if (tn_full_tile(a.R, a.No, a.Ni) || a.prologue != NT_PRO_NONE) { PC_TRY(launch_gemm_tn(a, st, defer)); continue; }
        if ((!a.Z && !a.z_onehot) || !a.A || !a.dW || !a.slabs || a.R <= 0 || a.No <= 0 || a.Ni <= 0) return PC_EINVAL;
        if (a.No % 4 || a.Ni % 4 || (a.Z && a.ldz % 4) || a.lda % 4 || a.lddw != a.Ni) return PC_ESHAPE;
        if (a.z_onehot && a.zaux) return PC_EINVAL;
        if (((uintptr_t)a.dW & 15) || (a.db && ((uintptr_t)a.db & 15)) || ((uintptr_t)a.slabs & 15)) return PC_ESHAPE;
        int nsplit, rps;
        tn_plan(a.R, a.No, a.Ni, &nsplit, &rps);
        if (thin < 1.0) {
            int s2 = (int)(nsplit * thin);
            if (s2 < 1) s2 = 1;
            rps = ((a.R + s2 - 1) / s2 + TK - 1) / TK * TK;
            nsplit = (a.R + rps - 1) / rps;
        }
        if ((size_t)nsplit * ((size_t)a.No * a.Ni + a.No) > a.slab_floats) return PC_EWORKSPACE;
        for (int k = 0; k < g.n; k++) {
            const float* lo = g.a[k].slabs; const float* hi = lo + g.a[k].slab_floats;
            if (a.slabs < hi && lo < a.slabs + a.slab_floats) return PC_EINVAL;
        }
        const int tiles_o = (a.No + TM - 1) / TM, tiles_i = (a.Ni + TM - 1) / TM;
        const int k = g.n++;
        g.a[k] = a; g.tiles_i[k] = tiles_i; g.nsplit[k] = nsplit; g.rps[k] = rps; g.block0[k] = blocks;
        blocks += tiles_o * tiles_i * nsplit;
        const int n_w = a.No * a.Ni, n_b = a.No;
        r.slabs[k] = a.slabs; r.nsplit[k] = nsplit; r.n_w[k] = n_w; r.n_b[k] = n_b; r.dW[k] = a.dW; r.db[k] = a.db;
        r.accumulate[k] = a.accumulate; r.block0[k] = rblocks;
        rblocks += ((n_w + (a.db ? n_b : 0)) / 4 * 8 + 255) / 256;
        flops += 2.0 * a.R * (double)a.No * a.Ni;
    }
    r.n = g.n;
    for (int i = 0; i < n_extra; i++) {
        const TnReduceJob& e = extra[i];
        if (!e.slabs || !e.out || e.nsplit < 1 || e.n < 4 || e.n % 4 || ((uintptr_t)e.slabs & 15) || ((uintptr_t)e.out & 15))
            return PC_EINVAL;
        const int k = r.n++;
        r.slabs[k] = e.slabs; r.nsplit[k] = e.nsplit; r.n_w[k] = e.n; r.n_b[k] = 0; r.dW[k] = e.out; r.db[k] = nullptr;
        r.accumulate[k] = e.accumulate; r.block0[k] = rblocks;
        rblocks += (e.n / 4 * 8 + 255) / 256;
    }
    if (r.n == 0) return PC_OK;
    for (int k = g.n; k <= PC_TN_GROUP; k++) g.block0[k] = blocks;
    for (int k = r.n; k <= PC_TN_RGROUP; k++) r.block0[k] = rblocks;
    if (g.n) {
        const int pb = pc_prof_begin(PC_KIND_GEMM_TN, flops, st);
        PC_LAUNCH(gemm_tn_group_kernel, dim3(blocks), dim3(256), 0, st, g);
        pc_prof_end(pb, st);
        PC_TRY(pc_launch_status());
    }
    if (defer) {
        for (int k = 0; k < r.n; k++)
            PC_TRY(tn_defer_push(defer, r.slabs[k], (size_t)r.nsplit[k] * ((size_t)r.n_w[k] + r.n_b[k]), r.nsplit[k], r.n_w[k],
                                 r.n_b[k], r.dW[k], r.db[k], r.accumulate[k]));
        return PC_OK;
    }
    PC_LAUNCH(tn_reduce_group_kernel, dim3(rblocks), dim3(256), 0, st, r);
    return pc_launch_status();
}
```

Measured before the change: 5.065 million.

## Launch w5 and w3 weight-gradient GEMMs as one paired split-K kernel

Adds a paired TN GEMM path that computes the FFN backward dW5/db5 and both halves of dW3/db3 in a single launch. The grid is split into three parts of row slices plus bn-finalize rider blocks, sized so each CU gets one workgroup. The tn8 kernel body moves into a shared header so a pair variant can be compiled from it. The aim is to remove a kernel launch and fill the GPU better than two sequential launches, at the cost of more workspace slabs and a fixed slice count.

```diff
diff --git a/include/pcompanion_hip.h b/include/pcompanion_hip.h
--- a/include/pcompanion_hip.h
+++ b/include/pcompanion_hip.h
@@ -25,9 +25,10 @@
 #define PC_ABI_VERSION 8
 int pc_abi_version(void);
 enum { PC_OPT_SIDE_QUEUE = 1, PC_OPT_SORTED_TABLE_GRADIENTS = 2, PC_OPT_BN_FINALIZE_SIDE = 3, PC_OPT_FUSED_LOSS = 4,
-       PC_OPT_FUSED_OUT_CHAIN = 5, PC_OPT_BN_FINALIZE_RIDES = 6 };
+       PC_OPT_FUSED_OUT_CHAIN = 5, PC_OPT_BN_FINALIZE_RIDES = 6, PC_OPT_TN_PAIR = 7 };
 int pc_set_option(int option, int value);
 int pc_get_option(int option, int* value);
+int pc_tn_pair_plan(int rows, int* slices, int* rows_per_split, int* used_slices, size_t* slab_floats, size_t* region_floats);
 int pc_release_device_state(void);
 enum {
     PC_FLAG_EXP_NO_MFMA = 1, PC_FLAG_EXP_NO_SPLIT = 2, PC_FLAG_EXP_NO_LDSREAD = 4, PC_FLAG_EXP_NO_DMA = 8,
diff --git a/p_companion_amd/_lib.py b/p_companion_amd/_lib.py
--- a/p_companion_amd/_lib.py
+++ b/p_companion_amd/_lib.py
@@ -72,6 +72,7 @@
 PC_OPT_FUSED_LOSS = 4
 PC_OPT_BN_FINALIZE_SIDE = 3
 PC_OPT_BN_FINALIZE_RIDES = 6
+PC_OPT_TN_PAIR = 7
 PC_OPT_SORTED_TABLE_GRADIENTS = 2
 
 SIGNATURES = {
@@ -80,6 +81,7 @@
     "pc_set_option": (_i, [_i, _i]),
     "pc_get_option": (_i, [_i, ctypes.POINTER(ctypes.c_int)]),
     "pc_release_device_state": (_i, []),
+    "pc_tn_pair_plan": (_i, [_i, _P(_i), _P(_i), _P(_i), _P(_sz), _P(_sz)]),
     "pc_p2v_ffn_workspace_bytes": (_sz, [_i]),
     "pc_p2v_ffn_forward_train": (_i, [_P(P2VTensors), _vp, _vp, _i, _P(Segments), _i, _vp, _P(FfnSaved), _vp, _sz, _vp]),
     "pc_p2v_ffn_forward_eval": (_i, [_P(P2VTensors), _vp, _vp, _i, _vp, _vp, _sz, _vp]),
diff --git a/p_companion_amd/csrc/common.h b/p_companion_amd/csrc/common.h
--- a/p_companion_amd/csrc/common.h
+++ b/p_companion_amd/csrc/common.h
@@ -466,6 +466,9 @@
 struct TnRider;
 int launch_gemm_tn_halves(const TnArgs& a, float* slabs0, float* slabs1, size_t slab_floats, hipStream_t st, TnDefer* defer,
                           const TnRider* rider = nullptr);
+int launch_gemm_tn_pair(const TnArgs& a5, const TnArgs& a3, float* slabs5, float* slabs30, float* slabs31, size_t slab_floats,
+                        hipStream_t st, TnDefer* defer, const TnRider* rider = nullptr);
+bool gemm_tn_pair_fits(int R, size_t slab_floats);
 size_t gemm_tn_workspace_floats(int R, int No, int Ni);
 #define PC_TN_GROUP 10
 #define PC_TN_EXTRA 2
@@ -530,6 +533,7 @@
 int pc_opt_bn_finalize_rides();
 int pc_opt_fused_loss();
 int pc_opt_fused_out_chain();
+int pc_opt_tn_pair();
 int triplet_loss_launch(const float* a, const float* p, const float* n, int batch, int k_neg, int dim, float margin,
                         float* loss, float* d_pos, float* d_neg, float* da, float* dp, float* dn, void* stream, int with_mean);
 int launch_dropout(const float* x, size_t n, const pc_dropout& d, unsigned stream_id, float* y, hipStream_t st);
diff --git a/p_companion_amd/csrc/ffn.hip b/p_companion_amd/csrc/ffn.hip
--- a/p_companion_amd/csrc/ffn.hip
+++ b/p_companion_amd/csrc/ffn.hip
@@ -365,7 +365,9 @@
     t5.Z = dy; t5.ldz = D; t5.A = sv->a2; t5.lda = PC_H; t5.R = rows; t5.No = D; t5.Ni = PC_H; t5.seg = si;
     t5.dW = g->w5; t5.lddw = PC_H; t5.db = g->b5; t5.accumulate = accumulate; t5.slabs = w.slabs[0];
     t5.slab_floats = w.slab_floats;
-    if (D == 256 && rows >= 8192 && (size_t)2 * 128 * ((size_t)128 * PC_H + 128) <= w.slab_floats) {
+    const bool paired = pc_opt_tn_pair() && D == 128 && sv->a1 && gemm_tn_pair_fits(rows, w.slab_floats);
+    if (paired) {
+    } else if (D == 256 && rows >= 8192 && (size_t)2 * 128 * ((size_t)128 * PC_H + 128) <= w.slab_floats) {
         const size_t half = (size_t)128 * ((size_t)128 * PC_H + 128);
         PC_TRY(launch_gemm_tn_halves(t5, w.slabs[0], w.slabs[0] + half, half, st, df));
     } else {
@@ -400,7 +402,9 @@
     t3.dW = g->w3; t3.lddw = PC_H; t3.db = g->b3; t3.accumulate = accumulate; t3.slabs = w.slabs[1];
     t3.slab_floats = w.slab_floats;
     if (sv->a1) {
-        if (rows >= 8192 && (size_t)128 * ((size_t)128 * PC_H + 128) <= w.slab_floats) {
+        if (paired) {
+            PC_TRY(launch_gemm_tn_pair(t5, t3, w.slabs[0], w.slabs[1], w.slabs[2], w.slab_floats, st, df, fin_rider.n ? &fin_rider : nullptr));
+        } else if (rows >= 8192 && (size_t)128 * ((size_t)128 * PC_H + 128) <= w.slab_floats) {
             PC_TRY(launch_gemm_tn_halves(t3, w.slabs[1], w.slabs[2], w.slab_floats, st, df, fin_rider.n ? &fin_rider : nullptr));
         } else {
             for (int half = 0; half < 2; half++) {
diff --git a/p_companion_amd/csrc/gemm_tn.hip b/p_companion_amd/csrc/gemm_tn.hip
--- a/p_companion_amd/csrc/gemm_tn.hip
+++ b/p_companion_amd/csrc/gemm_tn.hip
@@ -153,249 +153,10 @@
     tn_small_body(g.a[j], g.tiles_i[j], g.nsplit[j], g.rps[j], b - g.block0[j]);
 }
 
-__device__ __attribute__((aligned(64))) float pc_tn_zero_chunk[16];
-
-struct TnNoRider {};
-template <int WO, int WI, int TO, int TI, int TKC, int NST, bool APRO, bool ZPRO, bool RIDER = false>
-__global__ __launch_bounds__(64 * WO * WI, WO * WI / 4) void gemm_tn8_kernel(TnArgs a, int nsplit, int rows_per_split, int halves,
-                                                                             size_t slab_half_off,
-                                                                             std::conditional_t<RIDER, TnRider, TnNoRider> rider) {
-    constexpr int NWV = WO * WI, THREADS = 64 * NWV;
-    constexpr int NO = WO * TO * 32, NI = WI * TI * 32;
-    constexpr int ZRS = NO == 256 ? 260 : NO, ARS = NI == 256 ? 260 : NI;
-    constexpr bool ZSW = NO == 128, ASW = NI == 128;
-    static_assert((NO == 128 || NO == 256) && (NI == 128 || NI == 256), "image widths");
-    constexpr int ZF = TKC * ZRS, AF = TKC * ARS;
-    constexpr int STAGE = ZF * (ZPRO ? 2 : 1) + AF;
-    constexpr int JZ = TKC * NO / 256 / NWV, JA = TKC * NI / 256 / NWV;
-    static_assert((TKC * NO) % (256 * NWV) == 0 && (TKC * NI) % (256 * NWV) == 0, "images must split into whole wave instructions over the waves");
-    constexpr int JALL = JZ * (ZPRO ? 2 : 1) + JA;
-    __shared__ __attribute__((aligned(1024))) float smem[NST * STAGE];
-
-    const int tid = threadIdx.x, lane = tid & 63;
-    const int w = __builtin_amdgcn_readfirstlane(tid >> 6), wo = w % WO, wi = w / WO;
-    const int half = halves == 2 ? ((int)blockIdx.x >> 3) & 1 : 0;
-    const int split = halves == 2 ? (((int)blockIdx.x >> 4) << 3) + ((int)blockIdx.x & 7) : (int)blockIdx.x;
-    if (halves == 2) {
-        a.Z += half * (WO * TO * 32);
-        a.slabs += half * slab_half_off;
-        if (a.db) a.db += half * (WO * TO * 32);
-    }
-    const int r_begin = split * rows_per_split;
-    const int r_end = min(a.R, r_begin + rows_per_split);
-    const float* const zsrc0 = pc_tn_zero_chunk;
-    const unsigned lds0 = (unsigned)(uintptr_t)(lptr_t)&smem[0];
-    if constexpr (RIDER) {
-        int rid = -1;
-#pragma unroll
-        for (int i = 0; i < PC_TN_RIDERS; i++) rid = (int)blockIdx.x == rider.block[i] ? i : rid;
-        if (rid >= 0) {
-            static_assert(sizeof(smem) >= sizeof(BnFinBwdScratch) && THREADS == FIN4_CG * FIN4_LANES, "a finalize workgroup");
-            bn_finalize_bwd_body(rider.fin, rider.si, rid, (int)threadIdx.x, reinterpret_cast<BnFinBwdScratch*>(smem));
-            return;
-        }
-    }
-
-    int zr[JZ], zc[JZ], ar[JA], ac[JA];
-    unsigned zd[JZ], ad[JA];
-#pragma unroll
-    for (int j = 0; j < JZ; j++) {
-        const int g = w + NWV * j, f = g * 256 + lane * 4;
-        zr[j] = f / NO; zc[j] = f % NO;
-        if (ZSW && (zr[j] & 8)) zc[j] ^= 32;
-        zd[j] = (NO == 256 ? g * ZRS : g * 256) * 4;
-    }
-#pragma unroll
-    for (int j = 0; j < JA; j++) {
-        const int g = w + NWV * j, f = g * 256 + lane * 4;
-        ar[j] = f / NI; ac[j] = f % NI;
-        if (ASW && (ar[j] & 8)) ac[j] ^= 32;
-        ad[j] = (NI == 256 ? g * ARS : g * 256) * 4;
-    }
-    int gidx[JA];
-    auto load_gather = [&](int r0) {
-#pragma unroll
-        for (int j = 0; j < JA; j++) {
-            const int r = r0 + ar[j];
-            gidx[j] = (a.gather && r < r_end) ? a.gather[r] : r;
-        }
-    };
-    auto issue = [&](int st, int r0) {
-        const unsigned base = lds0 + st * (STAGE * 4);
-#pragma unroll
-        for (int j = 0; j < JZ; j++) {
-            const int r = r0 + zr[j];
-            const bool v = r < r_end && zc[j] < a.No;
-            dma16(v ? a.Z + (size_t)r * a.ldz + zc[j] : zsrc0, base + zd[j]);
-            if (ZPRO) dma16(v ? a.zaux + (size_t)r * a.ldzaux + zc[j] : zsrc0, base + ZF * 4 + zd[j]);
-        }
-#pragma unroll
-        for (int j = 0; j < JA; j++) {
-            const int r = r0 + ar[j];
-            const bool v = r < r_end && ac[j] < a.Ni && gidx[j] >= 0;
-            dma16(v ? a.A + (size_t)gidx[j] * a.lda + ac[j] : zsrc0, base + (ZPRO ? 2 : 1) * ZF * 4 + ad[j]);
-        }
-    };
-
-    constexpr int ZT = NO / 4, AT = NI / 4;
-    const int zrow = tid / ZT, zcol = (tid % ZT) * 4, arow = tid / AT, acol = (tid % AT) * 4;
-    int zseg = -1;
-    float4 zmu, zis, zsc, zc1, zc2;
-    auto transform = [&](float* stage, int r0) {
-        if (ZPRO && zcol < a.No) {
-            float* Zs = stage;
-            const float* Hs = stage + ZF;
-#pragma unroll
-            for (int p = 0; p < TKC / (THREADS / ZT); p++) {
-                const int rr = zrow + (THREADS / ZT) * p, r = r0 + rr;
-                if (r < r_end) {
-                    const int s = seg_of_row(a.seg, r);
-                    if (s != zseg) {
-                        const size_t o = (size_t)s * a.No + zcol;
-                        zmu = *reinterpret_cast<const float4*>(a.z_mean + o);
-                        zis = *reinterpret_cast<const float4*>(a.z_invstd + o);
-                        zsc = *reinterpret_cast<const float4*>(a.z_scale + o);
-                        zc1 = *reinterpret_cast<const float4*>(a.z_c1 + o);
-                        zc2 = *reinterpret_cast<const float4*>(a.z_c2 + o);
-                        zseg = s;
-                    }
-                    const int zp = rr * ZRS + ((ZSW && (rr & 8)) ? zcol ^ 32 : zcol);
-                    float4 z = *reinterpret_cast<const float4*>(&Zs[zp]);
-                    const float4 h = *reinterpret_cast<const float4*>(&Hs[zp]);
-                    const float zm = row_multiplicity(a.seg, r);
-                    z.x = zsc.x * (z.x - zm * (zc1.x + (h.x - zmu.x) * zis.x * zc2.x));
-                    z.y = zsc.y * (z.y - zm * (zc1.y + (h.y - zmu.y) * zis.y * zc2.y));
-                    z.z = zsc.z * (z.z - zm * (zc1.z + (h.z - zmu.z) * zis.z * zc2.z));
-                    z.w = zsc.w * (z.w - zm * (zc1.w + (h.w - zmu.w) * zis.w * zc2.w));
-                    *reinterpret_cast<float4*>(&Zs[zp]) = z;
-                }
-            }
-        }
-        if (APRO && acol < a.Ni) {
-            float* As = stage + (ZPRO ? 2 : 1) * ZF;
-            int aseg = -1;
-            float4 asc, ash;
-#pragma unroll
-            for (int p = 0; p < TKC / (THREADS / AT); p++) {
-                const int rr = arow + (THREADS / AT) * p, r = r0 + rr;
-                if (r < r_end) {
-                    const int s = seg_of_row(a.seg, r);
-                    if (s != aseg) {
-                        asc = *reinterpret_cast<const float4*>(a.pscale + (size_t)s * a.Ni + acol);
-                        ash = *reinterpret_cast<const float4*>(a.pshift + (size_t)s * a.Ni + acol);
-                        aseg = s;
-                    }
-                    const int ap = rr * ARS + ((ASW && (rr & 8)) ? acol ^ 32 : acol);
-                    float4 x = *reinterpret_cast<const float4*>(&As[ap]);
-                    x.x = fast_tanh(x.x * asc.x + ash.x);
-                    x.y = fast_tanh(x.y * asc.y + ash.y);
-                    x.z = fast_tanh(x.z * asc.z + ash.z);
-                    x.w = fast_tanh(x.w * asc.w + ash.w);
-                    *reinterpret_cast<float4*>(&As[ap]) = x;
-                }
-            }
-        }
-    };
-
-    f32x16 acc[TO][TI];
-    float zsum[TO];
-#pragma unroll
-    for (int i = 0; i < TO; i++) {
-        zsum[i] = 0.f;
-#pragma unroll
-        for (int j = 0; j < TI; j++)
-#pragma unroll
-            for (int r = 0; r < 16; r++) acc[i][j][r] = 0.f;
-    }
-
-    const int nchunk = (r_end - r_begin + TKC - 1) / TKC;
-#pragma unroll
-    for (int i = 0; i < NST - 1; i++)
-        if (i < nchunk) { load_gather(r_begin + i * TKC); issue(i, r_begin + i * TKC); }
-    if (NST - 1 < nchunk) load_gather(r_begin + (NST - 1) * TKC);
-    static_assert(TKC % 16 == 0, "chunks are whole k groups");
-    const int fz = 8 * (lane >> 5) * ZRS, fa = 8 * (lane >> 5) * ARS;
-    int zo[TO], xo[TI];
-#pragma unroll
-    for (int i = 0; i < TO; i++) zo[i] = (wo * (TO * 32) + 32 * i + (lane & 31)) ^ ((ZSW && lane >= 32) ? 32 : 0);
-#pragma unroll
-    for (int j = 0; j < TI; j++) xo[j] = (wi * (TI * 32) + 32 * j + (lane & 31)) ^ ((ASW && lane >= 32) ? 32 : 0);
-    int cur = 0;
-    for (int c = 0; c < nchunk; c++) {
-#ifndef PC_EXP_NO_VMWAIT
-        if (c + NST - 1 <= nchunk) { asm volatile("s_waitcnt vmcnt(%0)" ::"n"((NST - 2) * JALL) : "memory"); }
-        else { asm volatile("s_waitcnt vmcnt(0)" ::: "memory"); }
-#endif
-#ifndef PC_EXP_NO_BARRIER
-        __syncthreads();
-#endif
-#ifndef PC_EXP_NO_DMA
-        if (c + NST - 1 < nchunk) {
-            issue(cur == 0 ? NST - 1 : cur - 1, r_begin + (c + NST - 1) * TKC);
-            if (c + NST < nchunk) load_gather(r_begin + (c + NST) * TKC);
-        }
-#endif
-        float* stage = smem + cur * STAGE;
-        if (APRO || ZPRO) { transform(stage, r_begin + c * TKC); lds_sync(); }
-        const float* Zs = stage + fz;
-        const float* As = stage + (ZPRO ? 2 : 1) * ZF + fa;
-#pragma unroll
-        for (int g = 0; g < TKC / 16; g++) {
-#if defined(PC_EXP_NO_LDSREAD)
-#define PC_TNV(PTR, OFF) __int_as_float(a.R + t)
-#else
-#define PC_TNV(PTR, OFF) (PTR)[OFF]
-#endif
-            Split3 sx[TI];
-#pragma unroll
-            for (int j = 0; j < TI; j++) {
-                float v[8];
-#pragma unroll
-                for (int t = 0; t < 8; t++) v[t] = PC_TNV(As, (16 * g + t) * ARS + xo[j]);
-                sx[j] = PC_SPLIT(make_float4(v[0], v[1], v[2], v[3]), make_float4(v[4], v[5], v[6], v[7]));
-            }
-#pragma unroll
-            for (int i = 0; i < TO; i++) {
-                float v[8];
-#pragma unroll
-                for (int t = 0; t < 8; t++) v[t] = PC_TNV(Zs, (16 * g + t) * ZRS + zo[i]);
-                zsum[i] += ((v[0] + v[1]) + (v[2] + v[3])) + ((v[4] + v[5]) + (v[6] + v[7]));
-                const Split3 sz = PC_SPLIT(make_float4(v[0], v[1], v[2], v[3]), make_float4(v[4], v[5], v[6], v[7]));
-#define PC_TERM(PZ, PX) _Pragma("unroll") for (int j = 0; j < TI; j++) acc[i][j] = PC_MFMA(sz.PZ, sx[j].PX, acc[i][j]);
-                PC_PRIO_MFMA(PC_PRIO_TN_COND, 1);
-                PC_TERM(p2, p0) PC_TERM(p0, p2) PC_TERM(p1, p1) PC_TERM(p1, p0) PC_TERM(p0, p1) PC_TERM(p0, p0)
-                PC_PRIO_MFMA(PC_PRIO_TN_COND, 0);
-#undef PC_TERM
-            }
-        }
-        cur = cur + 1 == NST ? 0 : cur + 1;
-    }
-
-    float* slab = a.slabs + (size_t)split * ((size_t)a.No * a.Ni + a.No);
-#pragma unroll
-    for (int i = 0; i < TO; i++)
-#pragma unroll
-        for (int j = 0; j < TI; j++) {
-            const int ci = wi * (TI * 32) + j * 32 + (lane & 31);
-#pragma unroll
-            for (int reg = 0; reg < 16; reg++) {
-                const int o = wo * (TO * 32) + i * 32 + (reg & 3) + 8 * (reg >> 2) + 4 * (lane >> 5);
-#ifdef PC_EXP_NO_SLAB
-                if (o < a.No && ci < a.Ni && acc[i][j][reg] == 12345.678f) slab[(size_t)o * a.Ni + ci] = acc[i][j][reg];
-#else
-                if (o < a.No && ci < a.Ni) slab[(size_t)o * a.Ni + ci] = acc[i][j][reg];
-#endif
-            }
-        }
-    if (a.db && wi == 0) {
-#pragma unroll
-        for (int i = 0; i < TO; i++) {
-            const float s = zsum[i] + __shfl_xor(zsum[i], 32, 64);
-            const int o = wo * (TO * 32) + i * 32 + (lane & 31);
-            if (lane < 32 && o < a.No) slab[(size_t)a.No * a.Ni + o] = s;
-        }
-    }
-}
+#define TN8_KERNEL gemm_tn8_kernel
+#define TN8_ZERO pc_tn_zero_chunk
+#define TN8_PAIR 0
+#include "gemm_tn8.h"
 
 __device__ __forceinline__ void adam_rider4(const AdamRider& ad, size_t off, const float4 gv, float step_size, float bc2s) {
     float4 pv = *reinterpret_cast<float4*>(ad.p + off);
@@ -604,6 +365,75 @@
                          a.accumulate);
 }
 
+#ifndef PC_TN_PAIR_SLICES
+#define PC_TN_PAIR_SLICES 80
+static_assert(3 * PC_TN_PAIR_SLICES + PC_TN_RIDERS <= 256 && 3 * ((PC_TN_PAIR_SLICES + 7) / 8) + (PC_TN_RIDERS + 7) / 8 <= 32,
+              "three parts and the riders: one workgroup per CU of every XCD");
+#endif
+#define PC_TN_PAIR_PER ((size_t)128 * PC_H + 128)
+static void tn_pair_plan(int R, int* rows_per_split, int* used) {
+    int rps = (R + PC_TN_PAIR_SLICES - 1) / PC_TN_PAIR_SLICES;
+    rps = (rps + 31) / 32 * 32;
+    *rows_per_split = rps;
+    *used = (R + rps - 1) / rps;
+}
+bool gemm_tn_pair_fits(int R, size_t slab_floats) {
+    if (R < 8192) return false;
+    int rps, used;
+    tn_pair_plan(R, &rps, &used);
+    return (size_t)used * PC_TN_PAIR_PER <= slab_floats;
+}
+extern "C" int pc_tn_pair_plan(int rows, int* slices, int* rows_per_split, int* used_slices, size_t* slab_floats,
+                               size_t* region_floats) {
+    if (rows <= 0 || !slices || !rows_per_split || !used_slices || !slab_floats || !region_floats) return PC_EINVAL;
+    *slices = PC_TN_PAIR_SLICES;
+    tn_pair_plan(rows, rows_per_split, used_slices);
+    *slab_floats = (size_t)*used_slices * PC_TN_PAIR_PER;
+    *region_floats = gemm_tn_workspace_floats(rows, PC_H, PC_H);
+    for (size_t f : {gemm_tn_workspace_floats(rows, PC_D, PC_H), gemm_tn_workspace_floats(rows, PC_H, PC_D)})
+        if (f > *region_floats) *region_floats = f;
+    return PC_OK;
+}
+
+int launch_gemm_tn_pair(const TnArgs& a5, const TnArgs& a3, float* slabs5, float* slabs30, float* slabs31, size_t slab_floats,
+                        hipStream_t st, TnDefer* defer, const TnRider* rider) {
+    if (!a5.Z || !a5.A || !a5.dW || !a3.Z || !a3.A || !a3.dW || !slabs5 || !slabs30 || !slabs31 || !defer) return PC_EINVAL;
+    if (a5.R < 8192 || a3.R != a5.R || !a5.db || !a3.db) return PC_EINVAL;
+    for (const TnArgs* t : {&a5, &a3})
+        if (t->Ni != PC_H || t->ldz % 4 || t->lda % 4 || t->lddw != t->Ni || t->prologue != NT_PRO_NONE || t->zaux || t->z_onehot || t->gather)
+            return PC_ESHAPE;
+    if (a5.No != 128 || a3.No != 256) return PC_ESHAPE;
+    if (((uintptr_t)slabs5 | (uintptr_t)slabs30 | (uintptr_t)slabs31 | (uintptr_t)a5.dW | (uintptr_t)a3.dW | (uintptr_t)a5.db | (uintptr_t)a3.db) & 15)
+        return PC_ESHAPE;
+    int rps, used;
+    tn_pair_plan(a5.R, &rps, &used);
+    if ((size_t)used * PC_TN_PAIR_PER > slab_floats) return PC_EWORKSPACE;
+    TnArgs h = a5;
+    h.slabs = slabs5; h.slab_floats = slab_floats;
+    const TnPair pair = {{a3.Z, a3.A, slabs30, a3.ldz, a3.lda}, {a3.Z + 128, a3.A, slabs31, a3.ldz, a3.lda}};
+    const int last = used - 1;
+    int blocks = 24 * (last >> 3) + 16 + (last & 7) + 1;
+    TnRider rd = {};
+    if (rider && rider->n) {
+        if (rider->n != PC_TN_RIDERS) return PC_EINVAL;
+        rd = *rider;
+        int k = 0;
+        for (int b = 0; b < blocks && k < rd.n; b++)
+            if (((b / 24) << 3) + (b % 24 & 7) >= used) rd.block[k++] = b;
+        if (k < rd.n) {
+            for (k = 0; k < rd.n; k++) rd.block[k] = blocks + k;
+            blocks += rd.n;
+        }
+    }
+    const int pb = pc_prof_begin(PC_KIND_GEMM_TN, 2.0 * a5.R * ((double)a5.No * a5.Ni + (double)a3.No * a3.Ni), st);
+    const int rc = launch_tn8_pair(h, rps, pair, rd.n ? &rd : nullptr, blocks, st);
+    pc_prof_end(pb, st);
+    PC_TRY(rc);
+    PC_TRY(tn_defer_push(defer, slabs5, slab_floats, used, 128 * PC_H, 128, a5.dW, a5.db, a5.accumulate));
+    PC_TRY(tn_defer_push(defer, slabs30, slab_floats, used, 128 * PC_H, 128, a3.dW, a3.db, a3.accumulate));
+    return tn_defer_push(defer, slabs31, slab_floats, used, 128 * PC_H, 128, a3.dW + (size_t)128 * PC_H, a3.db + 128, a3.accumulate);
+}
+
 namespace {
 struct ForkSlot { int dev; hipStream_t main_st; int state; PcFork f; };
 ForkSlot g_fork_slots[32];
@@ -614,6 +444,7 @@
 std::atomic<int> g_opt_bn_finalize_rides{1};
 std::atomic<int> g_opt_fused_loss{1};
 std::atomic<int> g_opt_fused_out_chain{1};
+std::atomic<int> g_opt_tn_pair{0};
 std::atomic<int>* opt_slot(int option) {
     switch (option) {
         case PC_OPT_SIDE_QUEUE: return &g_opt_side_queue;
@@ -622,6 +453,7 @@
         case PC_OPT_FUSED_LOSS: return &g_opt_fused_loss;
         case PC_OPT_FUSED_OUT_CHAIN: return &g_opt_fused_out_chain;
         case PC_OPT_BN_FINALIZE_RIDES: return &g_opt_bn_finalize_rides;
+        case PC_OPT_TN_PAIR: return &g_opt_tn_pair;
         default: return nullptr;
     }
 }
@@ -631,6 +463,7 @@
 int pc_opt_bn_finalize_rides() { return g_opt_bn_finalize_rides.load(std::memory_order_relaxed); }
 int pc_opt_fused_loss() { return g_opt_fused_loss.load(std::memory_order_relaxed); }
 int pc_opt_fused_out_chain() { return g_opt_fused_out_chain.load(std::memory_order_relaxed); }
+int pc_opt_tn_pair() { return g_opt_tn_pair.load(std::memory_order_relaxed); }
 
 extern "C" int pc_set_option(int option, int value) {
     std::atomic<int>* o = opt_slot(option);
diff --git a/p_companion_amd/csrc/gemm_tn8.h b/p_companion_amd/csrc/gemm_tn8.h
--- /dev/null
+++ b/p_companion_amd/csrc/gemm_tn8.h
@@ -0,0 +1,263 @@
+__device__ __attribute__((aligned(64))) float TN8_ZERO[16];
+
+struct TnNoRider {};
+struct TnPairPart { const float* Z; const float* A; float* slabs; int ldz, lda; };
+struct TnPair { TnPairPart p1, p2; };
+int launch_tn8_pair(const TnArgs& a, int rows_per_split, const TnPair& pair, const TnRider* rider, int blocks, hipStream_t st);
+template <int WO, int WI, int TO, int TI, int TKC, int NST, bool APRO, bool ZPRO, bool RIDER = false>
+__global__ __launch_bounds__(64 * WO * WI, WO * WI / 4) void TN8_KERNEL(TnArgs a, int nsplit, int rows_per_split, int halves,
+                                                                        size_t slab_half_off,
+                                                                        std::conditional_t<RIDER, TnRider, TnNoRider> rider
+#if TN8_PAIR
+                                                                        , TnPair pair
+#endif
+                                                                        ) {
+    constexpr int NWV = WO * WI, THREADS = 64 * NWV;
+    constexpr int NO = WO * TO * 32, NI = WI * TI * 32;
+    constexpr int ZRS = NO == 256 ? 260 : NO, ARS = NI == 256 ? 260 : NI;
+    constexpr bool ZSW = NO == 128, ASW = NI == 128;
+    static_assert((NO == 128 || NO == 256) && (NI == 128 || NI == 256), "image widths");
+    constexpr int ZF = TKC * ZRS, AF = TKC * ARS;
+    constexpr int STAGE = ZF * (ZPRO ? 2 : 1) + AF;
+    constexpr int JZ = TKC * NO / 256 / NWV, JA = TKC * NI / 256 / NWV;
+    static_assert((TKC * NO) % (256 * NWV) == 0 && (TKC * NI) % (256 * NWV) == 0, "images must split into whole wave instructions over the waves");
+    constexpr int JALL = JZ * (ZPRO ? 2 : 1) + JA;
+    __shared__ __attribute__((aligned(1024))) float smem[NST * STAGE];
+
+    const int tid = threadIdx.x, lane = tid & 63;
+    const int w = __builtin_amdgcn_readfirstlane(tid >> 6), wo = w % WO, wi = w / WO;
+    const int half = halves == 2 ? ((int)blockIdx.x >> 3) & 1 : 0;
+#if TN8_PAIR
+    const int grp = (int)blockIdx.x / 24, in = (int)blockIdx.x - 24 * grp, part = in >> 3;
+    const int split = (grp << 3) + (in & 7);
+    a.Z = part == 0 ? a.Z : part == 1 ? pair.p1.Z : pair.p2.Z;
+    a.ldz = part == 0 ? a.ldz : part == 1 ? pair.p1.ldz : pair.p2.ldz;
+    a.A = part == 0 ? a.A : part == 1 ? pair.p1.A : pair.p2.A;
+    a.lda = part == 0 ? a.lda : part == 1 ? pair.p1.lda : pair.p2.lda;
+    a.slabs = part == 0 ? a.slabs : part == 1 ? pair.p1.slabs : pair.p2.slabs;
+#else
+    const int split = halves == 2 ? (((int)blockIdx.x >> 4) << 3) + ((int)blockIdx.x & 7) : (int)blockIdx.x;
+#endif
+    if (halves == 2) {
+        a.Z += half * (WO * TO * 32);
+        a.slabs += half * slab_half_off;
+        if (a.db) a.db += half * (WO * TO * 32);
+    }
+    const int r_begin = split * rows_per_split;
+    const int r_end = min(a.R, r_begin + rows_per_split);
+    const float* const zsrc0 = TN8_ZERO;
+    const unsigned lds0 = (unsigned)(uintptr_t)(lptr_t)&smem[0];
+    if constexpr (RIDER) {
+        int rid = -1;
+#pragma unroll
+        for (int i = 0; i < PC_TN_RIDERS; i++) rid = (int)blockIdx.x == rider.block[i] ? i : rid;
+        if (rid >= 0) {
+            static_assert(sizeof(smem) >= sizeof(BnFinBwdScratch) && THREADS == FIN4_CG * FIN4_LANES, "a finalize workgroup");
+            bn_finalize_bwd_body(rider.fin, rider.si, rid, (int)threadIdx.x, reinterpret_cast<BnFinBwdScratch*>(smem));
+            return;
+        }
+    }
+#if TN8_PAIR
+    if (r_begin >= a.R) return;
+#endif
+
+    int zr[JZ], zc[JZ], ar[JA], ac[JA];
+    unsigned zd[JZ], ad[JA];
+#pragma unroll
+    for (int j = 0; j < JZ; j++) {
+        const int g = w + NWV * j, f = g * 256 + lane * 4;
+        zr[j] = f / NO; zc[j] = f % NO;
+        if (ZSW && (zr[j] & 8)) zc[j] ^= 32;
+        zd[j] = (NO == 256 ? g * ZRS : g * 256) * 4;
+    }
+#pragma unroll
+    for (int j = 0; j < JA; j++) {
+        const int g = w + NWV * j, f = g * 256 + lane * 4;
+        ar[j] = f / NI; ac[j] = f % NI;
+        if (ASW && (ar[j] & 8)) ac[j] ^= 32;
+        ad[j] = (NI == 256 ? g * ARS : g * 256) * 4;
+    }
+    int gidx[JA];
+    auto load_gather = [&](int r0) {
+#pragma unroll
+        for (int j = 0; j < JA; j++) {
+            const int r = r0 + ar[j];
+            gidx[j] = (a.gather && r < r_end) ? a.gather[r] : r;
+        }
+    };
+    auto issue = [&](int st, int r0) {
+        const unsigned base = lds0 + st * (STAGE * 4);
+#pragma unroll
+        for (int j = 0; j < JZ; j++) {
+            const int r = r0 + zr[j];
+            const bool v = r < r_end && zc[j] < a.No;
+            dma16(v ? a.Z + (size_t)r * a.ldz + zc[j] : zsrc0, base + zd[j]);
+            if (ZPRO) dma16(v ? a.zaux + (size_t)r * a.ldzaux + zc[j] : zsrc0, base + ZF * 4 + zd[j]);
+        }
+#pragma unroll
+        for (int j = 0; j < JA; j++) {
+            const int r = r0 + ar[j];
+            const bool v = r < r_end && ac[j] < a.Ni && gidx[j] >= 0;
+            dma16(v ? a.A + (size_t)gidx[j] * a.lda + ac[j] : zsrc0, base + (ZPRO ? 2 : 1) * ZF * 4 + ad[j]);
+        }
+    };
+
+    constexpr int ZT = NO / 4, AT = NI / 4;
+    const int zrow = tid / ZT, zcol = (tid % ZT) * 4, arow = tid / AT, acol = (tid % AT) * 4;
+    int zseg = -1;
+    float4 zmu, zis, zsc, zc1, zc2;
+    auto transform = [&](float* stage, int r0) {
+        if (ZPRO && zcol < a.No) {
+            float* Zs = stage;
+            const float* Hs = stage + ZF;
+#pragma unroll
+            for (int p = 0; p < TKC / (THREADS / ZT); p++) {
+                const int rr = zrow + (THREADS / ZT) * p, r = r0 + rr;
+                if (r < r_end) {
+                    const int s = seg_of_row(a.seg, r);
+                    if (s != zseg) {
+                        const size_t o = (size_t)s * a.No + zcol;
+                        zmu = *reinterpret_cast<const float4*>(a.z_mean + o);
+                        zis = *reinterpret_cast<const float4*>(a.z_invstd + o);
+                        zsc = *reinterpret_cast<const float4*>(a.z_scale + o);
+                        zc1 = *reinterpret_cast<const float4*>(a.z_c1 + o);
+                        zc2 = *reinterpret_cast<const float4*>(a.z_c2 + o);
+                        zseg = s;
+                    }
+                    const int zp = rr * ZRS + ((ZSW && (rr & 8)) ? zcol ^ 32 : zcol);
+                    float4 z = *reinterpret_cast<const float4*>(&Zs[zp]);
+                    const float4 h = *reinterpret_cast<const float4*>(&Hs[zp]);
+                    const float zm = row_multiplicity(a.seg, r);
+                    z.x = zsc.x * (z.x - zm * (zc1.x + (h.x - zmu.x) * zis.x * zc2.x));
+                    z.y = zsc.y * (z.y - zm * (zc1.y + (h.y - zmu.y) * zis.y * zc2.y));
+                    z.z = zsc.z * (z.z - zm * (zc1.z + (h.z - zmu.z) * zis.z * zc2.z));
+                    z.w = zsc.w * (z.w - zm * (zc1.w + (h.w - zmu.w) * zis.w * zc2.w));
+                    *reinterpret_cast<float4*>(&Zs[zp]) = z;
+                }
+            }
+        }
+        if (APRO && acol < a.Ni) {
+            float* As = stage + (ZPRO ? 2 : 1) * ZF;
+            int aseg = -1;
+            float4 asc, ash;
+#pragma unroll
+            for (int p = 0; p < TKC / (THREADS / AT); p++) {
+                const int rr = arow + (THREADS / AT) * p, r = r0 + rr;
+                if (r < r_end) {
+                    const int s = seg_of_row(a.seg, r);
+                    if (s != aseg) {
+                        asc = *reinterpret_cast<const float4*>(a.pscale + (size_t)s * a.Ni + acol);
+                        ash = *reinterpret_cast<const float4*>(a.pshift + (size_t)s * a.Ni + acol);
+                        aseg = s;
+                    }
+                    const int ap = rr * ARS + ((ASW && (rr & 8)) ? acol ^ 32 : acol);
+                    float4 x = *reinterpret_cast<const float4*>(&As[ap]);
+                    x.x = fast_tanh(x.x * asc.x + ash.x);
+                    x.y = fast_tanh(x.y * asc.y + ash.y);
+                    x.z = fast_tanh(x.z * asc.z + ash.z);
+                    x.w = fast_tanh(x.w * asc.w + ash.w);
+                    *reinterpret_cast<float4*>(&As[ap]) = x;
+                }
+            }
+        }
+    };
+
+    f32x16 acc[TO][TI];
+    float zsum[TO];
+#pragma unroll
+    for (int i = 0; i < TO; i++) {
+        zsum[i] = 0.f;
+#pragma unroll
+        for (int j = 0; j < TI; j++)
+#pragma unroll
+            for (int r = 0; r < 16; r++) acc[i][j][r] = 0.f;
+    }
+
+    const int nchunk = (r_end - r_begin + TKC - 1) / TKC;
+#pragma unroll
+    for (int i = 0; i < NST - 1; i++)
+        if (i < nchunk) { load_gather(r_begin + i * TKC); issue(i, r_begin + i * TKC); }
+    if (NST - 1 < nchunk) load_gather(r_begin + (NST - 1) * TKC);
+    static_assert(TKC % 16 == 0, "chunks are whole k groups");
+    const int fz = 8 * (lane >> 5) * ZRS, fa = 8 * (lane >> 5) * ARS;
+    int zo[TO], xo[TI];
+#pragma unroll
+    for (int i = 0; i < TO; i++) zo[i] = (wo * (TO * 32) + 32 * i + (lane & 31)) ^ ((ZSW && lane >= 32) ? 32 : 0);
+#pragma unroll
+    for (int j = 0; j < TI; j++) xo[j] = (wi * (TI * 32) + 32 * j + (lane & 31)) ^ ((ASW && lane >= 32) ? 32 : 0);
+    int cur = 0;
+    for (int c = 0; c < nchunk; c++) {
+#ifndef PC_EXP_NO_VMWAIT
+        if (c + NST - 1 <= nchunk) { asm volatile("s_waitcnt vmcnt(%0)" ::"n"((NST - 2) * JALL) : "memory"); }
+        else { asm volatile("s_waitcnt vmcnt(0)" ::: "memory"); }
+#endif
+#ifndef PC_EXP_NO_BARRIER
+        __syncthreads();
+#endif
+#ifndef PC_EXP_NO_DMA
+        if (c + NST - 1 < nchunk) {
+            issue(cur == 0 ? NST - 1 : cur - 1, r_begin + (c + NST - 1) * TKC);
+            if (c + NST < nchunk) load_gather(r_begin + (c + NST) * TKC);
+        }
+#endif
+        float* stage = smem + cur * STAGE;
+        if (APRO || ZPRO) { transform(stage, r_begin + c * TKC); lds_sync(); }
+        const float* Zs = stage + fz;
+        const float* As = stage + (ZPRO ? 2 : 1) * ZF + fa;
+#pragma unroll
+        for (int g = 0; g < TKC / 16; g++) {
+#if defined(PC_EXP_NO_LDSREAD)
+#define PC_TNV(PTR, OFF) __int_as_float(a.R + t)
+#else
+#define PC_TNV(PTR, OFF) (PTR)[OFF]
+#endif
+            Split3 sx[TI];
+#pragma unroll
+            for (int j = 0; j < TI; j++) {
+                float v[8];
+#pragma unroll
+                for (int t = 0; t < 8; t++) v[t] = PC_TNV(As, (16 * g + t) * ARS + xo[j]);
+                sx[j] = PC_SPLIT(make_float4(v[0], v[1], v[2], v[3]), make_float4(v[4], v[5], v[6], v[7]));
+            }
+#pragma unroll
+            for (int i = 0; i < TO; i++) {
+                float v[8];
+#pragma unroll
+                for (int t = 0; t < 8; t++) v[t] = PC_TNV(Zs, (16 * g + t) * ZRS + zo[i]);
+                zsum[i] += ((v[0] + v[1]) + (v[2] + v[3])) + ((v[4] + v[5]) + (v[6] + v[7]));
+                const Split3 sz = PC_SPLIT(make_float4(v[0], v[1], v[2], v[3]), make_float4(v[4], v[5], v[6], v[7]));
+#define PC_TERM(PZ, PX) _Pragma("unroll") for (int j = 0; j < TI; j++) acc[i][j] = PC_MFMA(sz.PZ, sx[j].PX, acc[i][j]);
+                PC_PRIO_MFMA(PC_PRIO_TN_COND, 1);
+                PC_TERM(p2, p0) PC_TERM(p0, p2) PC_TERM(p1, p1) PC_TERM(p1, p0) PC_TERM(p0, p1) PC_TERM(p0, p0)
+                PC_PRIO_MFMA(PC_PRIO_TN_COND, 0);
+#undef PC_TERM
+            }
+        }
+        cur = cur + 1 == NST ? 0 : cur + 1;
+    }
+
+    float* slab = a.slabs + (size_t)split * ((size_t)a.No * a.Ni + a.No);
+#pragma unroll
+    for (int i = 0; i < TO; i++)
+#pragma unroll
+        for (int j = 0; j < TI; j++) {
+            const int ci = wi * (TI * 32) + j * 32 + (lane & 31);
+#pragma unroll
+            for (int reg = 0; reg < 16; reg++) {
+                const int o = wo * (TO * 32) + i * 32 + (reg & 3) + 8 * (reg >> 2) + 4 * (lane >> 5);
+#ifdef PC_EXP_NO_SLAB
+                if (o < a.No && ci < a.Ni && acc[i][j][reg] == 12345.678f) slab[(size_t)o * a.Ni + ci] = acc[i][j][reg];
+#else
+                if (o < a.No && ci < a.Ni) slab[(size_t)o * a.Ni + ci] = acc[i][j][reg];
+#endif
+            }
+        }
+    if (a.db && wi == 0) {
+#pragma unroll
+        for (int i = 0; i < TO; i++) {
+            const float s = zsum[i] + __shfl_xor(zsum[i], 32, 64);
+            const int o = wo * (TO * 32) + i * 32 + (lane & 31);
+            if (lane < 32 && o < a.No) slab[(size_t)a.No * a.Ni + o] = s;
+        }
+    }
+}
diff --git a/p_companion_amd/csrc/gemm_tn_pair.hip b/p_companion_amd/csrc/gemm_tn_pair.hip
--- /dev/null
+++ b/p_companion_amd/csrc/gemm_tn_pair.hip
@@ -0,0 +1,19 @@
+#include <type_traits>
+#include "common.h"
+#include "bn_finalize.h"
+#include "lds_dma.h"
+
+#define TN8_KERNEL gemm_tn8_pair_kernel
+#define TN8_ZERO pc_tn_pair_zero_chunk
+#define TN8_PAIR 1
+#include "gemm_tn8.h"
+
+int launch_tn8_pair(const TnArgs& a, int rows_per_split, const TnPair& pair, const TnRider* rider, int blocks, hipStream_t st) {
+    if (rider && rider->n)
+        PC_LAUNCH((gemm_tn8_pair_kernel<2, 4, 2, 2, 32, 2, false, false, true>), dim3(blocks), dim3(512), 0, st, a, 0, rows_per_split, 1,
+                  (size_t)0, *rider, pair);
+    else
+        PC_LAUNCH((gemm_tn8_pair_kernel<2, 4, 2, 2, 32, 2, false, false>), dim3(blocks), dim3(512), 0, st, a, 0, rows_per_split, 1,
+                  (size_t)0, TnNoRider{}, pair);
+    return pc_launch_status();
+}
```

Measured after the change: 5.061 million. About the same (-0.1%).
